# ezorita/seeq

Hardware: AMD Instinct MI355X
Metric: lines/s scanned (20 bp pattern, d=3, 150 bp reads; GB/s in gb_per_s) (higher is better)
Workload: dtype int (u16 automaton state ids; exact-pass columns u32 bit-vectors)

## Files before the change

seeq_amd/csrc/seeq_device.hip:

```cpp
#include <hip/hip_runtime.h>

#include <errno.h>
#include <pthread.h>
#include <stdint.h>
#include <stdio.h>
#include <stdlib.h>
#include <string.h>
#include <time.h>

#include "seeq_amd.h"
#include "seeq_kernel_core.h"
extern "C" {
#include "seeq_pattern.h"
}

static thread_local char g_last_error[256] = "";

static int hip_fail(hipError_t e, const char *what, int err_no)
{
   snprintf(g_last_error, sizeof g_last_error, "%s: %s", what, hipGetErrorString(e));
   seeqerr = 0;
   errno = err_no;
   return -1;
}

#define HIP_TRY(call, err_no)                                        \
   do {                                                              \
      hipError_t e_ = (call);                                        \
      if (e_ != hipSuccess) return hip_fail(e_, #call, (err_no));    \
   } while (0)

extern "C" const char *seeqdevLastError(void) { return g_last_error; }

static int use_device(int device)
{
   int cur = -1;
   if (hipGetDevice(&cur) == hipSuccess && cur == device) return 0;
   HIP_TRY(hipSetDevice(device), ENODEV);
   return 0;
}

extern "C" int seeqdevDeviceCount(void)
{
   int n = 0;
   if (hipGetDeviceCount(&n) != hipSuccess) return 0;
   return n;
}

extern "C" int seeqdevSetDevice(int device)
{
   HIP_TRY(hipSetDevice(device), ENODEV);
   return 0;
}

#include "seeq_types.h"
#include "seeq_scan_common.h"

static constexpr int WG = 256;
static constexpr int TILE = 16384;
static constexpr size_t FUSED_MIN_TILE = 512;
static constexpr int STREAM_NW_HOST = 16;
static constexpr uint32_t STREAM_CH_HOST = 128;
static constexpr size_t MAX_FUSED_GRID = 16384;
static constexpr size_t SAMPLE_BYTES = 65536;

#include "seeq_generic.h"
#include "seeq_scan.h"
#include "seeq_fused_post.h"
#include "seeq_direct.h"
#include "seeq_exact1.h"
#include "seeq_stream.h"
#include "seeq_pair.h"
#include "seeq_packed.h"
#include "seeq_multi.h"
#include "seeq_demux.h"
#include "seeq_tiles.h"
#include "seeq_fastq.h"
#include "seeq_strand.h"
#include "seeq_insert.h"
#include "seeq_tally.h"
#include "seeq_tally_group.h"
#include "seeq_tally_library.h"
#include "seeq_tally_collapse.h"
#include "seeq_qgate.h"
static_assert(sizeof(seeqdev_tally_pair_t) == 24 && sizeof(seeqdev_tally_group_t) == 24, "pair and group entries are written as three 64-bit words");
static_assert(sizeof(seeqdev_tally_collapse_t) == sizeof(uint4) && SEEQ_COLLAPSE_DIRECTIONAL == SEEQDEV_COLLAPSE_DIRECTIONAL && SEEQ_COLLAPSE_ANY == SEEQDEV_COLLAPSE_ANY,
              "collapse rows are written as uint4");
static_assert(sizeof(seeqdev_demux_t) == 16 && sizeof(seeqdev_hit_t) == sizeof(uint4), "demux records are written as uint4");
static_assert(sizeof(seeqdev_insert_t) == sizeof(uint4), "insert records are written as uint4");
static_assert(sizeof(seeqdev_tally_t) == sizeof(uint4) && SEEQ_TALLY_LEN_MAX == SEEQDEV_TALLY_MAX_LEN, "tally entries are written as uint4");
#include "seeq_post.h"
static_assert(STREAM_NW == STREAM_NW_HOST, "waves per k_stream workgroup");
extern "C" {
#include "seeq_dfa.h"
}
#include "seeq_synth.h"

static unsigned long g_pattern_ids = 0;

struct seeqdev_pattern {
   unsigned long id;
   int       wlen, tau, words;
   int       device;
   uint32_t *d_peq;
   char     *keys;
   uint32_t *h_peq;
   int       sdfa_state;
   uint16_t *d_sdfa;
   uint16_t *d_sdfa_skip;
   uint16_t *d_sdfa_restart;
   uint32_t  sdfa_rows, sdfa_final_base;
   int       sdfa_parts;
   int       sdfa_warm;
   double    sdfa_pacc;
   int       pair_state;
   uint16_t *d_pair;
   uint32_t  pair_units;
   uint32_t  pair_states;
   int       pair_parts, pair_mp, pair_warm;
   double    pair_pacc;
   int       quad_state;
   uint16_t *d_quad;
   uint32_t  quad_units;
   uint32_t  quad_states;
   int       quad_parts, quad_mp;
   double    quad_pacc;
   pthread_mutex_t plan_lock;
   struct seeqdev_pattern *twin;
};

#define SEEQ_FOR_WORDS(words, FN, ...) \
   ((words) <= 1 ? FN<1>(__VA_ARGS__) : (words) <= 2 ? FN<2>(__VA_ARGS__) : (words) <= 4 ? FN<4>(__VA_ARGS__) : (words) <= 8 ? FN<8>(__VA_ARGS__) : FN<16>(__VA_ARGS__))

extern "C" seeqdev_pattern_t *seeqdevPatternNew(const char *keys, int wlen, int tau)
{
   seeqerr = 0;
   if (!keys || wlen < 1 || tau < 0 || tau >= wlen) { errno = EINVAL; return NULL; }
   if (wlen > SEEQDEV_MAX_WLEN) {
      snprintf(g_last_error, sizeof g_last_error, "pattern longer than %d positions", SEEQDEV_MAX_WLEN);
      errno = E2BIG;
      return NULL;
   }
   if (seeqdevDeviceCount() < 1) {
      snprintf(g_last_error, sizeof g_last_error, "no HIP device: seeq-mi355x has no CPU matcher");
      errno = ENODEV;
      return NULL;
   }
   seeqdev_pattern *p = (seeqdev_pattern *)calloc(1, sizeof *p);
   if (!p) return NULL;
   p->id = __atomic_add_fetch(&g_pattern_ids, 1ul, __ATOMIC_RELAXED);
   pthread_mutex_init(&p->plan_lock, NULL);
   p->wlen = wlen; p->tau = tau; p->words = seeq_words_for(wlen);
   p->keys = (char *)malloc((size_t)wlen);
   if (p->keys) memcpy(p->keys, keys, (size_t)wlen);
   const size_t nw = (size_t)10 * p->words;
   uint32_t *h = (uint32_t *)malloc(nw * sizeof(uint32_t));
   char *rkeys = (char *)malloc((size_t)wlen);
   if (!h || !rkeys || !p->keys) { free(h); free(rkeys); free(p->keys); free(p); errno = ENOMEM; return NULL; }
   for (int i = 0; i < wlen; i++) rkeys[i] = keys[wlen - 1 - i];
   seeq_build_peq(keys, wlen, p->words, h);
   seeq_build_peq(rkeys, wlen, p->words, h + 5 * p->words);
   hipError_t e = hipGetDevice(&p->device);
   if (e == hipSuccess) e = hipMalloc((void **)&p->d_peq, nw * sizeof(uint32_t));
   if (e == hipSuccess) e = hipMemcpy(p->d_peq, h, nw * sizeof(uint32_t), hipMemcpyHostToDevice);
   free(rkeys);
   p->h_peq = h;
   if (e != hipSuccess) {
      hip_fail(e, "seeqdevPatternNew", e == hipErrorOutOfMemory ? ENOMEM : EIO);
      if (p->d_peq) (void)hipFree(p->d_peq);
      free(p->keys);
      free(h);
      free(p);
      return NULL;
   }
   return p;
}

extern "C" int seeqdevPatternDevice(const seeqdev_pattern_t *p) { return p ? p->device : -1; }

extern "C" void seeqdevPatternFree(seeqdev_pattern_t *p)
{
   if (!p) return;
   if (p->twin) seeqdevPatternFree(p->twin);
   (void)use_device(p->device);
   if (p->d_peq) (void)hipFree(p->d_peq);
   if (p->d_sdfa) (void)hipFree(p->d_sdfa);
   if (p->d_sdfa_skip) (void)hipFree(p->d_sdfa_skip);
   if (p->d_sdfa_restart) (void)hipFree(p->d_sdfa_restart);
   if (p->d_pair) (void)hipFree(p->d_pair);
   if (p->d_quad) (void)hipFree(p->d_quad);
   pthread_mutex_destroy(&p->plan_lock);
   free(p->keys);
   free(p->h_peq);
   free(p);
}

static void pattern_plan_stream(seeqdev_pattern *mp, bool complete_only)
{
   pthread_mutex_lock(&mp->plan_lock);
   if (mp->sdfa_state == 0 && mp->keys) {
      int state = -1;
      seeq_dfa_t *d = seeq_dfa_plan_stream(mp->keys, mp->wlen, mp->tau, complete_only ? 1 : 0);
      if (d) {
         const size_t bytes = (size_t)d->nrows * 16;
         uint16_t *skip = seeq_dfa_skip_variant(d);
         uint16_t *rst = d->nparts > 1 ? seeq_dfa_restart_variant(d) : nullptr;
         uint16_t *t0 = nullptr, *t1 = nullptr, *t2 = nullptr;
         if (skip && (rst || d->nparts <= 1) && hipMalloc((void **)&t0, bytes) == hipSuccess && hipMemcpy(t0, d->table, bytes, hipMemcpyHostToDevice) == hipSuccess &&
             hipMalloc((void **)&t1, bytes) == hipSuccess && hipMemcpy(t1, skip, bytes, hipMemcpyHostToDevice) == hipSuccess &&
             (!rst || (hipMalloc((void **)&t2, bytes) == hipSuccess && hipMemcpy(t2, rst, bytes, hipMemcpyHostToDevice) == hipSuccess))) {
            mp->d_sdfa = t0; mp->d_sdfa_skip = t1; mp->d_sdfa_restart = t2;
            mp->sdfa_rows = d->nrows;
            mp->sdfa_final_base = d->acc_final;
            mp->sdfa_parts = d->nparts;
            mp->sdfa_warm = d->warm;
            mp->sdfa_pacc = d->p_accept;
            state = 1;
         } else {
            if (t0) (void)hipFree(t0);
            if (t1) (void)hipFree(t1);
            if (t2) (void)hipFree(t2);
         }
         free(skip);
         free(rst);
         seeq_dfa_free(d);
      }
      __atomic_store_n(&mp->sdfa_state, state, __ATOMIC_RELEASE);
   }
   pthread_mutex_unlock(&mp->plan_lock);
}

static void pattern_plan_pair(seeqdev_pattern *mp)
{
   pthread_mutex_lock(&mp->plan_lock);
   if (mp->pair_state == 0 && mp->keys) {
      int state = -1;
      seeq_pair_t *d = seeq_pair_plan(mp->keys, mp->wlen, mp->tau);
      if (d) {
         const size_t bytes = d->table_bytes;
         uint16_t *t0 = nullptr;
         if (hipMalloc((void **)&t0, bytes) == hipSuccess && hipMemcpy(t0, d->table, bytes, hipMemcpyHostToDevice) == hipSuccess) {
            mp->d_pair = t0;
            mp->pair_units = d->table_bytes / 16;
            mp->pair_states = d->nstates;
            mp->pair_parts = d->nparts; mp->pair_mp = d->mp; mp->pair_warm = d->warm;
            mp->pair_pacc = d->p_accept;
            state = 1;
         } else if (t0) {
            (void)hipFree(t0);
         }
         seeq_pair_free(d);
      }
      __atomic_store_n(&mp->pair_state, state, __ATOMIC_RELEASE);
   }
   pthread_mutex_unlock(&mp->plan_lock);
}

static void pattern_plan_quad(seeqdev_pattern *mp)
{
   pthread_mutex_lock(&mp->plan_lock);
   if (mp->quad_state == 0 && mp->keys) {
      int state = -1;
      seeq_quad_t *d = seeq_quad_plan(mp->keys, mp->wlen, mp->tau);
      if (d) {
         uint16_t *t0 = nullptr;
         if (hipMalloc((void **)&t0, d->table_bytes) == hipSuccess && hipMemcpy(t0, d->table, d->table_bytes, hipMemcpyHostToDevice) == hipSuccess) {
            mp->d_quad = t0;
            mp->quad_units = d->table_bytes / 16;
            mp->quad_states = d->nstates;
            mp->quad_parts = d->nparts; mp->quad_mp = d->mp;
            mp->quad_pacc = d->p_accept;
            state = 1;
         } else if (t0) {
            (void)hipFree(t0);
         }
         seeq_quad_free(d);
      }
      __atomic_store_n(&mp->quad_state, state, __ATOMIC_RELEASE);
   }
   pthread_mutex_unlock(&mp->plan_lock);
}

struct MultiPlan {
   int            npat;
   unsigned long  ids[SEEQ_MULTI_MAX];
   int            state;
   seeqdev_pattern upat;
   uint16_t      *d_res_next;
   uint32_t      *d_res_mask;
   uint32_t       res_states;
   int            maxspan;
   int            m[SEEQ_MULTI_MAX], tau[SEEQ_MULTI_MAX], fw[SEEQ_MULTI_MAX];
   uint32_t      *d_eq;
   int            eq_options;
   uint32_t       pair_states, raw_states;
   int            lp_min, exact;
};

static void multi_plan_free(MultiPlan *mp)
{
   if (!mp) return;
   if (mp->d_res_next) (void)hipFree(mp->d_res_next);
   if (mp->d_res_mask) (void)hipFree(mp->d_res_mask);
   if (mp->d_eq) (void)hipFree(mp->d_eq);
   if (mp->upat.d_pair) (void)hipFree(mp->upat.d_pair);
   if (mp->upat.d_peq) (void)hipFree(mp->upat.d_peq);
   free(mp->upat.h_peq);
   free(mp);
}

static MultiPlan *multi_plan_for(MultiPlan **slot, const seeqdev_pattern_t *const *pats, int npat)
{
   MultiPlan *mp = *slot;
   if (mp && mp->npat == npat) {
      bool same = true;
      for (int k = 0; k < npat; k++) same = same && mp->ids[k] == pats[k]->id;
      if (same) return mp;
   }
   multi_plan_free(mp);
   *slot = mp = (MultiPlan *)calloc(1, sizeof *mp);
   if (!mp) return NULL;
   mp->npat = npat;
   mp->state = -1;
   mp->eq_options = -1;
   for (int k = 0; k < npat; k++) mp->ids[k] = pats[k]->id;
   if (npat < 2 || npat > SEEQ_MULTI_MAX) return mp;
   const char *keys[SEEQ_MULTI_MAX];
   for (int k = 0; k < npat; k++) {
      if (!pats[k]->keys || pats[k]->wlen > FUSED_MAX_WLEN2) return mp;
      keys[k] = pats[k]->keys; mp->m[k] = pats[k]->wlen; mp->tau[k] = pats[k]->tau;
      mp->fw[k] = pats[k]->wlen <= FUSED_MAX_WLEN ? 1 : 2;
   }
   seeq_multi_t *d = seeq_multi_build(keys, mp->m, mp->tau, npat);
   if (!d) return mp;
   if (d->maxspan <= FUSED_MAX_WLEN2) {
      seeqdev_pattern &u = mp->upat;
      u.id = __atomic_add_fetch(&g_pattern_ids, 1ul, __ATOMIC_RELAXED);
      u.wlen = d->maxspan; u.tau = 0; u.words = seeq_words_for(d->maxspan);
      u.device = pats[0]->device;
      u.sdfa_state = -1;
      u.h_peq = (uint32_t *)calloc((size_t)10 * u.words, sizeof(uint32_t));
      bool ok = u.h_peq != NULL;
      ok = ok && hipMalloc((void **)&u.d_peq, (size_t)10 * u.words * sizeof(uint32_t)) == hipSuccess;
      ok = ok && hipMemset(u.d_peq, 0, (size_t)10 * u.words * sizeof(uint32_t)) == hipSuccess;
      ok = ok && hipMalloc((void **)&u.d_pair, d->pair->table_bytes) == hipSuccess;
      ok = ok && hipMemcpy(u.d_pair, d->pair->table, d->pair->table_bytes, hipMemcpyHostToDevice) == hipSuccess;
      ok = ok && hipMalloc((void **)&mp->d_res_next, (size_t)d->res_states * 16) == hipSuccess;
      ok = ok && hipMemcpy(mp->d_res_next, d->res_next, (size_t)d->res_states * 16, hipMemcpyHostToDevice) == hipSuccess;
      ok = ok && hipMalloc((void **)&mp->d_res_mask, (size_t)d->res_states * 4) == hipSuccess;
      ok = ok && hipMemcpy(mp->d_res_mask, d->res_mask, (size_t)d->res_states * 4, hipMemcpyHostToDevice) == hipSuccess;
      ok = ok && hipMalloc((void **)&mp->d_eq, (size_t)npat * 1536 * sizeof(uint32_t)) == hipSuccess;
      if (ok) {
         u.pair_state = 1;
         u.pair_units = d->pair->table_bytes / 16;
         u.pair_states = d->pair->nstates;
         u.pair_parts = npat; u.pair_mp = d->pair->mp; u.pair_warm = d->pair->warm;
         u.pair_pacc = d->pair->p_accept;
         mp->res_states = d->res_states;
         mp->maxspan = d->maxspan;
         mp->pair_states = d->pair->nstates; mp->raw_states = d->pair->nstates_raw;
         mp->exact = d->res_exact;
         mp->lp_min = d->lp[0];
         for (int k = 1; k < npat; k++) if (d->lp[k] < mp->lp_min) mp->lp_min = d->lp[k];
         mp->state = 1;
      }
   }
   seeq_multi_free(d);
   return mp;
}

#include "seeq_plan.h"
#include "seeq_workspace.h"
#include "seeq_rerun.h"

struct OccMemo { const void *fn; size_t lds; int per_cu; };

struct EventPair {
   hipEvent_t ev[2];
   bool       made;
   float      ms;
   int begin(bool on, hipStream_t st)
   {
      if (!on) return 0;
      if (!made) {
         HIP_TRY(hipEventCreate(&ev[0]), EIO);
         HIP_TRY(hipEventCreate(&ev[1]), EIO);
         made = true;
      }
      HIP_TRY(hipEventRecord(ev[0], st), EIO);
      return 0;
   }
   int end(bool on, hipStream_t st)
   {
      if (on) HIP_TRY(hipEventRecord(ev[1], st), EIO);
      return 0;
   }
   void read(bool on)
   {
      ms = 0.f;
      if (on && made) (void)hipEventElapsedTime(&ms, ev[0], ev[1]);
   }
};

static constexpr size_t PACKED_SEG_READS_DEFAULT = (size_t)1 << 26;

struct seeqdev_scan {
   hipStream_t stream;
   bool        own_stream;
   int         device;
   EventPair   tm_h2d;
   float      *launch_ms; size_t cap_launch_ms;
   unsigned long long *clk_probe;
   size_t      cap_clk_probe;
   float       clk_mhz;
   bool        clk_valid;
   int         ncu;
   size_t      lds_per_wg;
   size_t      lds_per_cu;
   ScanKnobs   knobs;
   OccMemo     occ[8]; int nocc;
   bool        last_filter;
   int         last_plan[16];
   bool        last_packed_quad;
   size_t      pk_seg_reads;
   Workspace   ws;
   uint32_t *line_start;  size_t cap_lines;
   uint32_t *tile_cnt;    size_t cap_tiles;
   uint64_t *hitmask, *hdrmask; uint32_t *wave_off, *hdr_off; size_t cap_chunks;
   uint4    *ent;
   uint32_t *hit_start, *hit_line, *nh, *hit_col, *nh_sum; size_t cap_hitlines;
   struct OnePassWs {
      uint32_t *tile_cl, *tile_hits, *tile_dirty; uint64_t *tile_dmask;
      uint4    *tmp;
      uint32_t *wg_hits;
      uint32_t *wg_part;
      uint32_t *wg_lastnl;
   } ow;
   size_t cap_ftiles, cap_slices;
   uint32_t *d_eqtab, *h_eqtab;
   unsigned long eq_pat_id; int eq_options;
   double avg_line;
   double line_hint;
   uint8_t *h_sample;
   const void *avg_text; size_t avg_nbytes;
   int force_path;
   int last_path;
   seeqdev_hit_t *records; uint64_t *rec_off; size_t cap_records;
   seeqdev_hit_t *fq_rec; uint64_t *fq_off; uint32_t *fq_bsum; size_t cap_fq;
   FastqCnt *d_fqcnt, *h_fqcnt;
   bool fq_ws;
   bool fastq;
   bool fq_done;
   int  fq_want;
   uint32_t *scan_ws;           size_t cap_scan_ws;
   uint32_t *lead_fidx, *lead_flag, *lead_wend; unsigned long long *lead_key; size_t cap_lead;
   Counters *d_cnt;
   Counters *h_cnt;
   uint8_t *h_str;
   uint32_t *h_strout; size_t cap_strout;
   uint32_t  str_seq;
   uint8_t *d_text; size_t cap_text;
   seeqdev_counts_t *multi_cnt; size_t *multi_first; int multi_n, cap_multi_n;
   seeqdev_hit_t *multi_rec; size_t cap_multi_rec, multi_nrec;
   struct MultiPlan *mplan;
   bool      multi_active;
   int       multi_rc;
   uint32_t *ml_mask, *ml_first, *ml_last; size_t cap_ml;
   uint32_t *mp_idx, *mp_nh; size_t cap_mp;
   uint32_t *m_bsum; size_t cap_m_bsum;
   Counters *d_mcnt, *h_mcnt;
   MultiExact *d_mx, *h_mx; size_t mx_slots, mx_next;
   uint32_t *m_scan_ws; size_t cap_m_scan_ws;
   int       last_multi;
   uint32_t *dm_key, *dm_aux; size_t cap_dm_lines;
   uint4    *dm_out; size_t cap_dm_out;
   DemuxCnt *d_dmcnt, *h_dmcnt;
   size_t    dm_nrec;
   uint64_t  dm_nlines;
   seeqdev_hit_t *side_rec; uint64_t *side_off; size_t cap_side;
   uint4    *st_mrg; uint64_t *st_mrg_off; uint32_t *st_bsum; size_t cap_st_mrg;
   StrandCnt *d_stcnt, *h_stcnt;
   EventPair tm_st;
   uint4    *ins_jn; uint32_t *ins_bsum; uint64_t *ins_bbytes; size_t cap_ins_jn;
   uint4    *ins_rec; uint64_t *ins_off, *ins_pos; size_t cap_ins;
   InsertCnt *d_inscnt, *h_inscnt;
   size_t    ins_n;
   uint64_t  ins_text_bytes;
   bool      ins_staged; size_t ins_staged_nbytes;
   EventPair tm_ins;
   bool      ins_done;
   uint64_t *tl_key0, *tl_key1; uint32_t *tl_mat, *tl_sum, *tl_stat; size_t cap_tl;
   seeqdev_tally_t *tl_tab; size_t cap_tl_tab;
   TallyCnt *d_tlcnt, *h_tlcnt;
   size_t    tl_n;
   EventPair tm_tl;
   uint32_t *th_line; uint64_t *th_key; uint32_t *th_stat; size_t cap_th;
   size_t    th_n;
   uint32_t  th_key_bits;
   bool      th_done;
   bool      dm_done;
   uint64_t *tg_g0, *tg_g1; uint32_t *tg_sum, *tg_stat; size_t cap_tg;
   seeqdev_tally_pair_t *tg_pairs; size_t cap_tg_pairs;
   seeqdev_tally_group_t *tg_groups; size_t cap_tg_groups;
   TallyGroupCnt *d_tgcnt, *h_tgcnt;
   size_t    tg_np, tg_ng;
   EventPair tm_tg;
   uint64_t *lb_key; uint32_t *lb_id; size_t cap_lb;
   size_t    lb_n;
   int       lb_mismatch;
   uint32_t *lb_sum; size_t cap_lb_sum;
   uint4    *lb_nstat; size_t cap_lb_near;
   TallyLibCnt *d_lbcnt, *h_lbcnt;
   bool      tg_done;
   uint64_t  tg_npaired; uint32_t tg_max_len;
   uint32_t *tc_parent, *tc_proot; uint64_t *tc_pread; uint32_t *tc_rsum; uint64_t *tc_qsum; CollapseWg *tc_wst; size_t cap_tc;
   seeqdev_tally_collapse_t *tc_groups; uint4 *tc_gst; size_t cap_tc_groups;
   CollapseCnt *d_tccnt, *h_tccnt;
   size_t    tc_np, tc_ng;
   EventPair tm_tc;
   uint8_t  *qg_kind; uint32_t *qg_bsum; size_t cap_qg;
   uint4    *qg_rec; uint64_t *qg_off; size_t cap_qg_out;
   QGateCnt *d_qgcnt, *h_qgcnt;
   size_t    qg_n, qg_nsrc;
   bool      qg_done;
   bool      qg_from_inserts;
   EventPair tm_qg;
   uint32_t *pk_cand, *pk_slot, *pk_coff; uint64_t *pk_bmask; size_t cap_pk_reads;
   uint8_t  *pk_stage; size_t cap_pk_stage;
   uint8_t  *d_unpack; size_t cap_unpack;
   uint32_t *pk_last; size_t cap_pk_last;
   bool      is_packed; seeqdev_packed_t packed;
   const seeqdev_pattern *pat; const void *text; size_t nbytes; int options, want;
   bool ran;
   int  last_runs;
   seeqdev_counts_t counts;
   bool prof;
   hipEvent_t *ev;
   size_t nev_seg;
   size_t prof_segs;
   float acc_ms[4];
   float fwd_ms_avg;
   size_t seg_bytes;
   bool user_reserved;
   RerunFallback fallback;
   bool sample_dirty;
   unsigned sample_age;
};

static_assert(sizeof(seeqdev_scan) <= 8192, "seeqdev_scan has outgrown the tests' stand-in context");

static void *ws_hip_alloc(void *, int kind, size_t bytes)
{
   void *g = NULL;
   const hipError_t e = kind == WS_DEVICE ? hipMalloc(&g, bytes ? bytes : 16)
                      : hipHostMalloc(&g, bytes ? bytes : 16, kind == WS_COHERENT ? hipHostMallocCoherent : hipHostMallocDefault);
   if (e == hipSuccess) return g;
   (void)hipGetLastError();
   hip_fail(e, kind == WS_DEVICE ? "hipMalloc(workspace)" : "hipHostMalloc(workspace)", ENOMEM);
   return NULL;
}

static void ws_hip_release(void *, int kind, void *p)
{
   if (kind == WS_DEVICE) (void)hipFree(p);
   else (void)hipHostFree(p);
}

static int ws_hip_copy(void *ctx, int kind, void *dst, const void *src, size_t bytes)
{
   const hipStream_t st = ((seeqdev_scan *)ctx)->stream;
   HIP_TRY(hipStreamSynchronize(st), EIO);
   if (kind != WS_DEVICE) { memcpy(dst, src, bytes); return 0; }
   HIP_TRY(hipMemcpyAsync(dst, src, bytes, hipMemcpyDeviceToDevice, st), EIO);
   HIP_TRY(hipStreamSynchronize(st), EIO);
   return 0;
}

extern "C" seeqdev_scan_t *seeqdevScanNew(void *hip_stream)
{
   seeqerr = 0;
   if (seeqdevDeviceCount() < 1) {
      snprintf(g_last_error, sizeof g_last_error, "no HIP device: seeq-mi355x has no CPU matcher");
      errno = ENODEV;
      return NULL;
   }
   seeqdev_scan *s = (seeqdev_scan *)calloc(1, sizeof *s);
   if (!s) return NULL;
   if (hipGetDevice(&s->device) != hipSuccess) s->device = 0;
   s->ws.hooks = {ws_hip_alloc, ws_hip_release, s, ws_hip_copy};
   s->seg_bytes = (size_t)0xF0000000u;
   const char *env = getenv("SEEQ_SEGMENT_BYTES");
   if (env && atoll(env) >= 65536) s->seg_bytes = ((size_t)atoll(env) + 15) & ~(size_t)15;
   if (s->seg_bytes > 0xFFFF0000ull) s->seg_bytes = 0xFFFF0000ull;
   hipError_t e = hipSuccess;
   if (hip_stream) s->stream = (hipStream_t)hip_stream;
   else {
      e = hipStreamCreateWithFlags(&s->stream, hipStreamDefault);
      s->own_stream = true;
   }
   if (e == hipSuccess && ws_make(&s->ws, {{s->d_cnt, sizeof(Counters)}, {s->h_cnt, sizeof(Counters), WS_PINNED}, {s->h_eqtab, 2048 * sizeof(uint32_t), WS_PINNED},
                                           {s->d_eqtab, 2048 * sizeof(uint32_t)}, {s->h_sample, SAMPLE_BYTES, WS_PINNED}}))
      e = hipErrorOutOfMemory;
   {
      const char *pe = getenv("SEEQ_PATH");
      s->force_path = pe ? (!strcmp(pe, "generic") ? 1 : !strcmp(pe, "fused") ? 2 : 0) : 0;
      ScanKnobs &kn = s->knobs;
      const char *v;
      v = getenv("SEEQ_FUSED_KERNEL"); kn.kernel = v ? (!strcmp(v, "stream") ? 1 : !strcmp(v, "direct") ? 2 : !strcmp(v, "pair") ? 3 : 0) : 0;
      v = getenv("SEEQ_NO_LEADERS");   kn.no_leaders = v && atoi(v) == 1;
      v = getenv("SEEQ_TILE_BYTES");   kn.tile_bytes = v ? atoi(v) : 0;
      v = getenv("SEEQ_NO_FILTER");    kn.no_filter = v && atoi(v) == 1;
      v = getenv("SEEQ_STREAM_SUB");   kn.no_sub = v && atoi(v) == 0;
      v = getenv("SEEQ_STREAM_WU");    kn.min_wu = v ? atoi(v) : 0;
      v = getenv("SEEQ_NO_MYERS");     kn.no_myers = v && atoi(v) == 1;
      v = getenv("SEEQ_NO_WINDOW");    kn.no_window = v && atoi(v) == 1;
      v = getenv("SEEQ_EXPLAIN");      kn.explain = v && atoi(v) == 1;
      v = getenv("SEEQ_PACKED_QUAD");  kn.no_packed_quad = v && atoi(v) == 0;
      v = getenv("SEEQ_PACKED_SEG_READS");
      s->pk_seg_reads = v && atol(v) >= 64 && (size_t)atol(v) <= ((size_t)1 << 26) ? (size_t)atol(v) & ~(size_t)63 : PACKED_SEG_READS_DEFAULT;
      s->ncu = 256;
      s->lds_per_wg = 65536;
      s->lds_per_cu = 65536;
      int dev = 0;
      hipDeviceProp_t prop;
      if (e == hipSuccess && hipGetDevice(&dev) == hipSuccess && hipGetDeviceProperties(&prop, dev) == hipSuccess)
      { s->ncu = prop.multiProcessorCount; s->lds_per_wg = prop.sharedMemPerBlock; s->lds_per_cu = prop.maxSharedMemoryPerMultiProcessor; }
   }
   if (e != hipSuccess) {
      hip_fail(e, "seeqdevScanNew", EIO);
      seeqdevScanFree(s);
      return NULL;
   }
   return s;
}

extern "C" void seeqdevScanFree(seeqdev_scan_t *s)
{
   if (!s) return;
   (void)use_device(s->device);
   for (EventPair *t : {&s->tm_h2d, &s->tm_st, &s->tm_ins, &s->tm_tl, &s->tm_tg, &s->tm_tc, &s->tm_qg})
      if (t->made) { (void)hipEventDestroy(t->ev[0]); (void)hipEventDestroy(t->ev[1]); }
   (void)hipStreamSynchronize(s->stream);
   ws_free_all(&s->ws);
   multi_plan_free(s->mplan);
   for (size_t i = 0; i < 4 * s->nev_seg; i++) (void)hipEventDestroy(s->ev[i]);
   free(s->ev);
   free(s->launch_ms);
   free(s->multi_cnt); free(s->multi_first);
   if (s->own_stream && s->stream) (void)hipStreamDestroy(s->stream);
   free(s);
}

static int ensure_scan_ws(seeqdev_scan *s, size_t nblocks)
{
   return ws_grow(&s->ws, &s->cap_scan_ws, nblocks, {{s->scan_ws, nblocks * sizeof(uint32_t)}});
}

static size_t fastq_bsum_words(size_t n) { return 2 * (n / SEEQ_TILE + 2); }

static int reserve_impl(seeqdev_scan *s, size_t max_bytes, size_t max_lines, size_t max_hitlines, size_t max_records)
{
   seeqerr = 0;
   if (!s) { errno = EINVAL; return -1; }
   Workspace *w = &s->ws;
   if (max_bytes) {
      const size_t seg = max_bytes < s->seg_bytes ? max_bytes : s->seg_bytes;
      const size_t tiles = (seg + TILE - 1) / TILE + 1;
      if (ws_grow(w, &s->cap_tiles, tiles, {{s->tile_cnt, tiles * sizeof(uint32_t)}})) return -1;
      const size_t ftiles = seg / FUSED_MIN_TILE + 2;
      const size_t slices = MAX_FUSED_GRID;
      if (ws_grow(w, &s->cap_ftiles, ftiles, {{s->ow.tile_cl, ftiles * sizeof(uint32_t)}, {s->ow.tile_dirty, ftiles * sizeof(uint32_t)},
                                              {s->ow.tile_dmask, ftiles * sizeof(uint64_t)}, {s->ow.tile_hits, ftiles * sizeof(uint32_t)}})) return -1;
      if (ws_grow(w, &s->cap_slices, slices, {{s->ow.wg_hits, slices * sizeof(uint32_t)}, {s->ow.wg_part, 4 * slices * sizeof(uint32_t)},
                                              {s->ow.wg_lastnl, slices * sizeof(uint32_t)}})) return -1;
   }
   if (max_lines > s->cap_lines) {
      const size_t chunks = (max_lines + 63) / 64 + 1;
      if (ws_grow(w, &s->cap_lines, max_lines, {{s->line_start, (max_lines + 1) * sizeof(uint32_t)}, {s->hitmask, chunks * sizeof(uint64_t)},
                                                {s->hdrmask, chunks * sizeof(uint64_t)}, {s->wave_off, chunks * sizeof(uint32_t)},
                                                {s->hdr_off, chunks * sizeof(uint32_t)}})) return -1;
      s->cap_chunks = chunks;
   }
   if (ws_grow(w, &s->cap_hitlines, max_hitlines, {{s->hit_start, max_hitlines * sizeof(uint32_t)}, {s->hit_line, max_hitlines * sizeof(uint32_t)},
                                                   {s->ow.tmp, max_hitlines * sizeof(uint4)}, {s->nh, max_hitlines * sizeof(uint32_t)},
                                                   {s->hit_col, max_hitlines * sizeof(uint32_t)}, {s->ent, max_hitlines * sizeof(uint4)},
                                                   {s->nh_sum, 2 * (max_hitlines / 256 + 2) * sizeof(uint32_t)}})) return -1;
   if (s->fq_ws && max_records > s->cap_records) {
      if (ws_grow(w, &s->cap_records, max_records, {{s->records, max_records * sizeof(seeqdev_hit_t)}, {s->rec_off, max_records * sizeof(uint64_t)},
                                                    {s->fq_rec, max_records * sizeof(seeqdev_hit_t)}, {s->fq_off, max_records * sizeof(uint64_t)},
                                                    {s->fq_bsum, fastq_bsum_words(max_records) * sizeof(uint32_t)}})) return -1;
      s->cap_fq = s->cap_records;
   } else if (ws_grow(w, &s->cap_records, max_records, {{s->records, max_records * sizeof(seeqdev_hit_t)}, {s->rec_off, max_records * sizeof(uint64_t)}})) return -1;
   if (s->fq_ws) {
      const size_t n = s->cap_records;
      if (ws_grow(w, &s->cap_fq, n, {{s->fq_rec, n * sizeof(seeqdev_hit_t)}, {s->fq_off, n * sizeof(uint64_t)}, {s->fq_bsum, fastq_bsum_words(n) * sizeof(uint32_t)}})) return -1;
      if (ws_make(w, {{s->d_fqcnt, sizeof(FastqCnt)}, {s->h_fqcnt, sizeof(FastqCnt), WS_PINNED}})) return -1;
   }
   size_t largest = s->cap_tiles;
   if (s->cap_chunks > largest) largest = s->cap_chunks;
   if (s->cap_hitlines > largest) largest = s->cap_hitlines;
   if (s->cap_ftiles > largest) largest = s->cap_ftiles;
   size_t nb = largest / SCAN_BLOCK + 2;
   if (3 * (s->cap_ftiles / SCAN_BLOCK + 2) > nb) nb = 3 * (s->cap_ftiles / SCAN_BLOCK + 2);
   return ensure_scan_ws(s, nb);
}

extern "C" int seeqdevScanReserve(seeqdev_scan_t *s, size_t max_bytes, size_t max_lines, size_t max_hitlines,
                                  size_t max_records)
{
   if (reserve_impl(s, max_bytes, max_lines, max_hitlines, max_records)) return -1;
   if (max_lines) s->user_reserved = true;
   return 0;
}

extern "C" int seeqdevScanSetLineHint(seeqdev_scan_t *s, double avg_bytes_per_line)
{
   if (!s || avg_bytes_per_line < 0) { errno = EINVAL; return -1; }
   s->line_hint = avg_bytes_per_line;
   return 0;
}

extern "C" int seeqdevScanLastPath(const seeqdev_scan_t *s) { return s ? s->last_path : 0; }
extern "C" int seeqdevScanLastFilter(const seeqdev_scan_t *s) { return s && s->last_filter ? 1 : 0; }
extern "C" int seeqdevScanLastPlan(const seeqdev_scan_t *s, int out[16])
{
   if (!s || !out) { errno = EINVAL; return -1; }
   memcpy(out, s->last_plan, sizeof s->last_plan);
   return 0;
}
extern "C" int seeqdevScanLastPackedQuad(const seeqdev_scan_t *s) { return s && s->last_packed_quad ? 1 : 0; }
extern "C" int seeqdevScanLastRuns(const seeqdev_scan_t *s) { return s ? s->last_runs : 0; }

extern "C" int seeqdevScanFallback(const seeqdev_scan_t *s, unsigned *bits, int *scans_left)
{
   if (!s) { errno = EINVAL; return -1; }
   if (bits) *bits = s->fallback.bits;
   if (scans_left) *scans_left = s->fallback.bits ? s->fallback.ttl : 0;
   return 0;
}

extern "C" int seeqdevScanSetProfiling(seeqdev_scan_t *s, int on)
{
   if (!s) { errno = EINVAL; return -1; }
   s->prof = on != 0;
   return 0;
}

extern "C" int seeqdevScanLastTimes(const seeqdev_scan_t *s, float ms[4])
{
   if (!s || !ms) { errno = EINVAL; return -1; }
   for (int i = 0; i < 4; i++) ms[i] = s->acc_ms[i];
   return 0;
}

static int occupancy_of(seeqdev_scan *s, const void *fn, int threads, size_t lds)
{
   for (int i = 0; i < s->nocc; i++)
      if (s->occ[i].fn == fn && s->occ[i].lds == lds) return s->occ[i].per_cu;
   if (lds) HIP_TRY(hipFuncSetAttribute(fn, hipFuncAttributeMaxDynamicSharedMemorySize, (int)lds), EIO);
   int per_cu = 0;
   if (hipOccupancyMaxActiveBlocksPerMultiprocessor(&per_cu, fn, threads, lds) != hipSuccess || per_cu < 1) per_cu = 1;
   OccMemo &m = s->occ[s->nocc < 8 ? s->nocc++ : 7];
   m.fn = fn; m.lds = lds; m.per_cu = per_cu;
   return per_cu;
}

static int multi_post(seeqdev_scan *s, const ScanPlan &plan, const ScanArgs &ua, hipStream_t st);

static void pattern_automata(const seeqdev_pattern *p, PlanAutomata *au)
{
   au->sdfa_state = __atomic_load_n(&p->sdfa_state, __ATOMIC_ACQUIRE);
   au->sdfa_parts = p->sdfa_parts; au->sdfa_warm = p->sdfa_warm; au->sdfa_pacc = p->sdfa_pacc;
   au->pair_state = __atomic_load_n(&p->pair_state, __ATOMIC_ACQUIRE);
   au->pair_warm = p->pair_warm; au->pair_pacc = p->pair_pacc;
}

static void plan_ensure(void *ctx, int which, int complete_only, PlanAutomata *au)
{
   seeqdev_pattern *mp = (seeqdev_pattern *)ctx;
   if (which == 0) pattern_plan_stream(mp, complete_only != 0);
   else pattern_plan_pair(mp);
   pattern_automata(mp, au);
}

struct SegRun {
   ScanPlan  plan;
   int       nw;
   uint32_t  tile_bytes;
   unsigned  fused_grid, grid_lines;
   const void *stream_fn;
   size_t    dfa_lds, seg_bytes, nseg;
};

static unsigned capped_grid(const seeqdev_scan *s, size_t n, size_t per_cu)
{
   const size_t blocks = (n + WG - 1) / WG, cap = (size_t)s->ncu * per_cu;
   const unsigned g = (unsigned)(blocks < cap ? blocks : cap);
   return g ? g : 1;
}

static int prof_events(seeqdev_scan *s, size_t nseg)
{
   s->prof_segs = 0;
   if (!s->prof) return 0;
   if (nseg > s->nev_seg) {
      hipEvent_t *g = (hipEvent_t *)realloc(s->ev, 4 * nseg * sizeof(hipEvent_t));
      if (!g) { seeqerr = 0; errno = ENOMEM; return -1; }
      s->ev = g;
      while (s->nev_seg < nseg) {
         hipEvent_t *e4 = s->ev + 4 * s->nev_seg;
         for (int i = 0; i < 4; i++) {
            const hipError_t e = hipEventCreate(&e4[i]);
            if (e != hipSuccess) { while (i--) (void)hipEventDestroy(e4[i]); return hip_fail(e, "hipEventCreate", EIO); }
         }
         s->nev_seg++;
      }
   }
   s->prof_segs = nseg;
   return 0;
}

static int seg_end_flags(bool need_nh, bool superset, bool nh_is_count) { return (need_nh ? 1 : 0) | (superset && !nh_is_count ? 2 : 0); }

static int verify_variant(int want, int options, bool nh_is_count, int seg_flags, uint32_t *fin)
{
   const int var = (want == SEEQDEV_WANT_RECORDS && (options & 3) == SQ_BEST) ? VERIFY_BEST : nh_is_count ? VERIFY_ALL : VERIFY_ANY;
   *fin = (want == SEEQDEV_WANT_RECORDS && var == VERIFY_ALL) ? 0u : 1u + (uint32_t)seg_flags;
   return var;
}

static void eq_fill(uint32_t *tab, const seeqdev_pattern *pat, int options, int fw)
{
   const int Wp = pat->words;
   for (int dir = 0; dir < 2; dir++)
      for (int b = 0; b < 256; b++) {
         const uint8_t cls = sq_class_of((uint32_t)b, options);
         uint64_t v;
         if (cls < 5) {
            const uint32_t *q = pat->h_peq + (dir * 5 + cls) * Wp;
            const uint64_t col = (uint64_t)q[0] | (Wp > 1 ? (uint64_t)q[1] << 32 : 0);
            v = col << (32 * fw - pat->wlen);
         } else {
            v = cls == SQC_TERM ? FUSED_FLAG_TERM : FUSED_FLAG_SKIP;
         }
         uint32_t *dst = tab + (size_t)(dir * 256 + b) * fw;
         dst[0] = (uint32_t)v;
         if (fw == 2) dst[1] = (uint32_t)(v >> 32);
      }
}

static int eq_tables_upload(seeqdev_scan *s, const seeqdev_pattern *pat, int options, int fw)
{
   if (s->eq_pat_id == pat->id && s->eq_options == options) return 0;
   eq_fill(s->h_eqtab, pat, options, fw);
   memcpy(s->h_eqtab + (size_t)512 * fw, s->h_eqtab, (size_t)256 * fw * sizeof(uint32_t));
   s->h_eqtab[(size_t)512 * fw + (size_t)'\n' * fw] |= 3u;
   HIP_TRY(hipMemcpyAsync(s->d_eqtab, s->h_eqtab, (size_t)768 * fw * sizeof(uint32_t), hipMemcpyHostToDevice, s->stream), EIO);
   HIP_TRY(hipStreamSynchronize(s->stream), EIO);
   s->eq_pat_id = pat->id;
   s->eq_options = options;
   return 0;
}

static int run_setup(seeqdev_scan *s, SegRun &r)
{
   const seeqdev_pattern *pat = s->pat;
   const bool fasta = (s->options & SEEQDEV_FASTA) != 0, single = (s->options & SEEQDEV_SINGLELINE) != 0;
   r.grid_lines = capped_grid(s, s->cap_lines, 16);

   PlanIn pin;
   memset(&pin, 0, sizeof pin);
   pin.wlen = pat->wlen; pin.tau = pat->tau; pin.options = s->options; pin.want = s->want;
   pin.avg_line = s->avg_line; pin.line_hint = s->line_hint; pin.force_path = s->force_path;
   const RerunFallback &fb = s->fallback;
   pin.no_stream = fb.no_stream(); pin.force_ll = fb.force_ll(); pin.no_stream_nd = fb.no_stream_nd(); pin.no_window = fb.no_window();
   pin.no_leaders = fb.no_leaders(); pin.sample_dirty = s->sample_dirty; pin.multi_active = s->multi_active;
   pin.seg_bytes = s->seg_bytes; pin.kn = &s->knobs;
   PlanAutomata au;
   pattern_automata(pat, &au);
   r.plan = seeq_plan_scan(pin, au, plan_ensure, const_cast<seeqdev_pattern *>(pat));
   const ScanPlan &plan = r.plan;
   if (s->knobs.explain) seeq_plan_print(stderr, pin, au, plan);
   if (plan.rc) return plan.rc;
   const int fw = plan.fw, stream_wu = plan.stream_wu;
   if (plan.use_fused) {
      if (plan.use_stream) {
         r.nw = STREAM_NW;
         r.tile_bytes = 64u * STREAM_CH_HOST;
#define SEEQ_STREAM_FN(...) (stream_wu == 4 ? (const void *)k_stream<4, __VA_ARGS__> : stream_wu == 6 ? (const void *)k_stream<6, __VA_ARGS__> \
                                                                                                      : (const void *)k_stream<8, __VA_ARGS__>)
         r.stream_fn = plan.stream_sub == 2 ? SEEQ_STREAM_FN(false, false, 2)
                     : plan.stream_sub ? (plan.stream_ll ? SEEQ_STREAM_FN(false, true, 1) : SEEQ_STREAM_FN(false, false, 1))
                     : plan.stream_ll ? (fasta ? SEEQ_STREAM_FN(true, true) : SEEQ_STREAM_FN(false, true))
                     : fasta ? SEEQ_STREAM_FN(true, false) : SEEQ_STREAM_FN(false, false);
#undef SEEQ_STREAM_FN
         r.dfa_lds = ((size_t)pat->sdfa_rows * 16 + 15) & ~(size_t)15;
         if (plan.use_myers) {
#define SEEQ_MYERS_FN(FA, MY) (stream_wu == 16 ? (const void *)k_stream<16, FA, true, 0, MY> : (const void *)k_stream<32, FA, true, 0, MY>)
            r.stream_fn = fw == 1 ? (fasta ? SEEQ_MYERS_FN(true, 1) : SEEQ_MYERS_FN(false, 1)) : (fasta ? SEEQ_MYERS_FN(true, 2) : SEEQ_MYERS_FN(false, 2));
#undef SEEQ_MYERS_FN
            r.dfa_lds = (size_t)256 * fw * sizeof(uint32_t);
         }
         if (plan.use_pair) {
#define SEEQ_PAIR_FN(...) (stream_wu == 4 ? (const void *)k_pair<4, __VA_ARGS__> : stream_wu == 5 ? (const void *)k_pair<5, __VA_ARGS__> : stream_wu == 6 ? (const void *)k_pair<6, __VA_ARGS__> \
                          : stream_wu == 7 ? (const void *)k_pair<7, __VA_ARGS__> : (const void *)k_pair<8, __VA_ARGS__>)
            r.stream_fn = fasta ? SEEQ_PAIR_FN(true) : plan.ig ? SEEQ_PAIR_FN(false, true) : plan.pair_ll ? SEEQ_PAIR_FN(false, false, true) : SEEQ_PAIR_FN(false);
            r.dfa_lds = (size_t)pat->pair_units * 16;
#undef SEEQ_PAIR_FN
         }
      } else {
         r.nw = 4;
         double want = s->avg_line * 63.5;
         if (want < 512) want = 512;
         if (want > DIRECT_MAXRR * 1024) want = DIRECT_MAXRR * 1024;
         r.tile_bytes = ((uint32_t)want) & ~15u;
         if (s->knobs.tile_bytes >= 512 && s->knobs.tile_bytes <= DIRECT_MAXRR * 1024) r.tile_bytes = (uint32_t)s->knobs.tile_bytes & ~15u;
      }
      const void *fn = plan.use_stream ? r.stream_fn : fw == 1 ? (const void *)k_direct<4, 1> : (const void *)k_direct<4, 2>;
      const int per_cu = occupancy_of(s, fn, 64 * r.nw, r.dfa_lds);
      if (per_cu < 0) return -1;
      r.fused_grid = (unsigned)(s->ncu * per_cu);
      if ((size_t)r.fused_grid * r.nw > MAX_FUSED_GRID) r.fused_grid = (unsigned)(MAX_FUSED_GRID / r.nw);
      if (eq_tables_upload(s, pat, s->options, fw)) return -1;
   }
   s->last_path = plan.path;
   s->last_filter = plan.filter;
   {
      const int v[16] = {plan.rc, plan.path, plan.fw, plan.use_stream, plan.use_pair, plan.use_myers, plan.filter, plan.stream_ll, plan.stream_sub, plan.stream_wu,
                         plan.verify, plan.order2, plan.leaders, plan.window_ok, plan.ll_restart ? 2 : (plan.ll_filter ? 1 : 0), (int)plan.skip_back};
      memcpy(s->last_plan, v, sizeof v);
   }

   const size_t nbytes = s->nbytes;
   r.seg_bytes = single ? (nbytes ? nbytes : 1) : s->seg_bytes;
   if (single && nbytes > 0xFFFF0000ull) { seeqerr = 0; errno = E2BIG; return -1; }
   r.nseg = nbytes ? (nbytes + r.seg_bytes - 1) / r.seg_bytes : 0;
   if (prof_events(s, r.nseg)) return -1;
   if (s->prof && r.nseg > s->cap_clk_probe) {
      ws_release(&s->ws, s->clk_probe);
      s->cap_clk_probe = 0;
      if (ws_make(&s->ws, {{s->clk_probe, r.nseg * 4 * sizeof(unsigned long long), WS_PINNED}}) == 0) s->cap_clk_probe = r.nseg;
   }
   if (s->prof && s->clk_probe) memset(s->clk_probe, 0, r.nseg * 4 * sizeof(unsigned long long));
   s->clk_valid = s->prof && s->clk_probe && plan.use_pair && plan.use_fused;
   return 0;
}

static int seg_onepass(seeqdev_scan *s, const SegRun &r, ScanArgs &a, size_t sg, hipEvent_t *ev, bool &order2, uint32_t &stream_ntiles)
{
   const ScanPlan &plan = r.plan;
   const seeqdev_pattern *pat = s->pat;
   const seeqdev_scan::OnePassWs &ow = s->ow;
   hipStream_t st = s->stream;

   FusedArgs f;
   memset(&f, 0, sizeof f);
   f.text = a.text; f.nbytes = s->nbytes; f.seg_base = a.seg_base; f.seg_len = a.seg_len; f.first_seg = a.first_seg;
   f.tile_bytes = r.tile_bytes;
   f.ntiles = (uint32_t)(((uint64_t)a.seg_len + r.tile_bytes - 1) / r.tile_bytes);
   stream_ntiles = f.ntiles;
   f.eqtab = s->d_eqtab; f.peq = pat->d_peq;
   f.m = pat->wlen; f.tau = pat->tau; f.options = s->options; f.want = s->want;
   f.tile_cl = ow.tile_cl; f.tile_hits = ow.tile_hits; f.tmp = ow.tmp; f.cap_tmp = (uint32_t)s->cap_hitlines;
   f.wg_hits = ow.wg_hits; f.wg_part = ow.wg_part; f.wg_lastnl = plan.stream_ll ? ow.wg_lastnl : nullptr;
   f.tile_dirty = f.wg_lastnl ? ow.tile_dirty : nullptr;
   f.tile_dmask = f.wg_lastnl ? ow.tile_dmask : nullptr;
   f.cnt = s->d_cnt;
   f.clk_probe = (s->prof && s->clk_probe && plan.use_pair) ? s->clk_probe + 4 * sg : nullptr;
   uint32_t pos_bias = 0;
   if (plan.use_stream) {
      f.dfa = plan.stream_sub == 2 ? pat->d_sdfa_skip : plan.ll_restart ? pat->d_sdfa_restart : pat->d_sdfa; f.dfa_rows = pat->sdfa_rows; f.dfa_final_base = pat->sdfa_final_base;
      f.ll_filter = plan.ll_restart ? 2u : plan.ll_filter ? 1u : 0u;
      f.skip_thr = plan.skip_thr;
      if (plan.use_pair) { f.dfa = pat->d_pair; f.dfa_rows = pat->pair_units; f.dfa_final_base = 0; f.pair = 1; f.ig_thr = plan.ig ? (uint32_t)(pat->wlen - pat->tau) : 0u; }
      if (plan.use_myers) { f.dfa = (const uint16_t *)(s->d_eqtab + (size_t)512 * plan.fw); f.dfa_rows = (uint32_t)(64 * plan.fw); f.dfa_final_base = 0; f.pair = 2; }
      uint64_t room = 0xFFFFFFF0ull - a.seg_len;
      if (room > ((uint64_t)1 << 30)) room = (uint64_t)1 << 30;
      pos_bias = (uint32_t)(a.seg_base < room ? a.seg_base : room) & ~127u;
      f.pos_bias = pos_bias;
   }
   if (ev) { HIP_TRY(hipEventRecord(ev[0], st), EIO); HIP_TRY(hipEventRecord(ev[1], st), EIO); }
   const unsigned nsl = r.fused_grid * r.nw;
   f.slice_cap = f.cap_tmp / nsl;
   if (plan.use_stream) {
      void *kargs[] = {&f};
      HIP_TRY(hipLaunchKernel(r.stream_fn, dim3(r.fused_grid), dim3(64 * (unsigned)r.nw), kargs, r.dfa_lds, st), EIO);
   }
   else if (plan.use_direct && plan.fw == 2) hipLaunchKernelGGL((k_direct<4, 2>), dim3(r.fused_grid), dim3(256), 0, st, f);
   else hipLaunchKernelGGL((k_direct<4, 1>), dim3(r.fused_grid), dim3(256), 0, st, f);
   if (ev) HIP_TRY(hipEventRecord(ev[2], st), EIO);
   const uint32_t order_nb = (f.ntiles + SEEQ_ORDER_BLOCK - 1) / SEEQ_ORDER_BLOCK;
   order2 = plan.order2 && order_nb <= SEEQ_ORDER_MAX_BLOCKS && 2 * (size_t)order_nb <= s->cap_scan_ws;
   if (plan.ig) {
      if (!order2) { snprintf(g_last_error, sizeof g_last_error, "SQ_IGNORE on k_pair needs the three-launch ordering (segment too large for its block sums)"); seeqerr = 0; errno = EIO; return -1; }
      a.ig_thr = f.ig_thr; a.ig_ent = (const uint4 *)s->ent;
      {
         static const char base_of_key[9] = {0, 'A', 'C', 0, 'G', 0, 0, 0, 'T'};
         int cnt[4] = {0, 0, 0, 0}, best = 3;
         for (int i = 0; i < pat->wlen; i++) { const int kb = pat->keys[i] & 0x1F; if (kb == 1) cnt[0]++; else if (kb == 2) cnt[1]++; else if (kb == 4) cnt[2]++; else if (kb == 8) cnt[3]++; }
         for (int b = 2; b >= 0; b--) if (cnt[b] > cnt[best]) best = b;
         const int need = cnt[best] - pat->tau;
         a.ig_need = need > 0 ? (uint32_t)need : 0u;
         a.ig_bval = (uint32_t)(unsigned char)base_of_key[1 << best];
         a.ig_bmask = best == 3 ? 0xDEu : 0xDFu;
      }
   }
   const unsigned rgrid = nsl / 4 + 1 < 2048 ? nsl / 4 + 1 : 2048;
   if (order2) {
      seeq_launch_tiles_post(st, f, (uint32_t)nsl, s->scan_ws, order_nb);
      seeq_launch_order(rgrid, st, f, (uint32_t)nsl, (const uint32_t *)s->scan_ws, order_nb, s->ent);
   }
   else hipLaunchKernelGGL(k_fused_post, dim3(1), dim3(256), 0, st, f, (uint32_t)nsl);
   if (!order2 && (s->want != SEEQDEV_WANT_COUNTLINES || plan.superset)) {
      launch_scanset(st, s->scan_ws, f.tile_hits, f.tile_cl, f.tile_dirty, f.ntiles, nullptr, nullptr, f.tile_dirty ? &s->d_cnt->seg_dirty_tiles : nullptr);
      if (plan.use_stream) hipLaunchKernelGGL(k_stream_reorder, dim3(rgrid), dim3(256), 0, st, f, (uint32_t)nsl, s->hit_start, s->hit_line, s->nh, s->hit_col);
      else hipLaunchKernelGGL(k_fused_reorder, dim3(rgrid), dim3(256), 0, st, f, (uint32_t)nsl, s->hit_start, s->hit_line);
   }
   a.seg_base -= pos_bias;
   a.pos_bias = pos_bias;
   a.tile_dirty = f.tile_dirty; a.tile_dmask = f.tile_dmask; a.stream_ntiles = f.ntiles; a.stream_tile_bytes = r.tile_bytes;
   a.stream_ch = plan.stream_ll ? STREAM_CH_HOST : 0u;
   a.walk_ext = plan.walk_ext; a.ll_restart = plan.ll_restart ? 1u : 0u;
   return 0;
}

template <int W>
static int seg_index_forward(seeqdev_scan *s, const SegRun &r, ScanArgs &a, hipEvent_t *ev)
{
   Counters *c = s->d_cnt;
   hipStream_t st = s->stream;
   if (ev) HIP_TRY(hipEventRecord(ev[0], st), EIO);
   if (s->options & SEEQDEV_SINGLELINE) {
      hipLaunchKernelGGL(k_single_line, dim3(1), dim3(1), 0, st, a);
   } else {
      hipLaunchKernelGGL(k_nl_count, dim3(a.ntiles), dim3(WG), 0, st, a);
      hipLaunchKernelGGL(k_scan_tiles, dim3(1), dim3(WG), 0, st, a.tile_cnt, a.ntiles, &c->seg_nlines);
      hipLaunchKernelGGL(k_index_finalize, dim3(1), dim3(1), 0, st, a);
      hipLaunchKernelGGL(k_nl_write, dim3(a.ntiles), dim3(WG), 0, st, a);
   }
   if (ev) HIP_TRY(hipEventRecord(ev[1], st), EIO);
   hipLaunchKernelGGL(k_forward<W>, dim3(r.grid_lines), dim3(WG), 0, st, a);
   if (ev) HIP_TRY(hipEventRecord(ev[2], st), EIO);
   launch_scan<1>(st, s->scan_ws, a.hitmask, a.wave_off, s->cap_chunks, &c->seg_nlines, 63u, 6u, &c->seg_nhitlines);
   if (s->options & SEEQDEV_FASTA) launch_scan<1>(st, s->scan_ws, a.hdrmask, a.hdr_off, s->cap_chunks, &c->seg_nlines, 63u, 6u, &c->seg_nheaders);
   return 0;
}

template <int W>
static int seg_post(seeqdev_scan *s, const SegRun &r, ScanArgs &a, hipEvent_t *ev, bool order2, uint32_t stream_ntiles)
{
   const ScanPlan &plan = r.plan;
   const int want = s->want, fw = plan.fw;
   Counters *c = s->d_cnt;
   hipStream_t st = s->stream;

   if (!plan.use_fused) hipLaunchKernelGGL(k_compact, dim3(r.grid_lines), dim3(WG), 0, st, a);
   if (!plan.use_fused) hipLaunchKernelGGL(k_seg_mid, dim3(1), dim3(1), 0, st, a);
   const unsigned grid_hits = capped_grid(s, s->cap_hitlines, 16);
   if (order2) seeq_launch_bounds2(grid_hits, st, a, s->ent, s->hit_col);
   else if (plan.use_stream) hipLaunchKernelGGL(k_stream_bounds, dim3(grid_hits), dim3(256), 0, st, a, s->hit_col,
                                           (const uint32_t *)s->ow.tile_cl, stream_ntiles, r.tile_bytes);
   if (s->multi_active) {
      { const int mr = multi_post(s, plan, a, st); if (mr > 0) return -2; if (mr) return -1; }
      hipLaunchKernelGGL(k_seg_end, dim3(1), dim3(1), 0, st, a, 3);
      if (ev) HIP_TRY(hipEventRecord(ev[3], st), EIO);
      HIP_TRY(hipGetLastError(), EIO);
      return 1;
   }
   const uint32_t lead_wback = a.skip_back > 32u ? a.skip_back : 32u;
   if (plan.leaders) {
      if (ws_grow(&s->ws, &s->cap_lead, s->cap_hitlines, {{s->lead_fidx, s->cap_hitlines * sizeof(uint32_t)}, {s->lead_flag, s->cap_hitlines * sizeof(uint32_t)},
                                                          {s->lead_wend, s->cap_hitlines * sizeof(uint32_t)},
                                                          {s->lead_key, s->cap_hitlines * sizeof(unsigned long long)}})) return -1;
      const unsigned nbl = (unsigned)(s->cap_hitlines / LEAD_BLOCK + 1);
      hipLaunchKernelGGL(k_lead_reduce, dim3(nbl), dim3(256), 0, st, a, s->scan_ws);
      hipLaunchKernelGGL(k_lead_top, dim3(1), dim3(256), 0, st, a, s->scan_ws);
      hipLaunchKernelGGL(k_lead_apply, dim3(nbl), dim3(256), 0, st, a, (const uint32_t *)s->hit_col, (const uint32_t *)s->scan_ws, s->lead_fidx, s->lead_flag, s->ow.tmp, lead_wback, plan.lead_best ? s->lead_key : (unsigned long long *)nullptr);
      a.walk_end = s->lead_wend;
      if (plan.lead_best) a.filter = 1u;
      hipLaunchKernelGGL(k_lead_commit, dim3(grid_hits), dim3(256), 0, st, a, s->hit_col, (const uint4 *)s->ow.tmp);
   }
   const uint32_t *hcol = plan.use_stream ? s->hit_col : nullptr;
   uint4 *ecache = (plan.use_fused && plan.need_nh && want == SEEQDEV_WANT_RECORDS) ? s->ow.tmp : nullptr;
   const uint32_t *eqp = (const uint32_t *)s->d_eqtab;
   bool emitted = false;
   if (plan.verify) {
      const int var = verify_variant(want, s->options, plan.nh_is_count, seg_end_flags(plan.need_nh, plan.superset, plan.nh_is_count), &a.fin);
      a.nh_sum = s->nh_sum;
      a.nz_sum = plan.superset && plan.nh_is_count ? s->nh_sum + (s->cap_hitlines / 256 + 2) : nullptr;
      a.vrange = (plan.use_pair ? s->pat->pair_parts > 1 : s->pat->sdfa_parts > 1) ? 512u : 0u;
      seeq_launch_verify(fw, var, grid_hits, st, a, eqp, hcol, ecache);
      if (want == SEEQDEV_WANT_RECORDS && var != VERIFY_ALL) seeq_launch_emit1(grid_hits, st, a, ecache);
      else if (want == SEEQDEV_WANT_RECORDS && ecache)
         seeq_launch_emit_all(fw, grid_hits, grid_hits, st, a, eqp, hcol, ecache);
      emitted = want == SEEQDEV_WANT_RECORDS && (var != VERIFY_ALL || ecache);
   }
   else if (plan.need_nh) {
      if (plan.use_fused) {
   #define SEEQ_COUNT1(WW, WK) hipLaunchKernelGGL((k_exact1<SQ_MODE_COUNT, WW, -1, WK>), dim3(grid_hits), dim3(WG), 0, st, a, eqp, hcol, ecache)
         if (fw == 2) { if (a.stream_ch) SEEQ_COUNT1(2, true); else SEEQ_COUNT1(2, false); }
         else { if (a.stream_ch) SEEQ_COUNT1(1, true); else SEEQ_COUNT1(1, false); }
   #undef SEEQ_COUNT1
      }
      else hipLaunchKernelGGL((k_exact<W, SQ_MODE_COUNT>), dim3(grid_hits), dim3(WG), 0, st, a);
      if (plan.leaders) {
         hipLaunchKernelGGL(k_lead_check, dim3(grid_hits), dim3(256), 0, st, a, (const uint32_t *)s->hit_col, (const uint32_t *)s->lead_flag, lead_wback);
         if (plan.lead_best) {
            hipLaunchKernelGGL(k_lead_best, dim3(grid_hits), dim3(256), 0, st, a, (const uint32_t *)s->lead_fidx, s->lead_key, (const uint4 *)ecache, 0);
            hipLaunchKernelGGL(k_lead_best, dim3(grid_hits), dim3(256), 0, st, a, (const uint32_t *)s->lead_fidx, s->lead_key, (const uint4 *)ecache, 1);
         }
         else hipLaunchKernelGGL(k_lead_lines, dim3(grid_hits < 512 ? grid_hits : 512), dim3(256), 0, st, a, (const uint32_t *)s->lead_fidx, s->lead_flag);
      }
      else if (plan.superset && plan.nh_is_count) hipLaunchKernelGGL(k_count_nonzero, dim3(grid_hits < 512 ? grid_hits : 512), dim3(WG), 0, st, a);
      launch_scan<0>(st, s->scan_ws, a.nh, a.nh, s->cap_hitlines, &c->seg_nhitlines, 0u, 0u, &c->seg_nrec);
   }
   if (want == SEEQDEV_WANT_RECORDS && !emitted) {
      if (!plan.verify) hipLaunchKernelGGL(k_rec_check, dim3(1), dim3(1), 0, st, a);
      if (plan.use_fused) {
         const int mo = (s->options & 3) == SQ_COUNT ? SQ_FIRST : (s->options & 3);
   #define SEEQ_EMIT1(WW, OO, WK) hipLaunchKernelGGL((k_exact1<SQ_MODE_EMIT, WW, OO, WK>), dim3(grid_hits), dim3(WG), 0, st, a, eqp, hcol, ecache)
         if (a.stream_ch) {
            if (fw == 2) { if (mo == SQ_BEST) SEEQ_EMIT1(2, SQ_BEST, true); else SEEQ_EMIT1(2, -1, true); }
            else { if (mo == SQ_BEST) SEEQ_EMIT1(1, SQ_BEST, true); else SEEQ_EMIT1(1, -1, true); }
         } else {
            if (fw == 2) { if (mo == SQ_BEST) SEEQ_EMIT1(2, SQ_BEST, false); else SEEQ_EMIT1(2, -1, false); }
            else { if (mo == SQ_BEST) SEEQ_EMIT1(1, SQ_BEST, false); else SEEQ_EMIT1(1, -1, false); }
         }
   #undef SEEQ_EMIT1
      }
      else {
         hipLaunchKernelGGL((k_exact<W, SQ_MODE_EMIT>), dim3(grid_hits), dim3(WG), 0, st, a);
         hipLaunchKernelGGL(k_rec_offsets, dim3(grid_hits), dim3(WG), 0, st, a);
      }
   }
   return 0;
}

template <int W>
static int run_segments(seeqdev_scan *s)
{
   Counters *c = s->d_cnt;
   hipStream_t st = s->stream;
   HIP_TRY(hipMemsetAsync(c, 0, sizeof(Counters), st), EIO);
   SegRun r;
   memset(&r, 0, sizeof r);
   { const int rc = run_setup(s, r); if (rc) return rc; }
   const ScanPlan &plan = r.plan;
   const seeqdev_pattern *pat = s->pat;
   const size_t nbytes = s->nbytes;
   for (size_t sg = 0; sg < r.nseg; sg++) {
      hipEvent_t *ev = s->prof ? s->ev + 4 * sg : NULL;
      uint32_t stream_ntiles = 0;
      bool order2 = false;
      ScanArgs a;
      memset(&a, 0, sizeof a);
      a.text = (const uint8_t *)s->text;
      a.nbytes = nbytes;
      a.seg_base = (uint64_t)sg * r.seg_bytes;
      a.seg_len = (uint32_t)((nbytes - a.seg_base) < r.seg_bytes ? (nbytes - a.seg_base) : r.seg_bytes);
      a.first_seg = sg == 0;
      a.peq = pat->d_peq;
      a.m = pat->wlen; a.tau = pat->tau; a.options = s->options; a.want = s->want;
      a.line_start = s->line_start; a.cap_lines = (uint32_t)s->cap_lines;
      a.tile_cnt = s->tile_cnt; a.ntiles = (a.seg_len + TILE - 1) / TILE;
      a.hitmask = s->hitmask; a.hdrmask = s->hdrmask; a.wave_off = s->wave_off; a.hdr_off = s->hdr_off;
      a.hit_start = s->hit_start; a.hit_line = s->hit_line; a.cap_hitlines = (uint32_t)s->cap_hitlines; a.nh = s->nh;
      a.records = s->records; a.cap_records = s->cap_records; a.rec_off = s->rec_off;
      a.use_nh = plan.need_nh ? (plan.use_stream ? 3u : 1u) : 0u;
      a.filter = plan.filter ? 1u : 0u;
      a.skip_back = plan.skip_back;
      a.window_ok = plan.window_ok ? 1u : 0u;
      a.cnt = c;

      if (plan.use_fused) { if (seg_onepass(s, r, a, sg, ev, order2, stream_ntiles)) return -1; }
      else if (seg_index_forward<W>(s, r, a, ev)) return -1;
      if (s->want != SEEQDEV_WANT_COUNTLINES || plan.superset) {
         const int pr = seg_post<W>(s, r, a, ev, order2, stream_ntiles);
         if (pr < 0) return pr;
         if (pr > 0) continue;
      }
      if (!a.fin) hipLaunchKernelGGL(k_seg_end, dim3(1), dim3(1), 0, st, a, seg_end_flags(plan.need_nh, plan.superset, plan.nh_is_count));
      if (ev) HIP_TRY(hipEventRecord(ev[3], st), EIO);
      HIP_TRY(hipGetLastError(), EIO);
   }
   HIP_TRY(hipMemcpyAsync(s->h_cnt, c, sizeof(Counters), hipMemcpyDeviceToHost, st), EIO);
   return 0;
}


static int run_packed(seeqdev_scan *s)
{
   const seeqdev_pattern *pat = s->pat;
   const seeqdev_packed_t &b = s->packed;
   const int options = s->options, want = s->want;
   const int match_opt = options & 3;
   const bool nh_is_count = want == SEEQDEV_WANT_COUNTMATCH || (want == SEEQDEV_WANT_RECORDS && match_opt == SQ_ALL);
   const int seg_flags = seg_end_flags(true, true, nh_is_count);
   const int fw = pat->wlen <= FUSED_MAX_WLEN ? 1 : 2;
   Counters *c = s->d_cnt;
   hipStream_t st = s->stream;
   const uint32_t L = b.read_len;
   const bool direct = !(want == SEEQDEV_WANT_RECORDS && match_opt == SQ_ALL);
   const uint32_t pitch = (L + 1u + 15u) & ~15u;
   size_t PACKED_SEG_READS = s->pk_seg_reads;
   const size_t stage_lines_max = (size_t)(0xFFFF0000ull / pitch);
   if (!direct && PACKED_SEG_READS + 64u * MAX_FUSED_GRID > stage_lines_max)
      PACKED_SEG_READS = (stage_lines_max - 64u * MAX_FUSED_GRID) & ~(size_t)63;
   const size_t seg_reads = b.nreads < PACKED_SEG_READS ? (size_t)b.nreads : PACKED_SEG_READS;
   const size_t cap_use = (!direct && s->cap_hitlines > stage_lines_max) ? stage_lines_max : s->cap_hitlines;
   if (ws_grow(&s->ws, &s->cap_pk_reads, seg_reads, {{s->pk_cand, seg_reads * sizeof(uint32_t)}, {s->pk_slot, seg_reads * sizeof(uint32_t)},
                                                     {s->pk_coff, (seg_reads / 64 + 1) * sizeof(uint32_t)},
                                                     {s->pk_bmask, (seg_reads / 64 + 1) * sizeof(uint64_t)}})) return -1;
   if (!direct && ws_grow(&s->ws, &s->cap_pk_stage, cap_use * (size_t)pitch, {{s->pk_stage, cap_use * (size_t)pitch + 64}})) return -1;
   if (ws_grow(&s->ws, &s->cap_pk_last, s->cap_hitlines, {{s->pk_last, s->cap_hitlines * sizeof(uint32_t)}})) return -1;
   if (ensure_scan_ws(s, seg_reads / SCAN_BLOCK + 2)) return -1;
   if (eq_tables_upload(s, pat, options, fw)) return -1;
   HIP_TRY(hipMemsetAsync(c, 0, sizeof(Counters), st), EIO);
   s->clk_valid = false;
   const bool quad = pat->quad_state == 1 && !s->knobs.no_packed_quad && (pat->quad_pacc - pat->pair_pacc) * (double)L <= 0.04;
   s->last_packed_quad = quad;
   const size_t dfa_lds = quad ? (size_t)pat->quad_units * 16 : (size_t)pat->pair_units * 16;
   const void *walk_fn = quad ? (const void *)k_packed_walk<true> : (const void *)k_packed_walk<false>;
   int per_cu = occupancy_of(s, walk_fn, 64 * STREAM_NW, dfa_lds);
   if (per_cu < 0) return -1;
   unsigned wgrid = (unsigned)(s->ncu * per_cu);
   {
      const size_t nblocks = (seg_reads + 63) / 64, need = (nblocks + STREAM_NW_HOST - 1) / STREAM_NW_HOST;
      if (need < wgrid) wgrid = (unsigned)(need ? need : 1);
   }
   const unsigned grid_hits = capped_grid(s, s->cap_hitlines, 16);
   const size_t nseg = (size_t)((b.nreads + PACKED_SEG_READS - 1) / PACKED_SEG_READS);
   if (prof_events(s, nseg)) return -1;
   for (size_t sg = 0; sg < nseg; sg++) {
      hipEvent_t *ev = s->prof ? s->ev + 4 * sg : NULL;
      PackedArgs p;
      memset(&p, 0, sizeof p);
      p.bases = (const uint8_t *)b.bases; p.nmask = (const uint8_t *)b.nmask;
      p.first = (uint64_t)sg * PACKED_SEG_READS;
      p.nreads = (uint32_t)(b.nreads - p.first < PACKED_SEG_READS ? b.nreads - p.first : PACKED_SEG_READS);
      p.read_len = L; p.stride = b.stride; p.nstride = b.nstride;
      p.total_bytes = b.nreads * (uint64_t)b.stride;
      p.dfa = quad ? pat->d_quad : pat->d_pair; p.dfa_units = quad ? pat->quad_units : pat->pair_units;
      p.cand = s->pk_cand; p.cslot = s->pk_slot; p.boff = s->pk_coff; p.bmask = s->pk_bmask; p.stage = direct ? nullptr : s->pk_stage;
      p.wave_cap = (uint32_t)(cap_use / ((size_t)wgrid * STREAM_NW_HOST));
      p.pitch = pitch;
      p.hit_start = s->hit_start; p.hit_line = s->hit_line; p.hit_col = s->hit_col; p.hit_last = s->pk_last; p.nh = s->nh;
      p.cap = (uint32_t)cap_use;
      p.line_base = p.first;
      p.cnt = c;
      if (ev) { HIP_TRY(hipEventRecord(ev[0], st), EIO); HIP_TRY(hipEventRecord(ev[1], st), EIO); }
      {
         void *kargs[] = {&p};
         HIP_TRY(hipLaunchKernel(walk_fn, dim3(wgrid), dim3(64 * STREAM_NW), kargs, dfa_lds, st), EIO);
      }
      if (ev) HIP_TRY(hipEventRecord(ev[2], st), EIO);
      launch_scanset(st, s->scan_ws, s->pk_coff, nullptr, nullptr, (p.nreads + 63u) >> 6, &c->seg_nhitlines, nullptr, nullptr);
      hipLaunchKernelGGL(k_packed_counts, dim3(1), dim3(1), 0, st, p);
      hipLaunchKernelGGL(k_packed_list, dim3((unsigned)(((size_t)p.nreads / 1024 + 4) / 4)), dim3(256), 0, st, p);
      ScanArgs a;
      memset(&a, 0, sizeof a);
      a.text = direct ? nullptr : s->pk_stage;
      a.nbytes = direct ? 0 : cap_use * (uint64_t)pitch;
      a.seg_base = 0; a.seg_len = (uint32_t)a.nbytes; a.first_seg = sg == 0;
      a.peq = pat->d_peq;
      a.m = pat->wlen; a.tau = pat->tau; a.options = options & ~(MASK_NONDNA | MASK_INPUT); a.want = want;
      a.hit_start = s->hit_start; a.hit_line = s->hit_line; a.cap_hitlines = (uint32_t)s->cap_hitlines; a.nh = s->nh;
      a.records = s->records; a.cap_records = s->cap_records; a.rec_off = s->rec_off;
      a.use_nh = 3u; a.filter = 1u;
      a.skip_back = (uint32_t)(pat->wlen + pat->tau);
      a.hit_last = s->pk_last;
      a.window_ok = 1u;
      a.cnt = c;
      a.rec_pitch = L + 1u;
      const uint32_t *eqp = (const uint32_t *)s->d_eqtab;
      const uint32_t *hcol = s->hit_col;
      uint4 *ecache = want == SEEQDEV_WANT_RECORDS ? s->ow.tmp : nullptr;
      {
         const int var = verify_variant(want, options, nh_is_count, seg_flags, &a.fin);
         a.nh_sum = s->nh_sum;
         a.nz_sum = nh_is_count ? s->nh_sum + (s->cap_hitlines / 256 + 2) : nullptr;
         if (direct) seeq_launch_verify_packed(fw, var, grid_hits, st, a, b.bases, b.nmask, b.stride, b.nstride, L, p.total_bytes,
                                               b.nmask ? b.nreads * (uint64_t)b.nstride : 0ull, eqp, hcol, ecache);
         else seeq_launch_verify(fw, var, grid_hits, st, a, eqp, hcol, ecache);
         if (want == SEEQDEV_WANT_RECORDS && var != VERIFY_ALL) seeq_launch_emit1(grid_hits, st, a, ecache);
         else if (want == SEEQDEV_WANT_RECORDS) {
            seeq_launch_emit_all(fw, grid_hits, grid_hits, st, a, eqp, hcol, ecache);
            hipLaunchKernelGGL(k_seg_end, dim3(1), dim3(1), 0, st, a, seg_flags);
         }
      }
      if (ev) HIP_TRY(hipEventRecord(ev[3], st), EIO);
      HIP_TRY(hipGetLastError(), EIO);
   }
   HIP_TRY(hipMemcpyAsync(s->h_cnt, c, sizeof(Counters), hipMemcpyDeviceToHost, st), EIO);
   s->last_path = 8;
   s->last_filter = true;
   memset(s->last_plan, 0, sizeof s->last_plan);
   s->last_plan[1] = 8; s->last_plan[6] = 1;
   return 0;
}


static int dispatch_run(seeqdev_scan *s)
{
   if (s->is_packed) return run_packed(s);
   return SEEQ_FOR_WORDS(s->pat->words, run_segments, s);
}

static int scan_args_ok(const seeqdev_scan_t *s, const seeqdev_pattern_t *const *pats, int npat, int options, int want)
{
   if (!s || !pats || npat < 1 || want < 0 || want > 2) return 0;
   for (int k = 0; k < npat; k++) {
      if (!pats[k]) return 0;
      if (pats[k]->device != s->device) {
         snprintf(g_last_error, sizeof g_last_error, "pattern lives on device %d, scan context on device %d", pats[k]->device, s->device);
         return 0;
      }
   }
   return !((options & SEEQDEV_FASTQ) && (options & (SEEQDEV_FASTA | SEEQDEV_SINGLELINE | MASK_INPUT)));
}

static int scan_setup(seeqdev_scan_t *s, const seeqdev_pattern_t *pat, const void *d_text, size_t nbytes, int options, int want, int hl_div)
{
   seeqerr = 0;
   if (!scan_args_ok(s, &pat, 1, options, want) || (!d_text && nbytes)) { errno = EINVAL; return -1; }
   const bool fastq = (options & SEEQDEV_FASTQ) != 0;
   if (use_device(s->device)) return -1;
   s->fastq = fastq; s->fq_done = false; s->fq_want = want;
   if (fastq) {
      s->fq_ws = true;
      options &= ~SEEQDEV_FASTQ;
      if (want != SEEQDEV_WANT_RECORDS) {
         options = (options & ~MASK_MATCH) | (want == SEEQDEV_WANT_COUNTLINES ? SQ_FIRST : SQ_ALL);
         want = SEEQDEV_WANT_RECORDS;
      }
   }
   s->pat = pat; s->text = d_text; s->nbytes = nbytes; s->options = options; s->want = want;
   s->ran = false;
   s->is_packed = false;
   s->fallback.age();
   const RerunCaps w = seeq_first_reservation(nbytes < s->seg_bytes ? nbytes : s->seg_bytes, (options & SEEQDEV_SINGLELINE) != 0, hl_div,
                                              {s->cap_lines, s->cap_hitlines, s->cap_records}, s->user_reserved);
   if (reserve_impl(s, nbytes ? nbytes : 1, w.lines, w.hitlines, w.records)) return -1;
   if (s->line_hint > 0) {
      s->avg_line = s->line_hint;
   } else if (!(options & SEEQDEV_SINGLELINE) && nbytes && (s->avg_text != d_text || s->avg_nbytes != nbytes || ++s->sample_age >= 64)) {
      s->sample_age = 0;
      const size_t n = nbytes < SAMPLE_BYTES ? nbytes : SAMPLE_BYTES;
      HIP_TRY(hipMemcpyAsync(s->h_sample, d_text, n, hipMemcpyDeviceToHost, s->stream), EIO);
      HIP_TRY(hipStreamSynchronize(s->stream), EIO);
      size_t nl = 0;
      size_t foreign = 0;
      for (size_t i = 0; i < n; i++) {
         const uint8_t b = s->h_sample[i];
         nl += b == '\n';
         foreign += b != '\n' && sq_class_of(b, 0) >= 5;
      }
      s->avg_line = nl ? (double)n / (double)nl : 1e9;
      s->sample_dirty = foreign * 4096 > n;
      s->avg_text = d_text;
      s->avg_nbytes = nbytes;
   }
   return 0;
}

extern "C" int seeqdevScanRun(seeqdev_scan_t *s, const seeqdev_pattern_t *pat, const void *d_text, size_t nbytes,
                              int options, int want)
{
   if (scan_setup(s, pat, d_text, nbytes, options, want, SEEQ_HL_DIV)) return -1;
   if (dispatch_run(s)) return -1;
   s->ran = true;
   return 0;
}

static int rerun_next(seeqdev_scan *s, int run, const Counters &u, const Counters *per = NULL, int npat = 0)
{
   const RerunStep d = seeq_rerun_decide(run, {s->cap_lines, s->cap_hitlines, s->cap_records}, u, per, npat);
   s->fallback.note(d.note);
   if (d.verdict == RERUN_DONE) return 0;
   if (d.verdict == RERUN_NOT_ONE_WALK) return 2;
   if (d.verdict == RERUN_AGAIN) return reserve_impl(s, s->nbytes, d.cap.lines, d.cap.hitlines, d.cap.records) ? -1 : 1;
   const bool bad = d.verdict == RERUN_BAD_ENTRY;
   snprintf(g_last_error, sizeof g_last_error, "%s", bad ? "internal inconsistency in the hit list (k_stream_bounds)" : "workspace did not converge");
   errno = bad ? EIO : ENOMEM;
   return -1;
}

static seeqdev_counts_t counts_of(const Counters &h) { return {h.lines, h.matchlines, h.hits, h.records, h.headers}; }

static uint32_t cap_u32(size_t cap) { return (uint32_t)(cap < 0xFFFFFFFFull ? cap : 0xFFFFFFFFull); }

static int counters_copy(seeqdev_scan *s, void *h, const void *d, size_t bytes)
{
   HIP_TRY(hipGetLastError(), EIO);
   HIP_TRY(hipMemcpyAsync(h, d, bytes, hipMemcpyDeviceToHost, s->stream), EIO);
   return 0;
}

static int counters_fetch(seeqdev_scan *s, void *h, const void *d, size_t bytes)
{
   if (counters_copy(s, h, d, bytes)) return -1;
   HIP_TRY(hipStreamSynchronize(s->stream), EIO);
   return 0;
}

static int copy_out(seeqdev_scan *s, void *host_out, const void *base, size_t elem, size_t have, size_t first, size_t n)
{
   seeqerr = 0;
   if (!s || (!host_out && n) || first > have || n > have - first) { errno = EINVAL; return -1; }
   if (n == 0) return 0;
   if (use_device(s->device)) return -1;
   HIP_TRY(hipMemcpyAsync(host_out, (const char *)base + first * elem, n * elem, hipMemcpyDeviceToHost, s->stream), EIO);
   HIP_TRY(hipStreamSynchronize(s->stream), EIO);
   return 0;
}

static int fastq_filter(seeqdev_scan *s, const void *in, const uint64_t *off_in, uint32_t n, bool demux, FastqCnt *cnt)
{
   const hipStream_t st = s->stream;
   FastqArgs a;
   memset(&a, 0, sizeof a);
   a.in = (const uint4 *)in; a.off_in = off_in;
   a.out = (uint4 *)s->fq_rec; a.off_out = s->fq_off;
   a.n = n; a.cap_out = cap_u32(s->cap_fq);
   a.nb = (uint32_t)seeq_tiles_of(n);
   a.bsum = s->fq_bsum;
   a.cnt = s->d_fqcnt;
   if (!s->fq_rec || !s->d_fqcnt || n > s->cap_fq || fastq_bsum_words(s->cap_fq) < 2 * (size_t)a.nb) {
      snprintf(g_last_error, sizeof g_last_error, "FASTQ filter: %u records, scratch for %zu", n, s->cap_fq);
      errno = EIO;
      return -1;
   }
   HIP_TRY(hipMemsetAsync(s->d_fqcnt, 0, sizeof(FastqCnt), st), EIO);
   if (demux) hipLaunchKernelGGL(k_fastq_reduce<true>, dim3(a.nb), dim3(SEEQ_TILE_WG), 0, st, a);
   else hipLaunchKernelGGL(k_fastq_reduce<false>, dim3(a.nb), dim3(SEEQ_TILE_WG), 0, st, a);
   hipLaunchKernelGGL(k_fastq_top, dim3(1), dim3(SEEQ_TILE_WG), 0, st, a);
   hipLaunchKernelGGL(k_fastq_apply, dim3(a.nb), dim3(SEEQ_TILE_WG), 0, st, a);
   if (counters_fetch(s, s->h_fqcnt, s->d_fqcnt, sizeof(FastqCnt))) return -1;
   *cnt = *s->h_fqcnt;
   if (cnt->bad || cnt->kept > n || cnt->opened > cnt->kept) {
      snprintf(g_last_error, sizeof g_last_error, "internal inconsistency in the FASTQ filter (flags %u, %u of %u kept, %u lines)", cnt->bad, cnt->kept, n, cnt->opened);
      errno = EIO;
      return -1;
   }
   return 0;
}

static int fastq_filter_swap(seeqdev_scan *s, uint32_t n, FastqCnt *cnt)
{
   if (s->cap_fq != s->cap_records) {
      snprintf(g_last_error, sizeof g_last_error, "FASTQ filter: scratch for %zu records, record workspace for %zu", s->cap_fq, s->cap_records);
      errno = EIO;
      return -1;
   }
   if (fastq_filter(s, s->records, s->rec_off, n, false, cnt)) return -1;
   seeqdev_hit_t *r = s->records; s->records = s->fq_rec; s->fq_rec = r;
   uint64_t *o = s->rec_off; s->rec_off = s->fq_off; s->fq_off = o;
   return 0;
}

static int fastq_finish(seeqdev_scan *s, const Counters &h)
{
   if (h.records > 0xFFFFFFFFull) {
      snprintf(g_last_error, sizeof g_last_error, "SEEQDEV_FASTQ: more than 2^32 - 1 records to filter");
      errno = E2BIG;
      return -1;
   }
   FastqCnt f;
   f.kept = f.opened = 0;
   if (h.records && fastq_filter_swap(s, (uint32_t)h.records, &f)) return -1;
   s->counts.nlines = fastq_nlines(h.lines);
   s->counts.nmatchlines = f.opened;
   s->counts.nhits = s->fq_want == SEEQDEV_WANT_COUNTLINES ? f.opened : f.kept;
   s->counts.nrecords = s->fq_want == SEEQDEV_WANT_RECORDS ? f.kept : 0;
   s->counts.nheaders = 0;
   return 0;
}

extern "C" int seeqdevScanFetch(seeqdev_scan_t *s, seeqdev_counts_t *counts)
{
   seeqerr = 0;
   if (!s || !s->ran) { errno = EINVAL; return -1; }
   if (use_device(s->device)) return -1;
   for (int run = 0;; run++) {
      HIP_TRY(hipStreamSynchronize(s->stream), EIO);
      const Counters h = *s->h_cnt;
      const int next = rerun_next(s, run, h);
      if (next < 0) return -1;
      if (next == 0) {
         s->last_runs = run + 1;
         if (s->fastq) {
            if (!s->fq_done && fastq_finish(s, h)) return -1;
            s->fq_done = true;
         } else s->counts = counts_of(h);
         if (counts) *counts = s->counts;
         for (int i = 0; i < 4; i++) s->acc_ms[i] = 0.f;
         s->fwd_ms_avg = 0.f;
         for (size_t sg = 0; sg < s->prof_segs; sg++) {
            hipEvent_t *ev = s->ev + 4 * sg;
            float t01 = 0, t12 = 0, t23 = 0;
            if (sg == 0 && s->prof_segs > s->cap_launch_ms) {
               float *g = (float *)realloc(s->launch_ms, s->prof_segs * sizeof(float));
               if (g) { s->launch_ms = g; s->cap_launch_ms = s->prof_segs; }
            }
            (void)hipEventElapsedTime(&t01, ev[0], ev[1]);
            (void)hipEventElapsedTime(&t12, ev[1], ev[2]);
            (void)hipEventElapsedTime(&t23, ev[2], ev[3]);
            s->acc_ms[0] += t01; s->acc_ms[1] += t12; s->acc_ms[2] += t23; s->acc_ms[3] += t01 + t12 + t23;
            if (sg < s->cap_launch_ms) s->launch_ms[sg] = t12;
         }
         s->clk_mhz = 0.f;
         if (s->clk_valid && s->prof_segs && s->clk_probe && s->cap_clk_probe >= s->prof_segs) {
            double sum = 0; size_t nn = 0;
            for (size_t sg = 0; sg < s->prof_segs; sg++) {
               const unsigned long long *q = s->clk_probe + 4 * sg;
               if (q[3] > q[1] && q[2] > q[0]) { sum += (double)(q[2] - q[0]) / (double)(q[3] - q[1]) * 100.0; nn++; }
            }
            if (nn) s->clk_mhz = (float)(sum / (double)nn);
         }
         if (s->prof_segs) s->fwd_ms_avg = s->acc_ms[1] / (float)s->prof_segs;
         s->tm_h2d.read(s->prof);
         return 0;
      }
      if (dispatch_run(s)) return -1;
   }
}

extern "C" const seeqdev_hit_t *seeqdevScanRecordsDevice(const seeqdev_scan_t *s) { return s ? s->records : NULL; }

extern "C" int seeqdevScanCopyRecords(seeqdev_scan_t *s, seeqdev_hit_t *host_out, size_t first, size_t n)
{
   return copy_out(s, host_out, s ? s->records : NULL, sizeof(seeqdev_hit_t), s ? (size_t)s->counts.nrecords : 0, first, n);
}

extern "C" int seeqdevScanPacked(seeqdev_scan_t *s, const seeqdev_pattern_t *pat, const seeqdev_packed_t *batch, int options, int want)
{
   seeqerr = 0;
   if (!scan_args_ok(s, &pat, 1, options, want) || !batch || (batch->nreads && !batch->bases)) { errno = EINVAL; return -1; }
   if (batch->read_len < 1 || batch->read_len > 256 || batch->stride < (batch->read_len + 3) / 4 ||
       (batch->nmask && batch->nstride < (batch->read_len + 7) / 8) || (options & (MASK_INPUT | SEEQDEV_FASTA | SEEQDEV_SINGLELINE | SEEQDEV_FASTQ))) { errno = EINVAL; return -1; }
   if (use_device(s->device)) return -1;
   s->fastq = false;
   seeqdev_pattern *mp = const_cast<seeqdev_pattern *>(pat);
   if (pat->wlen <= FUSED_MAX_WLEN2 && __atomic_load_n(&mp->pair_state, __ATOMIC_ACQUIRE) == 0) pattern_plan_pair(mp);
   if (pat->wlen <= FUSED_MAX_WLEN2 && mp->pair_state == 1 && __atomic_load_n(&mp->quad_state, __ATOMIC_ACQUIRE) == 0) pattern_plan_quad(mp);
   if (pat->wlen > FUSED_MAX_WLEN2 || mp->pair_state != 1) {
      const size_t tbytes = (size_t)batch->nreads * (batch->read_len + 1u);
      if (ws_grow(&s->ws, &s->cap_unpack, tbytes, {{s->d_unpack, tbytes + 64}})) return -1;
      if (batch->nreads) {
         const uint64_t threads = batch->nreads * (uint64_t)(batch->read_len / 16u + 1u), blocks = (threads + 255) / 256;
         if (blocks > 0x7FFFFFFFull) { errno = E2BIG; return -1; }
         hipLaunchKernelGGL(k_unpack_ascii, dim3((unsigned)blocks), dim3(256), 0, s->stream, (const uint8_t *)batch->bases, (const uint8_t *)batch->nmask,
                            batch->nreads, batch->read_len, batch->stride, batch->nstride, s->d_unpack);
         HIP_TRY(hipGetLastError(), EIO);
      }
      s->avg_text = NULL;
      return seeqdevScanRun(s, pat, s->d_unpack, tbytes, options, want);
   }
   s->pat = pat; s->text = NULL; s->nbytes = 0; s->options = options; s->want = want;
   s->ran = false;
   s->is_packed = true;
   s->packed = *batch;
   const RerunCaps w = seeq_first_reservation_packed(batch->nreads < s->pk_seg_reads ? (size_t)batch->nreads : s->pk_seg_reads,
                                                     {s->cap_lines, s->cap_hitlines, s->cap_records}, s->user_reserved);
   if (reserve_impl(s, 1, w.lines, w.hitlines, w.records)) return -1;
   if (dispatch_run(s)) return -1;
   s->ran = true;
   return 0;
}

extern "C" int seeqdevPackReadsDevice(const void *d_text, uint64_t nreads, uint32_t read_len, void *d_bases, void *d_nmask, uint32_t stride, uint32_t nstride,
                                      void *hip_stream)
{
   seeqerr = 0;
   if ((!d_text || !d_bases) && nreads) { errno = EINVAL; return -1; }
   if (read_len < 1 || read_len > 256 || stride < (read_len + 3) / 4 || (d_nmask && nstride < (read_len + 7) / 8)) { errno = EINVAL; return -1; }
   if (nreads == 0) return 0;
   const uint64_t blocks = (nreads + 255) / 256;
   if (blocks > 0x7FFFFFFFull) { errno = E2BIG; return -1; }
   hipLaunchKernelGGL(k_pack_ascii, dim3((unsigned)blocks), dim3(256), 0, (hipStream_t)hip_stream, (const uint8_t *)d_text, nreads, read_len,
                      (uint8_t *)d_bases, (uint8_t *)d_nmask, stride, nstride);
   HIP_TRY(hipGetLastError(), EIO);
   return 0;
}

extern "C" long seeqdevPackReads(const char *text, size_t nbytes, uint32_t read_len, void *bases_out, void *nmask_out, uint32_t stride, uint32_t nstride)
{
   seeqerr = 0;
   if (!text || !bases_out || read_len < 1 || read_len > 256 || stride < (read_len + 3) / 4 || (nmask_out && nstride < (read_len + 7) / 8)) { errno = EINVAL; return -1; }
   uint8_t *bo = (uint8_t *)bases_out, *no = (uint8_t *)nmask_out;
   long r = 0;
   size_t p = 0;
   while (p < nbytes) {
      if (p + read_len > nbytes) { errno = EINVAL; return -1; }
      uint8_t *b = bo + (size_t)r * stride, *n = no ? no + (size_t)r * nstride : NULL;
      memset(b, 0, stride);
      if (n) memset(n, 0, nstride);
      for (uint32_t i = 0; i < read_len; i++) {
         const unsigned char ch = (unsigned char)text[p + i];
         const unsigned char up = ch & 0xDF;
         unsigned code;
         if (up == 'A' || up == 'C' || up == 'G' || up == 'T' || up == 'U') code = (ch >> 1) & 3u;
         else if (up == 'N') { code = 0; if (!n) { errno = EINVAL; return -1; } n[i >> 3] |= (uint8_t)(0x80u >> (i & 7)); }
         else { errno = EINVAL; return -1; }
         b[i >> 2] |= (uint8_t)(code << (6 - 2 * (i & 3)));
      }
      p += read_len;
      if (p < nbytes) { if (text[p] != '\n') { errno = EINVAL; return -1; } p++; }
      r++;
   }
   return r;
}

#include "seeq_text_alloc.h"

extern "C" int seeqdevScanCopyOffsets(seeqdev_scan_t *s, uint64_t *host_out, size_t first, size_t n)
{
   return copy_out(s, host_out, s ? s->rec_off : NULL, sizeof(uint64_t), s ? (size_t)s->counts.nrecords : 0, first, n);
}

static int text_ensure(seeqdev_scan *s, size_t nbytes)
{
   if (nbytes <= s->cap_text) return 0;
   const size_t cap = nbytes + (nbytes >> 2) + 4096;
   return ws_grow(&s->ws, &s->cap_text, cap, {{s->d_text, cap}});
}

static int text_upload(seeqdev_scan *s, const char *host_text, size_t nbytes, bool timed)
{
   if (text_ensure(s, nbytes)) return -1;
   if (s->tm_h2d.begin(timed, s->stream)) return -1;
   if (nbytes) HIP_TRY(hipMemcpyAsync(s->d_text, host_text, nbytes, hipMemcpyHostToDevice, s->stream), EIO);
   if (s->tm_h2d.end(timed, s->stream)) return -1;
   s->avg_text = NULL;
   s->ins_staged = false;
   return 0;
}

static int staged_text(seeqdev_scan *s, const char *who, const void **d_text, size_t *nbytes)
{
   if (*d_text) return 0;
   if (!s->ins_staged) {
      snprintf(g_last_error, sizeof g_last_error, "%s: the context holds no staged text of an inserts call", who);
      errno = EINVAL;
      return -1;
   }
   *d_text = s->d_text;
   *nbytes = s->ins_staged_nbytes;
   return 0;
}

static int side_keep(seeqdev_scan *s, size_t n)
{
   if (!n) return 0;
   if (ws_grow(&s->ws, &s->cap_side, n, {{s->side_rec, n * sizeof(seeqdev_hit_t)}, {s->side_off, n * sizeof(uint64_t)}})) return -1;
   HIP_TRY(hipMemcpyAsync(s->side_rec, s->records, n * sizeof(seeqdev_hit_t), hipMemcpyDeviceToDevice, s->stream), EIO);
   HIP_TRY(hipMemcpyAsync(s->side_off, s->rec_off, n * sizeof(uint64_t), hipMemcpyDeviceToDevice, s->stream), EIO);
   HIP_TRY(hipStreamSynchronize(s->stream), EIO);
   return 0;
}

extern "C" int seeqdevScanHostBegin(seeqdev_scan_t *s, const seeqdev_pattern_t *pat, const char *host_text, size_t nbytes,
                                    int options, int want)
{
   seeqerr = 0;
   if (!s || !pat || (!host_text && nbytes)) { errno = EINVAL; return -1; }
   if (use_device(s->device)) return -1;
   if (text_upload(s, host_text, nbytes, s->prof)) return -1;
   if (s->line_hint <= 0 && !(options & SEEQDEV_SINGLELINE) && nbytes) {
      const size_t n = nbytes < SAMPLE_BYTES ? nbytes : SAMPLE_BYTES;
      size_t nl = 0;
      for (size_t i = 0; i < n; i++) nl += host_text[i] == '\n';
      s->avg_line = nl ? (double)n / (double)nl : 1e9;
      s->avg_text = s->d_text;
      s->avg_nbytes = nbytes;
   }
   return seeqdevScanRun(s, pat, s->d_text, nbytes, options, want);
}

extern "C" int seeqdevScanHost(seeqdev_scan_t *s, const seeqdev_pattern_t *pat, const char *host_text, size_t nbytes,
                               int options, int want, seeqdev_counts_t *counts)
{
   if (seeqdevScanHostBegin(s, pat, host_text, nbytes, options, want)) return -1;
   return seeqdevScanFetch(s, counts);
}

#include "seeq_multi_host.h"
#include "seeq_demux_host.h"
#include "seeq_strand_host.h"
#include "seeq_insert_host.h"
#include "seeq_tally_host.h"
#include "seeq_tally_group_host.h"
#include "seeq_tally_library_host.h"
#include "seeq_tally_collapse_host.h"
#include "seeq_qgate_host.h"

extern "C" int seeqdevScanLastCopyMs(const seeqdev_scan_t *s, float *h2d_ms)
{
   if (!s || !h2d_ms) { errno = EINVAL; return -1; }
   *h2d_ms = s->tm_h2d.ms;
   return 0;
}

extern "C" int seeqdevScanLastLaunches(const seeqdev_scan_t *s) { return s ? (int)s->prof_segs : 0; }

extern "C" float seeqdevScanLastClockMHz(const seeqdev_scan_t *s) { return s ? s->clk_mhz : 0.f; }

extern "C" int seeqdevScanLastLaunchTimes(const seeqdev_scan_t *s, float *ms, int cap)
{
   if (!s || (!ms && cap > 0)) { errno = EINVAL; return -1; }
   const size_t n = s->prof_segs < s->cap_launch_ms ? s->prof_segs : s->cap_launch_ms;
   for (size_t i = 0; i < n && (int)i < cap; i++) ms[i] = s->launch_ms[i];
   return (int)n;
}

#include "seeq_string.h"
```

seeq_amd/csrc/seeq_order.h:

```cpp
#ifndef SEEQ_ORDER_H_
#define SEEQ_ORDER_H_

#define ORDER_SCAN_ITEMS 8
#define ORDER_SCAN_BLOCK (256 * ORDER_SCAN_ITEMS)
#define ORDER_MAX_BLOCKS 1024

__global__ __launch_bounds__(256) void k_tiles_post(FusedArgs f, uint32_t nslices, uint32_t *bsum, uint32_t nb)
{
   if (blockIdx.y == 2) {
      if (blockIdx.x == 0) fused_post_body(f, nslices);
      return;
   }
   __shared__ uint32_t s_wave[4];
   uint32_t *arr = blockIdx.y == 0 ? f.tile_hits : f.tile_cl;
   const uint32_t n = f.ntiles, base = blockIdx.x * ORDER_SCAN_BLOCK;
   uint32_t item[ORDER_SCAN_ITEMS], v = 0;
#pragma unroll
   for (int k = 0; k < ORDER_SCAN_ITEMS; k++) {
      const uint32_t i = base + threadIdx.x * ORDER_SCAN_ITEMS + k;
      item[k] = i < n ? arr[i] : 0u;
      v += item[k];
   }
   uint32_t tot;
   uint32_t ex = block_excl_scan(v, &tot, s_wave);
#pragma unroll
   for (int k = 0; k < ORDER_SCAN_ITEMS; k++) {
      const uint32_t i = base + threadIdx.x * ORDER_SCAN_ITEMS + k;
      if (i < n) arr[i] = ex;
      ex += item[k];
   }
   if (threadIdx.x == 0) bsum[blockIdx.y * nb + blockIdx.x] = tot;
}

__device__ __forceinline__ void order_block_prefix(const uint32_t *bsum, uint32_t nb, uint32_t *s_ph, uint32_t *s_pc, uint32_t *s_wave)
{
   uint32_t run_h = 0, run_c = 0;
   for (uint32_t b0 = 0; b0 < nb; b0 += 256u) {
      const uint32_t i = b0 + threadIdx.x;
      const uint32_t vh = i < nb ? bsum[i] : 0u, vc = i < nb ? bsum[nb + i] : 0u;
      uint32_t th, tc;
      const uint32_t eh = block_excl_scan(vh, &th, s_wave), ec = block_excl_scan(vc, &tc, s_wave);
      if (i < nb) { s_ph[i] = run_h + eh; s_pc[i] = run_c + ec; }
      run_h += th; run_c += tc;
   }
   __syncthreads();
}

__global__ __launch_bounds__(256) void k_order(FusedArgs f, uint32_t nslices, const uint32_t *bsum, uint32_t nb, uint4 *ent)
{
   __shared__ uint32_t s_ph[ORDER_MAX_BLOCKS], s_pc[ORDER_MAX_BLOCKS], s_wave[4];
   order_block_prefix(bsum, nb, s_ph, s_pc, s_wave);
   const Counters *c = f.cnt;
   if (c->overflow & OVF_HITLINES) return;
   const uint32_t lane = threadIdx.x & 63;
   const uint32_t lines0 = (uint32_t)c->lines;
   for (uint32_t sl = blockIdx.x * 4 + (threadIdx.x >> 6); sl < nslices; sl += gridDim.x * 4) {
      const uint32_t n = f.wg_hits[sl];
      const uint4 *slice = f.tmp + (size_t)sl * f.slice_cap;
      for (uint32_t i0 = lane; i0 < n; i0 += 256) {
         uint4 e[4];
         uint32_t th[4], tc[4];
#pragma unroll
         for (int u = 0; u < 4; u++) e[u] = i0 + 64u * u < n ? slice[i0 + 64u * u] : make_uint4(0u, 0u, 0u, 0u);
#pragma unroll
         for (int u = 0; u < 4; u++) {
            const uint32_t tile = e[u].x & 0x1FFFFFFFu;
            const bool ok = i0 + 64u * u < n;
            th[u] = ok ? f.tile_hits[tile] + s_ph[tile / ORDER_SCAN_BLOCK] : 0u;
            tc[u] = ok ? f.tile_cl[tile] + s_pc[tile / ORDER_SCAN_BLOCK] : 0u;
         }
#pragma unroll
         for (int u = 0; u < 4; u++) {
            if (i0 + 64u * u >= n) continue;
            const uint32_t dst = th[u] + (e[u].y & 0x1FFFu);
            ent[dst] = make_uint4(e[u].z, lines0 + tc[u] + e[u].w + 1u , (e[u].x >> 31) | (((e[u].y >> 13) & 0x3FFFFu) << 1), (e[u].x >> 29) & 3u);
         }
      }
   }
}

__device__ __forceinline__ uint32_t order_last_nl16(const fused_v4u &v)
{
   const uint32_t g3 = nl_flags(v.w), g2 = nl_flags(v.z), g1 = nl_flags(v.y), g0 = nl_flags(v.x);
   if (g3) return 13u + ((31u - (uint32_t)__builtin_clz(g3)) >> 3);
   if (g2) return 9u + ((31u - (uint32_t)__builtin_clz(g2)) >> 3);
   if (g1) return 5u + ((31u - (uint32_t)__builtin_clz(g1)) >> 3);
   if (g0) return 1u + ((31u - (uint32_t)__builtin_clz(g0)) >> 3);
   return 0u;
}

__device__ __forceinline__ uint64_t order_line_start(const uint8_t *text, uint64_t hi)
{
   uint64_t q = hi;
   while (q >= 128) {
      fused_v4u v[8];
#pragma unroll
      for (int u = 0; u < 8; u++) v[u] = *reinterpret_cast<const fused_v4u_unaligned *>(text + q - 128 + 16 * u);
#pragma unroll
      for (int u = 7; u >= 0; u--) {
         const uint32_t r = order_last_nl16(v[u]);
         if (r) return q - 128 + 16 * u + r;
      }
      q -= 128;
   }
   while (q > 0) { if (text[q - 1] == '\n') return q; q--; }
   return 0;
}

__device__ __forceinline__ void order_marker_word(uint32_t w, uint32_t nby, uint32_t bm, uint32_t bv, uint32_t &ns, uint32_t &nb)
{
   const uint32_t keepm = nby >= 4u ? 0xFFFFFFFFu : (1u << (8u * nby)) - 1u;
   const uint32_t y = (w ^ __builtin_amdgcn_perm(0x474E5554u, 0x43FF41FFu, w & 0x07070707u)) & keepm;
   ns += (uint32_t)__popc((((y & 0x5F5F5F5Fu) + 0x7F7F7F7Fu) | y) & 0x80808080u);
   const uint32_t z = ((w & bm) ^ bv) | ~keepm;
   nb += (uint32_t)__popc(~(((z & 0x7F7F7F7Fu) + 0x7F7F7F7Fu) | z) & 0x80808080u);
}

__device__ __forceinline__ bool order_marker_holds(const ScanArgs &a, uint64_t q)
{
   const uint8_t *text = a.text;
   uint32_t ns = 0, nb = 0, len = 0;
   const uint32_t bm = a.ig_bmask * 0x01010101u, bv = a.ig_bval * 0x01010101u;
   uint64_t p = q;
   for (; p + 16 <= a.nbytes; p += 16) {
      const fused_v4u v = *reinterpret_cast<const fused_v4u_unaligned *>(text + p);
      const uint32_t f0 = nl_flags(v.x), f1 = nl_flags(v.y), f2 = nl_flags(v.z), f3 = nl_flags(v.w);
      if ((f0 | f1 | f2 | f3) == 0u) {
         order_marker_word(v.x, 4u, bm, bv, ns, nb); order_marker_word(v.y, 4u, bm, bv, ns, nb);
         order_marker_word(v.z, 4u, bm, bv, ns, nb); order_marker_word(v.w, 4u, bm, bv, ns, nb);
         len += 16u;
         if (len > (1u << 20)) return true;
         continue;
      }
      const uint32_t wf = f0 ? 0u : f1 ? 1u : f2 ? 2u : 3u;
      const uint32_t fw = f0 ? f0 : f1 ? f1 : f2 ? f2 : f3;
      const uint32_t nby = (uint32_t)__builtin_ctz(fw) >> 3;
      order_marker_word(v.x, wf > 0u ? 4u : nby, bm, bv, ns, nb);
      if (wf >= 1u) order_marker_word(v.y, wf > 1u ? 4u : nby, bm, bv, ns, nb);
      if (wf >= 2u) order_marker_word(v.z, wf > 2u ? 4u : nby, bm, bv, ns, nb);
      if (wf >= 3u) order_marker_word(v.w, nby, bm, bv, ns, nb);
      len += 4u * wf + nby;
      return ns != 0u && len - ns >= a.ig_thr && nb >= a.ig_need;
   }
   for (; p < a.nbytes && text[p] != '\n'; p++) {
      const uint32_t ch = text[p], up = ch & 0xDFu;
      if (!(up == 'A' || up == 'C' || up == 'G' || up == 'T' || up == 'U' || up == 'N')) ns++;
      if (((ch & a.ig_bmask) ^ a.ig_bval) == 0u) nb++;
      len++;
   }
   return ns != 0u && len - ns >= a.ig_thr && nb >= a.ig_need;
}

__global__ __launch_bounds__(256) void k_bounds2(ScanArgs a, uint4 *ent, uint32_t *hit_col)
{
   Counters *c = a.cnt;
   const uint32_t nhl = c->seg_nhitlines;
   const uint32_t stride = gridDim.x * 256;
   const uint64_t segb = a.seg_base + a.pos_bias;
   const uint32_t prev0 = c->prev_hit_line;
   for (uint32_t k = blockIdx.x * 256 + threadIdx.x; k < nhl; k += stride) {
      const uint4 e = ent[k];
      const uint32_t prev = k ? ent[k - 1].y : prev0;
      const uint32_t unresolved = e.z & 1u, col = e.z >> 1;
      a.hit_line[k] = e.y;
      uint32_t repeat = e.y == prev ? 1u : 0u;
      if (repeat && k != 0u && a.ig_thr != 0u) {
         const uint4 pe = ent[k - 1];
         const uint32_t pprev = k > 1u ? ent[k - 2].y : prev0;
         if ((pe.w & 3u) == 2u && pprev != pe.y) {
            const uint64_t pq = (pe.z & 1u) ? order_line_start(a.text, a.seg_base + pe.x) : a.seg_base + pe.x;
            const uint32_t pholds = (pq < a.seg_base || order_marker_holds(a, pq)) ? 1u : 0u;
            if (!pholds) repeat = 0u;
         }
      }
      if (repeat) {
         hit_col[k] = unresolved ? e.x : e.x + col;
         if (a.window_ok && e.y == prev0 && !a.first_seg) {
            bool voids = true;
            if (a.ig_thr && (e.w & 2u) && unresolved) {
               const uint64_t hp0 = a.seg_base + e.x;
               voids = hp0 < a.nbytes && order_marker_holds(a, order_line_start(a.text, hp0));
            }
            if (voids) atomicOr(&c->overflow, OVF_SEAM);
         }
         a.hit_start[k] = 0xFFFFFFFFu;
         continue;
      }
      if (!unresolved) {
         uint32_t keep = 1u;
         if (a.ig_need != 0u && (e.w & 2u) != 0u) {
            const uint32_t holds = order_marker_holds(a, a.seg_base + e.x) ? 1u : 0u;
            if (!holds) { keep = e.w & 1u; ent[k].w = e.w | 4u; }
         }
         a.hit_start[k] = keep ? e.x : 0xFFFFFFFFu; hit_col[k] = keep ? col : 0u;
         continue;
      }
      const uint64_t hp = a.seg_base + e.x;
      if (hp >= a.nbytes || hp < segb || hp >= segb + a.seg_len) {
         atomicOr(&c->overflow, OVF_BAD_ENTRY);
         a.hit_start[k] = 0xFFFFFFFFu;
         hit_col[k] = 0u;
         continue;
      }
      const uint64_t q = order_line_start(a.text, hp);
      uint32_t keep = 1u, holds = 1u;
      if (a.ig_thr != 0u && (e.w & 2u) != 0u && q >= a.seg_base) holds = order_marker_holds(a, q) ? 1u : 0u;
      if (!holds) {
         keep = e.w & 1u;
         ent[k].w = e.w | 4u;
      }
      uint32_t out_start, out_col;
      if (q < a.seg_base) { atomicOr(&c->overflow, OVF_NO_STREAM); out_start = 0xFFFFFFFFu; out_col = 0u; }
      else if (!keep) { out_start = 0xFFFFFFFFu; out_col = 0u; }
      else { out_start = (uint32_t)(q - a.seg_base); out_col = (uint32_t)(hp - q); }
      a.hit_start[k] = out_start;
      hit_col[k] = out_col;
   }
}

#endif
```

seeq_amd/csrc/seeq_post.h:

```cpp
#ifndef SEEQ_POST_H_
#define SEEQ_POST_H_

#include <hip/hip_runtime.h>
#include "seeq_types.h"
#include "seeq_scan_common.h"

#define VERIFY_ANY  0
#define VERIFY_BEST 1
#define VERIFY_ALL  2

void seeq_launch_verify(int fw, int var, unsigned grid, hipStream_t st, const ScanArgs &a, const uint32_t *eq, const uint32_t *hit_col,
                        uint4 *cache);
struct VerifyPacked;
void seeq_launch_verify_packed(int fw, int var, unsigned grid, hipStream_t st, const ScanArgs &a, const void *bases, const void *nmask, uint32_t stride,
                               uint32_t nstride, uint32_t read_len, uint64_t total_bytes, uint64_t ntotal_bytes, const uint32_t *eq, const uint32_t *hit_col, uint4 *cache);
void seeq_launch_emit1(unsigned grid, hipStream_t st, const ScanArgs &a, const uint4 *cache);
void seeq_launch_emit_all(int fw, unsigned grid, unsigned vgrid, hipStream_t st, const ScanArgs &a, const uint32_t *eq, const uint32_t *hit_col, uint4 *cache);

#define SEEQ_ORDER_MAX_BLOCKS 1024
#define SEEQ_ORDER_BLOCK      2048
void seeq_launch_tiles_post(hipStream_t st, const FusedArgs &f, uint32_t nslices, uint32_t *bsum, uint32_t nb);
void seeq_launch_order(unsigned grid, hipStream_t st, const FusedArgs &f, uint32_t nslices, const uint32_t *bsum, uint32_t nb, uint4 *ent);
void seeq_launch_bounds2(unsigned grid, hipStream_t st, const ScanArgs &a, uint4 *ent, uint32_t *hit_col);

#endif
```

seeq_amd/csrc/seeq_text_alloc.h:

```cpp
#ifndef SEEQ_TEXT_ALLOC_H_
#define SEEQ_TEXT_ALLOC_H_

extern "C" void *seeqdevHostAlloc(size_t bytes)
{
   void *p = NULL;
   hipError_t e = hipHostMalloc(&p, bytes ? bytes : 1, hipHostMallocPortable);
   if (e != hipSuccess) { snprintf(g_last_error, sizeof g_last_error, "hipHostMalloc: %s", hipGetErrorString(e)); errno = ENOMEM; return NULL; }
   return p;
}

extern "C" void seeqdevHostFree(void *p)
{
   if (p) (void)hipHostFree(p);
}

static void scan_forget(seeqdev_scan *s)
{
   s->pat = nullptr;
   s->ran = false;
   memset(&s->counts, 0, sizeof s->counts);
}

extern "C" void *seeqdevTextAllocFor(seeqdev_scan_t *scan, size_t bytes, int candidates, seeqdev_textinfo_t *info)
{
   seeqerr = 0;
   if (info) memset(info, 0, sizeof *info);
   if (bytes == 0) bytes = 1;
   void *blk[12] = {nullptr};
   size_t blk_bytes[12] = {0};
   float ms[12] = {0};
   int n = 0;
   if (candidates > 12) candidates = 12;
   if (candidates < 2 || bytes < ((size_t)64 << 20)) candidates = 1;
   size_t p2 = 1;
   while (p2 < bytes) p2 <<= 1;
   seeqdev_scan_t *sc = nullptr;
   const size_t seg = bytes < (size_t)0xF0000000u ? bytes : (size_t)0xF0000000u;
   const size_t headroom = seg / 2 + ((size_t)256 << 20);
   size_t peak = 0;
   for (int i = 0; i < candidates; i++) {
      size_t want = bytes;
      if (i > 0) {
         want = p2;
         size_t freeb = 0, total = 0;
         if (hipMemGetInfo(&freeb, &total) != hipSuccess) break;
         if (want + headroom > freeb) { want = bytes; if (want + headroom > freeb) break; }
      }
      if (hipMalloc(&blk[n], want) != hipSuccess) { (void)hipGetLastError(); blk[n] = nullptr; break; }
      blk_bytes[n] = want;
      peak += want;
      n++;
   }
   if (n == 0) { hip_fail(hipErrorOutOfMemory, "seeqdevTextAlloc", ENOMEM); return NULL; }
   int best = 0;
   if (n > 1) {
      static const char plain[] = "GATGTAGCGCGATTAGCCTG";
      char keys[20];
      for (int i = 0; i < 20; i++) keys[i] = plain[i] == 'A' ? 1 : plain[i] == 'C' ? 2 : plain[i] == 'G' ? 4 : 8;
      seeqdev_pattern_t *pat = seeqdevPatternNew(keys, 20, 3);
      sc = pat ? (scan ? scan : seeqdevScanNew(NULL)) : NULL;
      const bool own_sc = scan == nullptr;
      const bool prof_was = sc ? sc->prof : false;
      const uint64_t nreads = bytes / 151;
      bool ok = pat && sc && nreads > 0 && seeqdevScanSetProfiling(sc, 1) == 0;
      for (int i = 0; ok && i < n; i++) {
         ok = seeqdevSynthReads(blk[i], 0, nreads, 150, plain, 20, 3, 0x5EE92025ull, NULL) == 0 && hipStreamSynchronize(NULL) == hipSuccess;
         for (int rep = 0; ok && rep < 2; rep++) {
            seeqdev_counts_t cnt;
            ok = seeqdevScanRun(sc, pat, blk[i], (size_t)nreads * 151, SQ_BEST, SEEQDEV_WANT_COUNTLINES) == 0 && seeqdevScanFetch(sc, &cnt) == 0;
         }
         float t[4] = {0, 0, 0, 0};
         if (ok) ok = seeqdevScanLastTimes(sc, t) == 0;
         ms[i] = t[1];
      }
      if (sc && own_sc) seeqdevScanFree(sc);
      else if (sc) { (void)seeqdevScanSetProfiling(sc, prof_was ? 1 : 0); scan_forget(sc); }
      if (pat) seeqdevPatternFree(pat);
      if (ok) {
         for (int i = 1; i < n; i++) if (ms[i] < ms[best]) best = i;
         if (info) { for (int i = 0; i < n; i++) info->probe_ms[i] = ms[i]; info->nprobed = n; }
      }
      for (int i = 0; i < n; i++) if (i != best) (void)hipFree(blk[i]);
      seeqerr = 0;
   }
   if (info) { info->chosen = best; info->allocated_bytes = blk_bytes[best]; info->probe_peak_bytes = n > 1 ? peak + headroom : peak; }
   return blk[best];
}

extern "C" void *seeqdevTextAllocInfo(size_t bytes, int candidates, seeqdev_textinfo_t *info) { return seeqdevTextAllocFor(NULL, bytes, candidates, info); }

extern "C" void *seeqdevTextAlloc(size_t bytes, int candidates, float *probe_ms, int *nprobed)
{
   seeqdev_textinfo_t info;
   void *p = seeqdevTextAllocInfo(bytes, candidates, &info);
   if (nprobed) *nprobed = p ? info.nprobed : 0;
   if (p && probe_ms) for (int i = 0; i < info.nprobed; i++) probe_ms[i] = info.probe_ms[i];
   return p;
}

extern "C" void seeqdevTextFree(void *d_text)
{
   if (d_text) (void)hipFree(d_text);
}

#endif
```

seeq_amd/csrc/seeq_verify.h:

```cpp
#ifndef SEEQ_VERIFY_H_
#define SEEQ_VERIFY_H_

#include "seeq_post.h"

__device__ __forceinline__ uint32_t verify_top(uint32_t x, uint32_t n) { return (uint32_t)((((uint64_t)x) << 32) >> n); }

#define VERIFY_ADDR(dst, word, SEL) \
   asm("v_lshlrev_b32_sdwa %0, %1, %2 dst_sel:DWORD dst_unused:UNUSED_PAD src0_sel:DWORD src1_sel:BYTE_" #SEL : "=v"(dst) : "v"(sh), "v"(word))

#define VERIFY_BARE 0
#define VERIFY_REV  1
#define VERIFY_FWD  2
template <int W> struct verify_col;
template <> struct verify_col<1> {
   template <int MODE>
   static __device__ __forceinline__ void run(const fused_eq_t<1> &e, fused_state_t<1> &st, uint32_t lim, uint32_t &L, uint32_t &PH, uint32_t &MH, uint32_t &T)
   {
      const uint32_t eq = e.w0, pv = st.pv, mv = st.mv;
      if (MODE == VERIFY_FWD) T = __builtin_amdgcn_alignbit(eq, T, 1);
      const uint32_t s = (eq & pv) + pv;
      const uint32_t d0 = ((s ^ pv) | eq) | mv;
      const uint32_t ph = mv | ~(d0 | pv);
      const uint32_t mh = pv & d0;
      if (MODE == VERIFY_FWD) { PH = __builtin_amdgcn_alignbit(PH, ph, 31); MH = __builtin_amdgcn_alignbit(MH, mh, 31); }
      uint32_t ph2, mh2, score = st.score;
      asm("v_add_co_u32 %0, vcc, %2, %2\n\tv_addc_co_u32 %1, vcc, 0, %1, vcc" : "=v"(ph2), "+v"(score) : "v"(ph) : "vcc");
      asm("v_add_co_u32 %0, vcc, %2, %2\n\tv_subbrev_co_u32 %1, vcc, 0, %1, vcc" : "=v"(mh2), "+v"(score) : "v"(mh) : "vcc");
      st.pv = mh2 | ~(d0 | ph2);
      st.mv = ph2 & d0;
      st.score = score;
      if (MODE != VERIFY_BARE) L = __builtin_amdgcn_alignbit(L, lim - score, 31);
   }
};
template <> struct verify_col<2> {
   template <int MODE>
   static __device__ __forceinline__ void run(const fused_eq_t<2> &e, fused_state_t<2> &st, uint32_t lim, uint32_t &L, uint32_t &PH, uint32_t &MH, uint32_t &T)
   {
      const uint32_t pv0 = st.pv0, pv1 = st.pv1, mv0 = st.mv0, mv1 = st.mv1;
      if (MODE == VERIFY_FWD) T = __builtin_amdgcn_alignbit(e.w0, T, 1);
      const uint64_t pv = ((uint64_t)pv1 << 32) | pv0, eq = ((uint64_t)e.w1 << 32) | e.w0;
      const uint64_t s = (eq & pv) + pv;
      const uint32_t s0 = (uint32_t)s, s1 = (uint32_t)(s >> 32);
      const uint32_t d00 = ((s0 ^ pv0) | e.w0) | mv0, d01 = ((s1 ^ pv1) | e.w1) | mv1;
      const uint32_t ph0 = mv0 | ~(d00 | pv0), ph1 = mv1 | ~(d01 | pv1);
      const uint32_t mh0 = pv0 & d00, mh1 = pv1 & d01;
      if (MODE == VERIFY_FWD) { PH = __builtin_amdgcn_alignbit(PH, ph1, 31); MH = __builtin_amdgcn_alignbit(MH, mh1, 31); }
      uint32_t p0, p1, m0, m1, score = st.score;
      asm("v_add_co_u32 %0, vcc, %3, %3\n\tv_addc_co_u32 %1, vcc, %4, %4, vcc\n\tv_addc_co_u32 %2, vcc, 0, %2, vcc"
          : "=&v"(p0), "=&v"(p1), "+v"(score) : "v"(ph0), "v"(ph1) : "vcc");
      asm("v_add_co_u32 %0, vcc, %3, %3\n\tv_addc_co_u32 %1, vcc, %4, %4, vcc\n\tv_subbrev_co_u32 %2, vcc, 0, %2, vcc"
          : "=&v"(m0), "=&v"(m1), "+v"(score) : "v"(mh0), "v"(mh1) : "vcc");
      st.pv0 = m0 | ~(d00 | p0); st.pv1 = m1 | ~(d01 | p1);
      st.mv0 = p0 & d00;         st.mv1 = p1 & d01;
      st.score = score;
      if (MODE != VERIFY_BARE) L = __builtin_amdgcn_alignbit(L, lim - score, 31);
   }
};

template <int W, int MODE>
__device__ __forceinline__ void verify_word(uint32_t word, uint32_t eq_base, uint32_t sh, fused_state_t<W> &st, uint32_t lim,
                                            uint32_t &L, uint32_t &PH, uint32_t &MH, uint32_t &T)
{
   uint32_t a0, a1, a2, a3;
   VERIFY_ADDR(a0, word, 0); VERIFY_ADDR(a1, word, 1); VERIFY_ADDR(a2, word, 2); VERIFY_ADDR(a3, word, 3);
   const fused_eq_t<W> e0 = fused_eq_load<W>(eq_base + a0), e1 = fused_eq_load<W>(eq_base + a1),
                       e2 = fused_eq_load<W>(eq_base + a2), e3 = fused_eq_load<W>(eq_base + a3);
   if (MODE != VERIFY_REV) {
      verify_col<W>::template run<MODE>(e0, st, lim, L, PH, MH, T);
      verify_col<W>::template run<MODE>(e1, st, lim, L, PH, MH, T);
      verify_col<W>::template run<MODE>(e2, st, lim, L, PH, MH, T);
      verify_col<W>::template run<MODE>(e3, st, lim, L, PH, MH, T);
   } else {
      verify_col<W>::template run<MODE>(e3, st, lim, L, PH, MH, T);
      verify_col<W>::template run<MODE>(e2, st, lim, L, PH, MH, T);
      verify_col<W>::template run<MODE>(e1, st, lim, L, PH, MH, T);
      verify_col<W>::template run<MODE>(e0, st, lim, L, PH, MH, T);
   }
}

__device__ __forceinline__ uint32_t verify_word_of(const fused_v4u (&v)[4], int g)
{
   const fused_v4u &q = v[g >> 2];
   return (g & 3) == 0 ? q.x : (g & 3) == 1 ? q.y : (g & 3) == 2 ? q.z : q.w;
}

template <int W>
__device__ __forceinline__ uint32_t verify_reverse(const ScanArgs &a, bool need, uint64_t off, uint32_t i, uint32_t dist,
                                                   uint32_t eqr_base, uint32_t sh, uint32_t m, uint32_t tau1)
{
   constexpr int NB = W == 1 ? 32 : 64;
   constexpr int NV = NB / 16;
   const uint64_t end = off + i;
   const bool fast = need && end >= (uint64_t)NB;
   fused_v4u v[4];
   {
#pragma unroll
      for (int q = 0; q < NV; q++) v[q] = fused_v4u{0u, 0u, 0u, 0u};
      if (fast) {
         const uint8_t *p = a.text + (end - NB);
#pragma unroll
         for (int q = 0; q < NV; q++) v[q] = *reinterpret_cast<const fused_v4u_unaligned *>(p + 16 * q);
      }
   }
   fused_state_t<W> st;
   st.init(m);
   uint32_t Rh = 0, Rl = 0, dummy = 0;
   uint32_t nsteps = NB;
#pragma unroll
   for (int g = 0; g < NB / 4; g++) {
      const uint32_t seen = g < 8 ? Rh : Rl;
      const uint32_t full = (g & 7) == 0 ? 0u : (1u << (4 * (g & 7))) - 1u;
      const bool more = fast && (g < 8 || Rh == 0xFFFFFFFFu) && seen == full && 4u * g < i;
      if (!__any(more)) { nsteps = 4u * g; break; }
      const uint32_t word = verify_word_of(v, NV * 4 - 1 - g);
      verify_word<W, VERIFY_REV>(word, eqr_base, sh, st, dist, g < 8 ? Rh : Rl, dummy, dummy, dummy);
   }
   uint32_t start = 0;
   bool slow = need && !fast;
   if (fast) {
      const uint32_t nh_ = nsteps < 32u ? nsteps : 32u, nl_ = nsteps > 32u ? nsteps - 32u : 0u;
      const uint64_t F = ((uint64_t)verify_top(~Rh, nh_) << 32) | verify_top(~Rl, nl_);
      const uint32_t j = F ? (uint32_t)__builtin_clzll(F) + 1u : 0xFFFFFFFFu;
      if (j <= i) start = i - j;
      else slow = true;
   }
   if (slow) start = exact1_reverse<W>(a.text, off, a.nbytes, i, dist, eqr_base, m, tau1, nullptr);
   return start;
}

template <int VAR>
struct verify_rules {
   uint32_t prevL, latch, nhits, best_d, best_end, ce0, ce1;
   bool done;
   template <typename EMIT2>
   __device__ __forceinline__ void group(uint32_t L, uint32_t PH, uint32_t MH, uint32_t tcol, uint32_t s_in, uint32_t p0, EMIT2 second)
   {
      uint32_t Q = (L >> 1) | (prevL << 31);
      int lastj = -1;
      while (Q) {
         const uint32_t j = (uint32_t)__builtin_clz(Q);
         Q &= ~(0x80000000u >> j);
         const uint32_t below = ~(0xFFFFFFFFu >> j);
         const uint32_t streak = s_in + (uint32_t)__popc(PH & below) - (uint32_t)__popc(MH & below);
         const bool rise = j == tcol || ((PH << j) & 0x80000000u) != 0u;
         const bool zero = streak == 0u;
         const uint32_t p = p0 + j;
         if (VAR == VERIFY_BEST) {
            if ((rise || zero) && streak < best_d) { best_d = streak; best_end = p; }
         } else {
            if ((int)j != lastj + 1) latch = 0u;
            const bool emit = rise ? latch == 0u : zero;
            latch = (rise || zero) ? 1u : 0u;
            lastj = (int)j;
            if (emit) {
               if (nhits == 0u) { ce0 = p; ce1 = streak; }
               else second(p, streak);
               nhits++;
               if (VAR == VERIFY_ANY) { Q = 0; done = true; }
            }
         }
      }
      if (VAR != VERIFY_BEST && lastj != 31) latch = 0u;
      prevL = L & 1u;
   }
};

__device__ __forceinline__ bool verify_prefix_dirty(const ScanArgs &a, uint64_t off, uint32_t pos)
{
   const bool nul_only = (a.options & SQ_CONVERT) != 0;
   uint32_t bad = 0;
   for (uint32_t o = 0; __any(o < pos && bad == 0u); o += 64u) {
      if (o >= pos || bad) continue;
      const uint64_t p0 = off + o;
      fused_v4u v[4];
      if (p0 + 64 <= a.nbytes) {
#pragma unroll
         for (int q = 0; q < 4; q++) v[q] = *reinterpret_cast<const fused_v4u_unaligned *>(a.text + p0 + 16 * q);
      } else {
#pragma unroll
         for (int q = 0; q < 4; q++) v[q] = direct_load16(a.text, p0 + 16 * q, a.nbytes);
      }
      const uint32_t n = pos - o;
#pragma unroll
      for (int g = 0; g < 16; g++) {
         const uint32_t w = verify_word_of(v, g);
         const uint32_t b = nul_only ? (~(((w & 0x7F7F7F7Fu) + 0x7F7F7F7Fu) | w) & 0x80808080u) : fused_bad4(w);
         const uint32_t keep = n >= 4u * g + 4u ? 0xFFFFFFFFu : n <= 4u * g ? 0u : (1u << (8u * (n - 4u * g))) - 1u;
         bad |= b & keep;
      }
   }
   return bad != 0u;
}

template <int W, int VAR>
__device__ __forceinline__ void verify_body(const ScanArgs &a, const uint32_t *eq2, const uint32_t *hit_col, uint4 *cache)
{
   __shared__ __align__(8) uint32_t s_eqf[256 * W];
   __shared__ __align__(8) uint32_t s_eqr[256 * W];
   __shared__ uint32_t s_novf[4], s_wave[4];
   if (threadIdx.x < 4) s_novf[threadIdx.x] = 0;
   for (int i = threadIdx.x; i < 256 * W; i += 256) { s_eqf[i] = eq2[i]; s_eqr[i] = eq2[256 * W + i]; }
   __syncthreads();
   const uint32_t eqf_base = (uint32_t)(uintptr_t)(fused_lds_cu32 *)s_eqf;
   const uint32_t eqr_base = (uint32_t)(uintptr_t)(fused_lds_cu32 *)s_eqr;
   Counters *c = a.cnt;
   const uint32_t nhl = c->seg_nhitlines;
   const uint32_t m = (uint32_t)a.m, tau = (uint32_t)a.tau, tau1 = tau + 1u;
   const bool caching = cache != nullptr && a.want == SEEQDEV_WANT_RECORDS;
   const bool dirty = c->dirty != 0;
   uint32_t sh = W == 1 ? 2u : 3u;
   asm volatile("" : "+v"(sh));
   const uint32_t ovf_r = (a.cap_hitlines > nhl ? a.cap_hitlines - nhl : 0u) / (gridDim.x * 4u);
   const uint32_t wave_id = threadIdx.x >> 6;
   uint4 *const ovf_all = cache ? cache + nhl : nullptr;
   __shared__ uint16_t s_idx[1024];
   __shared__ uint32_t s_cnt[1024];
   const bool compact = a.vrange != 0u;
   const uint32_t range = (a.vrange == 512u || a.vrange == 1024u) && nhl >= 65536u ? a.vrange : 256u;
   const uint32_t nranges = (nhl + range - 1u) / range;
#define VERIFY_NR        ((nranges == 0u || nranges > gridDim.x) ? gridDim.x : nranges)
#define VERIFY_MY_LISTS  (blockIdx.x < VERIFY_NR ? (gridDim.x - blockIdx.x + VERIFY_NR - 1u) / VERIFY_NR : 0u)
#define VERIFY_LIST_ROOM (ovf_r > 1u ? ovf_r - 1u : 0u)
   for (uint32_t rg = blockIdx.x; rg < nranges; rg += gridDim.x) {
    const uint32_t r0 = rg * range;
    uint32_t nact = 0;
    if (!compact) {
       s_cnt[threadIdx.x] = 0u;
       nact = nhl - r0 < 256u ? nhl - r0 : 256u;
    }
    else for (uint32_t u = 0; u < range; u += 256u) {
       const uint32_t k = r0 + u + threadIdx.x;
       const bool live = k < nhl;
       const uint32_t kk = (a.hit_idx && live) ? a.hit_idx[k] : k;
       const bool act = live && a.hit_start[kk] != 0xFFFFFFFFu;
       s_cnt[u + threadIdx.x] = 0u;
       uint32_t tot;
       const uint32_t ex = block_excl_scan(act ? 1u : 0u, &tot, s_wave);
       if (act) s_idx[nact + ex] = (uint16_t)(u + threadIdx.x);
       if (live && !act && caching) cache[k] = make_uint4(0u, 0u, 0u, 0u);
       nact += tot;
    }
    __syncthreads();
    for (uint32_t j0 = 0; j0 < nact; j0 += 256u) {
      bool done = j0 + threadIdx.x >= nact;
      const uint32_t k = r0 + (done ? 0u : compact ? (uint32_t)s_idx[j0 + threadIdx.x] : threadIdx.x);
#define VERIFY_MINE (j0 + threadIdx.x < nact)
      const uint32_t kk = (a.hit_idx && !done) ? a.hit_idx[k] : k;
      const uint32_t hs = done ? 0u : a.hit_start[kk];
      if (hs == 0xFFFFFFFFu) done = true;
      const uint64_t off = done ? a.seg_base : a.seg_base + hs;
      if (a.use_nh == 3 && (a.options & SEEQDEV_FASTA) && !done && a.text[off] == '>') done = true;
      uint32_t pos = 0, stop_at = 0xFFFFFFFFu;
      if (!done) {
         const uint32_t col = hit_col[kk];
         if (col > a.skip_back) pos = col - a.skip_back;
         if (a.window_ok) {
            uint32_t lastcol = a.hit_last ? a.hit_last[kk] : col;
            bool unbounded = false;
            if (a.hit_idx) { unbounded = lastcol == 0xFFFFFFFFu; lastcol += a.skip_back - (m + tau1 - 1u); }
            else for (uint32_t j = k + 1; j < nhl && a.hit_start[j] == 0xFFFFFFFFu; j++) lastcol = hit_col[j] - hs;
            if (!unbounded) stop_at = lastcol + m + tau1 + 1u;
         }
      }
      if (dirty && verify_prefix_dirty(a, off, pos)) pos = 0;
      fused_state_t<W> st;
      st.init(m);
      verify_rules<VAR> r;
      r.prevL = 0; r.latch = 0; r.nhits = 0; r.best_d = tau1; r.best_end = 0; r.ce0 = 0; r.ce1 = 0; r.done = false;
      auto second = [&](uint32_t p, uint32_t streak) {
         if (VAR == VERIFY_ALL && caching) {
            const uint32_t idx = atomicAdd(&s_novf[wave_id], 1u);
            const uint32_t list_room = VERIFY_LIST_ROOM;
            if (idx < VERIFY_MY_LISTS * list_room) {
               const uint32_t t = idx / list_room;
               ovf_all[(size_t)((blockIdx.x + t * VERIFY_NR) * 4u + wave_id) * ovf_r + 1u + (idx - t * list_room)] = make_uint4(k, r.nhits, p, streak);
            }
         }
      };
      while (__any(!done)) {
         fused_v4u v[4];
         {
            const uint64_t p0 = off + pos;
            if (p0 + 64 <= a.nbytes) {
#pragma unroll
               for (int q = 0; q < 4; q++) v[q] = *reinterpret_cast<const fused_v4u_unaligned *>(a.text + p0 + 16 * q);
            } else {
#pragma unroll
               for (int q = 0; q < 4; q++) v[q] = direct_load16(a.text, p0 + 16 * q, a.nbytes);
            }
         }
         const uint32_t stop_rel = done ? 0u : stop_at - pos;
         const uint32_t s_in = st.score;
         uint32_t Lh = 0, Ll = 0, Ph = 0, Pl = 0, Mh = 0, Ml = 0, Th = 0, Tl = 0;
         uint32_t ncols = 64;
#pragma unroll
         for (int g = 0; g < 16; g++) {
            if (!__any(stop_rel > 4u * g)) { ncols = 4u * g; break; }
            verify_word<W, VERIFY_FWD>(verify_word_of(v, g), eqf_base, sh, st, tau, g < 8 ? Lh : Ll, g < 8 ? Ph : Pl, g < 8 ? Mh : Ml, g < 8 ? Th : Tl);
         }
         const uint32_t nh_ = ncols < 32u ? ncols : 32u, nl_ = ncols > 32u ? ncols - 32u : 0u;
         Lh = verify_top(~Lh, nh_); Ph = verify_top(Ph, nh_); Mh = verify_top(Mh, nh_); Th = verify_top(__builtin_bitreverse32(Th), nh_);
         Ll = verify_top(~Ll, nl_); Pl = verify_top(Pl, nl_); Ml = verify_top(Ml, nl_); Tl = verify_top(__builtin_bitreverse32(Tl), nl_);
         uint32_t tcol = Th ? (uint32_t)__builtin_clz(Th) : Tl ? 32u + (uint32_t)__builtin_clz(Tl) : 64u;
         tcol = stop_rel < tcol ? stop_rel : tcol;
         if (done) { Lh = 0; Ll = 0; r.prevL = 0; }
         if (tcol < 32u) { Lh &= ~(0xFFFFFFFFu >> tcol); Ll = 0; }
         else if (tcol < 64u) Ll &= ~(0xFFFFFFFFu >> (tcol - 32u));
         r.group(Lh, Ph, Mh, tcol, s_in, pos, second);
         if (__any(!r.done && (Ll | r.prevL) != 0u)) {
            const uint32_t s_mid = s_in + (uint32_t)__popc(Ph) - (uint32_t)__popc(Mh);
            if (!r.done) r.group(Ll, Pl, Ml, tcol - 32u, s_mid, pos + 32u, second);
         } else {
            if (VAR != VERIFY_BEST) r.latch = 0u;
            r.prevL = 0u;
         }
         if (tcol < 64u || r.done) done = true;
         pos += done ? 0u : 64u;
      }
      uint32_t nhits = r.nhits, ce0 = r.ce0, ce1 = r.ce1;
      if (VAR == VERIFY_BEST) { nhits = r.best_d < tau1 ? 1u : 0u; ce0 = r.best_end; ce1 = r.best_d; }
      uint32_t ce2 = 0, ce3 = 0;
      if (caching) {
         const bool need = VERIFY_MINE && nhits != 0u;
         if (__any(need)) {
            const uint32_t s0 = verify_reverse<W>(a, need, off, ce0, ce1, eqr_base, sh, m, tau1);
            if (need) { ce2 = s0; ce3 = 1u; }
         }
      }
      if (caching && VERIFY_MINE) cache[k] = make_uint4(ce0, ce1, ce2, ce3);
      if (VERIFY_MINE) s_cnt[k - r0] = nhits;
#undef VERIFY_MINE
    }
    __syncthreads();
    for (uint32_t u = 0; u < range && r0 + u < nhl; u += 256u) {
      const uint32_t k0 = r0 + u, k = k0 + threadIdx.x;
      const uint32_t nhits = s_cnt[u + threadIdx.x];
      uint32_t tot;
      const uint32_t ex = block_excl_scan(nhits, &tot, s_wave);
      if (k < nhl) a.nh[k] = ex;
      if (threadIdx.x == 0) a.nh_sum[k0 >> 8] = tot;
      if (a.nz_sum) {
         const uint32_t nzw = (uint32_t)__popcll(__ballot(nhits != 0u));
         if ((threadIdx.x & 63u) == 0) s_wave[wave_id] = nzw;
         __syncthreads();
         if (threadIdx.x == 0) a.nz_sum[k0 >> 8] = s_wave[0] + s_wave[1] + s_wave[2] + s_wave[3];
         __syncthreads();
      }
    }
    __syncthreads();
   }
   if (caching && (threadIdx.x & 63u) == 0) {
      const uint32_t n = s_novf[wave_id];
      if (ovf_r) {
         const uint32_t my_lists = VERIFY_MY_LISTS, list_room = VERIFY_LIST_ROOM, nr = VERIFY_NR;
         for (uint32_t t = 0; t < my_lists; t++) {
            const uint32_t before = t * list_room;
            const uint32_t cnt = n > before ? (n - before < list_room ? n - before : list_room) : 0u;
            ovf_all[(size_t)((blockIdx.x + t * nr) * 4u + wave_id) * ovf_r] = make_uint4(cnt, 0u, 0u, 0u);
         }
         if (n > my_lists * list_room) c->seg_novf = 1u;
      }
      else if (n) c->seg_novf = 1u;
#undef VERIFY_NR
#undef VERIFY_MY_LISTS
#undef VERIFY_LIST_ROOM
   }
}

__global__ __launch_bounds__(256) void k_nh_top(ScanArgs a)
{
   __shared__ uint32_t s_wave[4];
   Counters *c = a.cnt;
   const uint32_t nhl = c->seg_nhitlines;
   const uint32_t nch = (nhl + 255u) >> 8;
   uint32_t running = 0, nz = 0;
   for (uint32_t b0 = 0; b0 < nch; b0 += 2048u) {
      uint32_t item[8], v = 0;
#pragma unroll
      for (int q = 0; q < 8; q++) {
         const uint32_t i = b0 + threadIdx.x * 8u + q;
         item[q] = i < nch ? a.nh_sum[i] : 0u;
         if (a.nz_sum && i < nch) nz += a.nz_sum[i];
      }
#pragma unroll
      for (int q = 0; q < 8; q++) v += item[q];
      uint32_t tot;
      uint32_t ex = running + block_excl_scan(v, &tot, s_wave);
#pragma unroll
      for (int q = 0; q < 8; q++) {
         const uint32_t i = b0 + threadIdx.x * 8u + q;
         if (i < nch) a.nh_sum[i] = ex;
         ex += item[q];
      }
      running += tot;
   }
   if (a.nz_sum) {
      uint32_t tot;
      block_excl_scan(nz, &tot, s_wave);
      nz = tot;
   }
   if (threadIdx.x == 0) {
      c->seg_nrec = running;
      if (a.nz_sum) c->seg_nmatch = nz;
      if (a.want == SEEQDEV_WANT_RECORDS) rec_check_body(a);
      c->emit_nhl = nhl;
      c->emit_base = c->records;
      if (a.fin) seg_end_body(a, (int)a.fin - 1);
   }
}

__global__ __launch_bounds__(256) void k_emit1(ScanArgs a, const uint4 *cache)
{
   const Counters *c = a.cnt;
   if (c->overflow & OVF_RECORDS) return;
   const uint32_t nhl = c->emit_nhl;
   const uint64_t base = c->emit_base;
   for (uint32_t k = blockIdx.x * 256u + threadIdx.x; k < nhl; k += gridDim.x * 256u) {
      const uint4 ce = cache[k];
      if (!ce.w) continue;
      const uint32_t kk = a.hit_idx ? a.hit_idx[k] : k;
      const uint64_t slot = base + nh_at(a, k);
      seeqdev_hit_t h;
      h.line = a.hit_line[kk];
      h.start = ce.z;
      h.end = ce.x;
      h.dist = ce.y;
      a.records[slot] = h;
      a.rec_off[slot] = rec_off_of(a, a.seg_base + a.hit_start[kk], h.line);
   }
}

template <int W>
__global__ __launch_bounds__(256, W == 1 ? 6 : 5) void k_emit_all(ScanArgs a, const uint32_t *eq2, const uint32_t *hit_col, uint4 *cache, uint32_t vgrid)
{
   const Counters *c = a.cnt;
   if (c->overflow & OVF_RECORDS) return;
   if (c->seg_novf) { exact1_body<SQ_MODE_EMIT, W, -1, false>(a, eq2, hit_col, cache); return; }
   __shared__ __align__(8) uint32_t s_eqr[256 * W];
   for (int i = threadIdx.x; i < 256 * W; i += 256) s_eqr[i] = eq2[256 * W + i];
   __syncthreads();
   const uint32_t eqr_base = (uint32_t)(uintptr_t)(fused_lds_cu32 *)s_eqr;
   const uint32_t nhl = c->seg_nhitlines;
   const uint64_t base = c->records;
   const uint32_t m = (uint32_t)a.m, tau1 = (uint32_t)a.tau + 1u;
   uint32_t sh = W == 1 ? 2u : 3u;
   asm volatile("" : "+v"(sh));
   for (uint32_t k = blockIdx.x * 256u + threadIdx.x; k < nhl; k += gridDim.x * 256u) {
      const uint4 ce = cache[k];
      if (!ce.w) continue;
      const uint32_t kk = a.hit_idx ? a.hit_idx[k] : k;
      const uint64_t slot = base + nh_at(a, k);
      seeqdev_hit_t h;
      h.line = a.hit_line[kk];
      h.start = ce.z;
      h.end = ce.x;
      h.dist = ce.y;
      a.records[slot] = h;
      a.rec_off[slot] = rec_off_of(a, a.seg_base + a.hit_start[kk], h.line);
   }
   const uint32_t nlists = vgrid * 4u;
   const uint32_t ovf_r = (a.cap_hitlines > nhl ? a.cap_hitlines - nhl : 0u) / nlists;
   if (!ovf_r) return;
   const uint32_t lane = threadIdx.x & 63u;
   for (uint32_t l = blockIdx.x * 4u + (threadIdx.x >> 6); l < nlists; l += gridDim.x * 4u) {
      const uint4 *ovf = cache + nhl + (size_t)l * ovf_r;
      const uint32_t novf = (uint32_t)__builtin_amdgcn_readfirstlane((int)ovf[0].x);
      for (uint32_t e0 = 1u; e0 <= novf; e0 += 64u) {
         const bool need = e0 + lane <= novf;
         const uint4 o = need ? ovf[e0 + lane] : make_uint4(0u, 0u, 0u, 0u);
         const uint32_t ox = (need && a.hit_idx) ? a.hit_idx[o.x] : o.x;
         const uint32_t hs = need ? a.hit_start[ox] : 0u;
         const uint64_t off = a.seg_base + hs;
         const uint32_t s0 = verify_reverse<W>(a, need, off, o.z, o.w, eqr_base, sh, m, tau1);
         if (need) {
            const uint64_t slot = base + nh_at(a, o.x) + o.y;
            seeqdev_hit_t h;
            h.line = a.hit_line[ox];
            h.start = s0;
            h.end = o.z;
            h.dist = o.w;
            a.records[slot] = h;
            a.rec_off[slot] = rec_off_of(a, off, h.line);
         }
      }
   }
}

template <int W, int VAR, int OCC>
__global__ __launch_bounds__(256, OCC) void k_verify(ScanArgs a, const uint32_t *eq2, const uint32_t *hit_col, uint4 *cache)
{
   verify_body<W, VAR>(a, eq2, hit_col, cache);
}

#undef VERIFY_ADDR

#endif
```

seeq_amd/csrc/seeq_verify.hip:

```cpp
#include <hip/hip_runtime.h>

#include <stdint.h>

#include "seeq_amd.h"
#include "seeq_kernel_core.h"
#include "seeq_types.h"
#include "seeq_scan_common.h"
#include "seeq_direct.h"
#include "seeq_exact1.h"
#include "seeq_verify.h"
#include "seeq_verify_packed.h"
#include "seeq_order.h"
#include "seeq_post.h"

void seeq_launch_verify(int fw, int var, unsigned grid, hipStream_t st, const ScanArgs &a, const uint32_t *eq, const uint32_t *hit_col,
                        uint4 *cache)
{
#define SEEQ_VERIFY(WW, VV) hipLaunchKernelGGL((k_verify<WW, VV, (WW == 1 ? 6 : 5)>), dim3(grid), dim3(256), 0, st, a, eq, hit_col, cache)
   if (fw == 1) {
      if (var == VERIFY_BEST) SEEQ_VERIFY(1, VERIFY_BEST); else if (var == VERIFY_ALL) SEEQ_VERIFY(1, VERIFY_ALL); else SEEQ_VERIFY(1, VERIFY_ANY);
   } else {
      if (var == VERIFY_BEST) SEEQ_VERIFY(2, VERIFY_BEST); else if (var == VERIFY_ALL) SEEQ_VERIFY(2, VERIFY_ALL); else SEEQ_VERIFY(2, VERIFY_ANY);
   }
#undef SEEQ_VERIFY
   hipLaunchKernelGGL(k_nh_top, dim3(1), dim3(256), 0, st, a);
}

void seeq_launch_emit1(unsigned grid, hipStream_t st, const ScanArgs &a, const uint4 *cache)
{
   hipLaunchKernelGGL(k_emit1, dim3(grid), dim3(256), 0, st, a, cache);
}

void seeq_launch_emit_all(int fw, unsigned grid, unsigned vgrid, hipStream_t st, const ScanArgs &a, const uint32_t *eq, const uint32_t *hit_col, uint4 *cache)
{
   if (fw == 1) hipLaunchKernelGGL(k_emit_all<1>, dim3(grid), dim3(256), 0, st, a, eq, hit_col, cache, vgrid);
   else hipLaunchKernelGGL(k_emit_all<2>, dim3(grid), dim3(256), 0, st, a, eq, hit_col, cache, vgrid);
}

static_assert(ORDER_MAX_BLOCKS == SEEQ_ORDER_MAX_BLOCKS && ORDER_SCAN_BLOCK == SEEQ_ORDER_BLOCK, "seeq_order.h / seeq_post.h");

void seeq_launch_tiles_post(hipStream_t st, const FusedArgs &f, uint32_t nslices, uint32_t *bsum, uint32_t nb)
{
   hipLaunchKernelGGL(k_tiles_post, dim3(nb ? nb : 1, 3), dim3(256), 0, st, f, nslices, bsum, nb);
}

void seeq_launch_order(unsigned grid, hipStream_t st, const FusedArgs &f, uint32_t nslices, const uint32_t *bsum, uint32_t nb, uint4 *ent)
{
   hipLaunchKernelGGL(k_order, dim3(grid), dim3(256), 0, st, f, nslices, bsum, nb, ent);
}

void seeq_launch_bounds2(unsigned grid, hipStream_t st, const ScanArgs &a, uint4 *ent, uint32_t *hit_col)
{
   hipLaunchKernelGGL(k_bounds2, dim3(grid), dim3(256), 0, st, a, ent, hit_col);
}

void seeq_launch_verify_packed(int fw, int var, unsigned grid, hipStream_t st, const ScanArgs &a, const void *bases, const void *nmask, uint32_t stride,
                               uint32_t nstride, uint32_t read_len, uint64_t total_bytes, uint64_t ntotal_bytes, const uint32_t *eq, const uint32_t *hit_col, uint4 *cache)
{
   VerifyPacked pk;
   pk.bases = (const uint8_t *)bases; pk.nmask = (const uint8_t *)nmask; pk.stride = stride; pk.nstride = nstride; pk.read_len = read_len;
   pk.total_bytes = total_bytes; pk.ntotal_bytes = ntotal_bytes;
#define SEEQ_VERIFYP(WW, VV) hipLaunchKernelGGL((k_verify_packed<WW, VV>), dim3(grid), dim3(256), 0, st, a, pk, eq, hit_col, cache)
   if (fw == 1) {
      if (var == VERIFY_BEST) SEEQ_VERIFYP(1, VERIFY_BEST); else if (var == VERIFY_ALL) SEEQ_VERIFYP(1, VERIFY_ALL); else SEEQ_VERIFYP(1, VERIFY_ANY);
   } else {
      if (var == VERIFY_BEST) SEEQ_VERIFYP(2, VERIFY_BEST); else if (var == VERIFY_ALL) SEEQ_VERIFYP(2, VERIFY_ALL); else SEEQ_VERIFYP(2, VERIFY_ANY);
   }
#undef SEEQ_VERIFYP
   hipLaunchKernelGGL(k_nh_top, dim3(1), dim3(256), 0, st, a);
}
```

Measured before the change: 26.68 billion.

## Batch post-scan kernels across groups of segments with per-segment workspace regions

```diff
diff --git a/seeq_amd/csrc/seeq_device.hip b/seeq_amd/csrc/seeq_device.hip
--- a/seeq_amd/csrc/seeq_device.hip
+++ b/seeq_amd/csrc/seeq_device.hip
@@ -372,6 +372,7 @@
 #include "seeq_plan.h"
 #include "seeq_workspace.h"
 #include "seeq_rerun.h"
+#include "seeq_post_group.h"
 
 struct OccMemo { const void *fn; size_t lds; int per_cu; };
 
@@ -437,6 +438,7 @@
       uint32_t *wg_lastnl;
    } ow;
    size_t cap_ftiles, cap_slices;
+   unsigned post_group, ws_regions;
    uint32_t *d_eqtab, *h_eqtab;
    unsigned long eq_pat_id; int eq_options;
    double avg_line;
@@ -598,7 +600,7 @@
       e = hipStreamCreateWithFlags(&s->stream, hipStreamDefault);
       s->own_stream = true;
    }
-   if (e == hipSuccess && ws_make(&s->ws, {{s->d_cnt, sizeof(Counters)}, {s->h_cnt, sizeof(Counters), WS_PINNED}, {s->h_eqtab, 2048 * sizeof(uint32_t), WS_PINNED},
+   if (e == hipSuccess && ws_make(&s->ws, {{s->d_cnt, (1 + SEEQ_POST_GROUP_MAX) * sizeof(Counters)}, {s->h_cnt, sizeof(Counters), WS_PINNED}, {s->h_eqtab, 2048 * sizeof(uint32_t), WS_PINNED},
                                            {s->d_eqtab, 2048 * sizeof(uint32_t)}, {s->h_sample, SAMPLE_BYTES, WS_PINNED}}))
       e = hipErrorOutOfMemory;
    {
@@ -618,6 +620,8 @@
       v = getenv("SEEQ_PACKED_QUAD");  kn.no_packed_quad = v && atoi(v) == 0;
       v = getenv("SEEQ_PACKED_SEG_READS");
       s->pk_seg_reads = v && atol(v) >= 64 && (size_t)atol(v) <= ((size_t)1 << 26) ? (size_t)atol(v) & ~(size_t)63 : PACKED_SEG_READS_DEFAULT;
+      s->post_group = seeq_post_group_knob(getenv("SEEQ_POST_GROUP"));
+      s->ws_regions = s->post_group;
       s->ncu = 256;
       s->lds_per_wg = 65536;
       s->lds_per_cu = 65536;
@@ -658,21 +662,32 @@
 
 static size_t fastq_bsum_words(size_t n) { return 2 * (n / SEEQ_TILE + 2); }
 
+static int reserve_regions(seeqdev_scan *s, size_t regions, size_t ftiles, size_t slices, size_t max_hitlines)
+{
+   Workspace *w = &s->ws;
+   const size_t R = regions;
+   if (ftiles && ws_grow(w, &s->cap_ftiles, ftiles, {{s->ow.tile_cl, R * ftiles * sizeof(uint32_t)}, {s->ow.tile_dirty, ftiles * sizeof(uint32_t)},
+                                                     {s->ow.tile_dmask, ftiles * sizeof(uint64_t)}, {s->ow.tile_hits, R * ftiles * sizeof(uint32_t)}})) return -1;
+   if (slices && ws_grow(w, &s->cap_slices, slices, {{s->ow.wg_hits, R * slices * sizeof(uint32_t)}, {s->ow.wg_part, R * 4 * slices * sizeof(uint32_t)},
+                                                     {s->ow.wg_lastnl, slices * sizeof(uint32_t)}})) return -1;
+   return ws_grow(w, &s->cap_hitlines, max_hitlines, {{s->hit_start, R * max_hitlines * sizeof(uint32_t)}, {s->hit_line, R * max_hitlines * sizeof(uint32_t)},
+                                                      {s->ow.tmp, R * max_hitlines * sizeof(uint4)}, {s->nh, R * max_hitlines * sizeof(uint32_t)},
+                                                      {s->hit_col, R * max_hitlines * sizeof(uint32_t)}, {s->ent, R * max_hitlines * sizeof(uint4)},
+                                                      {s->nh_sum, R * seeq_post_nhsum_words(max_hitlines) * sizeof(uint32_t)}});
+}
+
 static int reserve_impl(seeqdev_scan *s, size_t max_bytes, size_t max_lines, size_t max_hitlines, size_t max_records)
 {
    seeqerr = 0;
    if (!s) { errno = EINVAL; return -1; }
    Workspace *w = &s->ws;
+   size_t ftiles = 0, slices = 0;
    if (max_bytes) {
       const size_t seg = max_bytes < s->seg_bytes ? max_bytes : s->seg_bytes;
       const size_t tiles = (seg + TILE - 1) / TILE + 1;
       if (ws_grow(w, &s->cap_tiles, tiles, {{s->tile_cnt, tiles * sizeof(uint32_t)}})) return -1;
-      const size_t ftiles = seg / FUSED_MIN_TILE + 2;
-      const size_t slices = MAX_FUSED_GRID;
-      if (ws_grow(w, &s->cap_ftiles, ftiles, {{s->ow.tile_cl, ftiles * sizeof(uint32_t)}, {s->ow.tile_dirty, ftiles * sizeof(uint32_t)},
-                                              {s->ow.tile_dmask, ftiles * sizeof(uint64_t)}, {s->ow.tile_hits, ftiles * sizeof(uint32_t)}})) return -1;
-      if (ws_grow(w, &s->cap_slices, slices, {{s->ow.wg_hits, slices * sizeof(uint32_t)}, {s->ow.wg_part, 4 * slices * sizeof(uint32_t)},
-                                              {s->ow.wg_lastnl, slices * sizeof(uint32_t)}})) return -1;
+      ftiles = seg / FUSED_MIN_TILE + 2;
+      slices = MAX_FUSED_GRID;
    }
    if (max_lines > s->cap_lines) {
       const size_t chunks = (max_lines + 63) / 64 + 1;
@@ -681,10 +696,12 @@
                                                 {s->hdr_off, chunks * sizeof(uint32_t)}})) return -1;
       s->cap_chunks = chunks;
    }
-   if (ws_grow(w, &s->cap_hitlines, max_hitlines, {{s->hit_start, max_hitlines * sizeof(uint32_t)}, {s->hit_line, max_hitlines * sizeof(uint32_t)},
-                                                   {s->ow.tmp, max_hitlines * sizeof(uint4)}, {s->nh, max_hitlines * sizeof(uint32_t)},
-                                                   {s->hit_col, max_hitlines * sizeof(uint32_t)}, {s->ent, max_hitlines * sizeof(uint4)},
-                                                   {s->nh_sum, 2 * (max_hitlines / 256 + 2) * sizeof(uint32_t)}})) return -1;
+   if (reserve_regions(s, s->ws_regions, ftiles, slices, max_hitlines)) {
+      if (s->ws_regions == 1 || errno != ENOMEM) return -1;
+      s->ws_regions = 1;
+      if (reserve_regions(s, 1, ftiles, slices, max_hitlines)) return -1;
+      seeqerr = 0;
+   }
    if (s->fq_ws && max_records > s->cap_records) {
       if (ws_grow(w, &s->cap_records, max_records, {{s->records, max_records * sizeof(seeqdev_hit_t)}, {s->rec_off, max_records * sizeof(uint64_t)},
                                                     {s->fq_rec, max_records * sizeof(seeqdev_hit_t)}, {s->fq_off, max_records * sizeof(uint64_t)},
@@ -702,6 +719,10 @@
    if (s->cap_ftiles > largest) largest = s->cap_ftiles;
    size_t nb = largest / SCAN_BLOCK + 2;
    if (3 * (s->cap_ftiles / SCAN_BLOCK + 2) > nb) nb = 3 * (s->cap_ftiles / SCAN_BLOCK + 2);
+   {
+      const size_t ob = 2 * (size_t)s->ws_regions * (s->cap_ftiles / SEEQ_ORDER_BLOCK + 1);
+      if (ob > nb) nb = ob;
+   }
    return ensure_scan_ws(s, nb);
 }
 
@@ -946,7 +967,8 @@
    return 0;
 }
 
-static int seg_onepass(seeqdev_scan *s, const SegRun &r, ScanArgs &a, size_t sg, hipEvent_t *ev, bool &order2, uint32_t &stream_ntiles)
+static int seg_onepass(seeqdev_scan *s, const SegRun &r, ScanArgs &a, size_t sg, hipEvent_t *ev, bool &order2, uint32_t &stream_ntiles,
+                       const PostGroup *pg = nullptr, unsigned z = 0, FusedArgs *fout = nullptr)
 {
    const ScanPlan &plan = r.plan;
    const seeqdev_pattern *pat = s->pat;
@@ -966,6 +988,10 @@
    f.tile_dirty = f.wg_lastnl ? ow.tile_dirty : nullptr;
    f.tile_dmask = f.wg_lastnl ? ow.tile_dmask : nullptr;
    f.cnt = s->d_cnt;
+   if (pg) {
+      f.tile_cl += (size_t)z * pg->tile_stride; f.tile_hits += (size_t)z * pg->tile_stride; f.tmp += (size_t)z * pg->hl_stride;
+      f.wg_hits += (size_t)z * pg->slice_stride; f.wg_part += (size_t)z * pg->slice_stride * 4;
+   }
    f.clk_probe = (s->prof && s->clk_probe && plan.use_pair) ? s->clk_probe + 4 * sg : nullptr;
    uint32_t pos_bias = 0;
    if (plan.use_stream) {
@@ -974,9 +1000,7 @@
       f.skip_thr = plan.skip_thr;
       if (plan.use_pair) { f.dfa = pat->d_pair; f.dfa_rows = pat->pair_units; f.dfa_final_base = 0; f.pair = 1; f.ig_thr = plan.ig ? (uint32_t)(pat->wlen - pat->tau) : 0u; }
       if (plan.use_myers) { f.dfa = (const uint16_t *)(s->d_eqtab + (size_t)512 * plan.fw); f.dfa_rows = (uint32_t)(64 * plan.fw); f.dfa_final_base = 0; f.pair = 2; }
-      uint64_t room = 0xFFFFFFF0ull - a.seg_len;
-      if (room > ((uint64_t)1 << 30)) room = (uint64_t)1 << 30;
-      pos_bias = (uint32_t)(a.seg_base < room ? a.seg_base : room) & ~127u;
+      pos_bias = seeq_stream_pos_bias(a.seg_base, a.seg_len);
       f.pos_bias = pos_bias;
    }
    if (ev) { HIP_TRY(hipEventRecord(ev[0], st), EIO); HIP_TRY(hipEventRecord(ev[1], st), EIO); }
@@ -989,6 +1013,7 @@
    else if (plan.use_direct && plan.fw == 2) hipLaunchKernelGGL((k_direct<4, 2>), dim3(r.fused_grid), dim3(256), 0, st, f);
    else hipLaunchKernelGGL((k_direct<4, 1>), dim3(r.fused_grid), dim3(256), 0, st, f);
    if (ev) HIP_TRY(hipEventRecord(ev[2], st), EIO);
+   if (fout) *fout = f;
    const uint32_t order_nb = (f.ntiles + SEEQ_ORDER_BLOCK - 1) / SEEQ_ORDER_BLOCK;
    order2 = plan.order2 && order_nb <= SEEQ_ORDER_MAX_BLOCKS && 2 * (size_t)order_nb <= s->cap_scan_ws;
    if (plan.ig) {
@@ -1006,12 +1031,13 @@
       }
    }
    const unsigned rgrid = nsl / 4 + 1 < 2048 ? nsl / 4 + 1 : 2048;
-   if (order2) {
+   if (pg) {}
+   else if (order2) {
       seeq_launch_tiles_post(st, f, (uint32_t)nsl, s->scan_ws, order_nb);
       seeq_launch_order(rgrid, st, f, (uint32_t)nsl, (const uint32_t *)s->scan_ws, order_nb, s->ent);
    }
    else hipLaunchKernelGGL(k_fused_post, dim3(1), dim3(256), 0, st, f, (uint32_t)nsl);
-   if (!order2 && (s->want != SEEQDEV_WANT_COUNTLINES || plan.superset)) {
+   if (!pg && !order2 && (s->want != SEEQDEV_WANT_COUNTLINES || plan.superset)) {
       launch_scanset(st, s->scan_ws, f.tile_hits, f.tile_cl, f.tile_dirty, f.ntiles, nullptr, nullptr, f.tile_dirty ? &s->d_cnt->seg_dirty_tiles : nullptr);
       if (plan.use_stream) hipLaunchKernelGGL(k_stream_reorder, dim3(rgrid), dim3(256), 0, st, f, (uint32_t)nsl, s->hit_start, s->hit_line, s->nh, s->hit_col);
       else hipLaunchKernelGGL(k_fused_reorder, dim3(rgrid), dim3(256), 0, st, f, (uint32_t)nsl, s->hit_start, s->hit_line);
@@ -1136,6 +1162,48 @@
    return 0;
 }
 
+static unsigned post_group_of(const seeqdev_scan *s, const SegRun &r)
+{
+   const ScanPlan &plan = r.plan;
+   if (s->post_group < 2 || !(plan.use_fused && plan.use_stream && plan.order2 && plan.verify)) return 0;
+   if (plan.ig || s->multi_active || plan.leaders || plan.stream_ll || plan.pair_ll) return 0;
+   if (s->want == SEEQDEV_WANT_COUNTLINES && !plan.superset) return 0;
+   if (s->want == SEEQDEV_WANT_RECORDS && !plan.need_nh) return 0;
+   const uint32_t seg_len = seeq_post_seg_len(s->nbytes, r.seg_bytes, 0);
+   const uint32_t order_nb = seeq_post_order_blocks(seeq_post_tiles(seg_len, r.tile_bytes));
+   if (seeq_post_tiles(seg_len, r.tile_bytes) > s->cap_ftiles || (size_t)r.fused_grid * r.nw > s->cap_slices) return 0;
+   const unsigned g = seeq_post_group_size(s->post_group, s->ws_regions, order_nb, s->cap_scan_ws);
+   return g;
+}
+
+static int group_post(seeqdev_scan *s, const SegRun &r, ScanArgs &a, const FusedArgs &f, PostGroup &g)
+{
+   const ScanPlan &plan = r.plan;
+   const int want = s->want, fw = plan.fw;
+   hipStream_t st = s->stream;
+   const unsigned nsl = r.fused_grid * r.nw;
+   const unsigned rgrid = nsl / 4 + 1 < 2048 ? nsl / 4 + 1 : 2048;
+   const uint32_t order_nb = seeq_post_order_blocks(g.row[0].ntiles);
+   g.grp = s->d_cnt + 1;
+   g.tot = s->d_cnt;
+   g.end_flags = (uint32_t)seg_end_flags(plan.need_nh, plan.superset, plan.nh_is_count);
+   seeq_launch_tiles_post_group(st, f, g, (uint32_t)nsl, s->scan_ws, order_nb);
+   seeq_launch_order_group(rgrid, st, f, g, (uint32_t)nsl, (const uint32_t *)s->scan_ws, s->ent);
+   const unsigned grid_hits = capped_grid(s, s->cap_hitlines, 16);
+   seeq_launch_bounds2_group(grid_hits, st, a, g, s->ent, s->hit_col);
+   uint4 *ecache = (plan.need_nh && want == SEEQDEV_WANT_RECORDS) ? s->ow.tmp : nullptr;
+   const uint32_t *eqp = (const uint32_t *)s->d_eqtab;
+   const int var = verify_variant(want, s->options, plan.nh_is_count, (int)g.end_flags, &a.fin);
+   a.fin = 0;
+   a.nh_sum = s->nh_sum;
+   a.nz_sum = plan.superset && plan.nh_is_count ? s->nh_sum + (s->cap_hitlines / 256 + 2) : nullptr;
+   a.vrange = (plan.use_pair ? s->pat->pair_parts > 1 : s->pat->sdfa_parts > 1) ? 512u : 0u;
+   seeq_launch_verify_group(fw, var, grid_hits, st, a, g, eqp, s->hit_col, ecache);
+   if (want == SEEQDEV_WANT_RECORDS && var != VERIFY_ALL) seeq_launch_emit1_group(grid_hits, st, a, g, ecache);
+   else if (want == SEEQDEV_WANT_RECORDS) seeq_launch_emit_all_group(fw, grid_hits, grid_hits, st, a, g, eqp, s->hit_col, ecache);
+   return 0;
+}
+
 template <int W>
 static int run_segments(seeqdev_scan *s)
 {
@@ -1148,8 +1216,19 @@
    const ScanPlan &plan = r.plan;
    const seeqdev_pattern *pat = s->pat;
    const size_t nbytes = s->nbytes;
+   const unsigned gsize = post_group_of(s, r);
+   PostGroup pg;
+   memset(&pg, 0, sizeof pg);
+   FusedArgs f0;
+   ScanArgs a0;
+   unsigned gn = 0;
    for (size_t sg = 0; sg < r.nseg; sg++) {
       hipEvent_t *ev = s->prof ? s->ev + 4 * sg : NULL;
+      const unsigned z = gsize ? (unsigned)(sg % gsize) : 0;
+      if (gsize && z == 0) {
+         gn = seeq_post_group_rows(&pg, nbytes, r.seg_bytes, r.tile_bytes, sg, gsize);
+         seeq_post_group_strides(&pg, s->cap_hitlines, s->cap_ftiles, s->cap_slices, seeq_post_order_blocks(pg.row[0].ntiles));
+      }
       uint32_t stream_ntiles = 0;
       bool order2 = false;
       ScanArgs a;
@@ -1172,6 +1251,14 @@
       a.window_ok = plan.window_ok ? 1u : 0u;
       a.cnt = c;
 
+      if (gsize) {
+         if (seg_onepass(s, r, a, sg, ev, order2, stream_ntiles, &pg, z, z == 0 ? &f0 : nullptr)) return -1;
+         if (z == 0) a0 = a;
+         if (z + 1 == gn && group_post(s, r, a0, f0, pg)) return -1;
+         if (ev) HIP_TRY(hipEventRecord(ev[3], st), EIO);
+         HIP_TRY(hipGetLastError(), EIO);
+         continue;
+      }
       if (plan.use_fused) { if (seg_onepass(s, r, a, sg, ev, order2, stream_ntiles)) return -1; }
       else if (seg_index_forward<W>(s, r, a, ev)) return -1;
       if (s->want != SEEQDEV_WANT_COUNTLINES || plan.superset) {
diff --git a/seeq_amd/csrc/seeq_order.h b/seeq_amd/csrc/seeq_order.h
--- a/seeq_amd/csrc/seeq_order.h
+++ b/seeq_amd/csrc/seeq_order.h
@@ -1,11 +1,54 @@
 #ifndef SEEQ_ORDER_H_
 #define SEEQ_ORDER_H_
+
+#include "seeq_post_group.h"
 
 #define ORDER_SCAN_ITEMS 8
 #define ORDER_SCAN_BLOCK (256 * ORDER_SCAN_ITEMS)
 #define ORDER_MAX_BLOCKS 1024
 
-__global__ __launch_bounds__(256) void k_tiles_post(FusedArgs f, uint32_t nslices, uint32_t *bsum, uint32_t nb)
+__device__ __forceinline__ void post_group_fused(FusedArgs &f, const PostGroup &g, uint32_t z)
+{
+   const PostGroupRow &r = g.row[z];
+   f.seg_base = r.base + r.pos_bias; f.seg_len = r.seg_len; f.first_seg = r.first_seg; f.pos_bias = r.pos_bias; f.ntiles = r.ntiles;
+   f.tile_cl += (size_t)z * g.tile_stride; f.tile_hits += (size_t)z * g.tile_stride;
+   f.tmp += (size_t)z * g.hl_stride;
+   f.wg_hits += (size_t)z * g.slice_stride; f.wg_part += (size_t)z * g.slice_stride * 4;
+   f.cnt = g.grp + z;
+}
+
+__device__ __forceinline__ void post_group_args(ScanArgs &a, const PostGroup &g, uint32_t z)
+{
+   const PostGroupRow &r = g.row[z];
+   a.seg_base = r.base; a.seg_len = r.seg_len; a.first_seg = r.first_seg; a.pos_bias = r.pos_bias; a.stream_ntiles = r.ntiles;
+   a.hit_start += (size_t)z * g.hl_stride; a.hit_line += (size_t)z * g.hl_stride; a.nh += (size_t)z * g.hl_stride;
+   a.nh_sum += (size_t)z * g.nhsum_stride;
+   if (a.nz_sum) a.nz_sum += (size_t)z * g.nhsum_stride;
+   a.cnt = g.grp + z;
+}
+
+struct PostGroupView { uint32_t lines0, nhl, dirty, hl_ovf; };
+__device__ __forceinline__ PostGroupView post_group_view(const PostGroup &g, uint32_t z)
+{
+   const Counters *t = g.tot;
+   uint32_t lines = (uint32_t)t->lines, ovf = t->overflow, dirty = t->dirty;
+   for (uint32_t i = 0; i < z; i++) {
+      const Counters *c = g.grp + i;
+      lines += c->seg_nlines - c->seg_nheaders;
+      ovf |= c->overflow;
+      dirty |= c->dirty;
+   }
+   ovf |= g.grp[z].overflow;
+   dirty |= g.grp[z].dirty;
+   PostGroupView v;
+   v.lines0 = lines;
+   v.hl_ovf = ovf & OVF_HITLINES;
+   v.nhl = v.hl_ovf ? 0u : g.grp[z].seg_nhitlines;
+   v.dirty = dirty;
+   return v;
+}
+
+__device__ __forceinline__ void tiles_post_body(const FusedArgs &f, uint32_t nslices, uint32_t *bsum, uint32_t nb)
 {
    if (blockIdx.y == 2) {
       if (blockIdx.x == 0) fused_post_body(f, nslices);
@@ -30,6 +73,21 @@
       ex += item[k];
    }
    if (threadIdx.x == 0) bsum[blockIdx.y * nb + blockIdx.x] = tot;
+}
+
+__global__ __launch_bounds__(256) void k_tiles_post(FusedArgs f, uint32_t nslices, uint32_t *bsum, uint32_t nb) { tiles_post_body(f, nslices, bsum, nb); }
+
+__global__ __launch_bounds__(256) void k_tiles_post_g(FusedArgs f, PostGroup g, uint32_t nslices, uint32_t *bsum)
+{
+   const uint32_t z = blockIdx.z;
+   post_group_fused(f, g, z);
+   const uint32_t nb = (f.ntiles + ORDER_SCAN_BLOCK - 1) / ORDER_SCAN_BLOCK;
+   if (blockIdx.y == 2) {
+      if (blockIdx.x != 0) return;
+      if (threadIdx.x == 0) { Counters zero = {}; *f.cnt = zero; }
+   }
+   else if (blockIdx.x >= nb) return;
+   tiles_post_body(f, nslices, bsum + (size_t)z * g.bsum_stride, nb);
 }
 
 __device__ __forceinline__ void order_block_prefix(const uint32_t *bsum, uint32_t nb, uint32_t *s_ph, uint32_t *s_pc, uint32_t *s_wave)
@@ -46,14 +104,12 @@
    __syncthreads();
 }
 
-__global__ __launch_bounds__(256) void k_order(FusedArgs f, uint32_t nslices, const uint32_t *bsum, uint32_t nb, uint4 *ent)
+__device__ __forceinline__ void order_body(const FusedArgs &f, uint32_t nslices, const uint32_t *bsum, uint32_t nb, uint4 *ent, uint32_t lines0, uint32_t hl_ovf)
 {
    __shared__ uint32_t s_ph[ORDER_MAX_BLOCKS], s_pc[ORDER_MAX_BLOCKS], s_wave[4];
    order_block_prefix(bsum, nb, s_ph, s_pc, s_wave);
-   const Counters *c = f.cnt;
-   if (c->overflow & OVF_HITLINES) return;
+   if (hl_ovf) return;
    const uint32_t lane = threadIdx.x & 63;
-   const uint32_t lines0 = (uint32_t)c->lines;
    for (uint32_t sl = blockIdx.x * 4 + (threadIdx.x >> 6); sl < nslices; sl += gridDim.x * 4) {
       const uint32_t n = f.wg_hits[sl];
       const uint4 *slice = f.tmp + (size_t)sl * f.slice_cap;
@@ -77,6 +133,19 @@
          }
       }
    }
+}
+
+__global__ __launch_bounds__(256) void k_order(FusedArgs f, uint32_t nslices, const uint32_t *bsum, uint32_t nb, uint4 *ent)
+{
+   order_body(f, nslices, bsum, nb, ent, (uint32_t)f.cnt->lines, f.cnt->overflow & OVF_HITLINES);
+}
+
+__global__ __launch_bounds__(256) void k_order_g(FusedArgs f, PostGroup g, uint32_t nslices, const uint32_t *bsum, uint4 *ent)
+{
+   const uint32_t z = blockIdx.z;
+   const PostGroupView v = post_group_view(g, z);
+   post_group_fused(f, g, z);
+   order_body(f, nslices, bsum + (size_t)z * g.bsum_stride, (f.ntiles + ORDER_SCAN_BLOCK - 1) / ORDER_SCAN_BLOCK, ent + (size_t)z * g.hl_stride, v.lines0, v.hl_ovf);
 }
 
 __device__ __forceinline__ uint32_t order_last_nl16(const fused_v4u &v)
@@ -151,13 +220,11 @@
    return ns != 0u && len - ns >= a.ig_thr && nb >= a.ig_need;
 }
 
-__global__ __launch_bounds__(256) void k_bounds2(ScanArgs a, uint4 *ent, uint32_t *hit_col)
+__device__ __forceinline__ void bounds2_body(ScanArgs &a, uint4 *ent, uint32_t *hit_col, uint32_t nhl, uint32_t prev0)
 {
    Counters *c = a.cnt;
-   const uint32_t nhl = c->seg_nhitlines;
    const uint32_t stride = gridDim.x * 256;
    const uint64_t segb = a.seg_base + a.pos_bias;
-   const uint32_t prev0 = c->prev_hit_line;
    for (uint32_t k = blockIdx.x * 256 + threadIdx.x; k < nhl; k += stride) {
       const uint4 e = ent[k];
       const uint32_t prev = k ? ent[k - 1].y : prev0;
@@ -190,7 +257,7 @@
          uint32_t keep = 1u;
          if (a.ig_need != 0u && (e.w & 2u) != 0u) {
             const uint32_t holds = order_marker_holds(a, a.seg_base + e.x) ? 1u : 0u;
-            if (!holds) { keep = e.w & 1u; ent[k].w = e.w | 4u; }
+            if (!holds) { keep = e.w & 1u; atomicOr(&ent[k].w, 4u); }
          }
          a.hit_start[k] = keep ? e.x : 0xFFFFFFFFu; hit_col[k] = keep ? col : 0u;
          continue;
@@ -207,7 +274,7 @@
       if (a.ig_thr != 0u && (e.w & 2u) != 0u && q >= a.seg_base) holds = order_marker_holds(a, q) ? 1u : 0u;
       if (!holds) {
          keep = e.w & 1u;
-         ent[k].w = e.w | 4u;
+         atomicOr(&ent[k].w, 4u);
       }
       uint32_t out_start, out_col;
       if (q < a.seg_base) { atomicOr(&c->overflow, OVF_NO_STREAM); out_start = 0xFFFFFFFFu; out_col = 0u; }
@@ -218,4 +285,24 @@
    }
 }
 
+__global__ __launch_bounds__(256) void k_bounds2(ScanArgs a, uint4 *ent, uint32_t *hit_col)
+{
+   bounds2_body(a, ent, hit_col, a.cnt->seg_nhitlines, a.cnt->prev_hit_line);
+}
+
+__global__ __launch_bounds__(256) void k_bounds2_g(ScanArgs a, PostGroup g, uint4 *ent, uint32_t *hit_col)
+{
+   const uint32_t z = blockIdx.z;
+   const PostGroupView v = post_group_view(g, z);
+   if (v.nhl == 0u) return;
+   uint32_t prev0 = g.tot->prev_hit_line;
+   if (a.use_nh == 3u)
+      for (uint32_t i = z; i-- > 0u; ) {
+         const uint32_t n = g.grp[i].seg_nhitlines;
+         if (n) { prev0 = ent[(size_t)i * g.hl_stride + n - 1u].y; break; }
+      }
+   post_group_args(a, g, z);
+   bounds2_body(a, ent + (size_t)z * g.hl_stride, hit_col + (size_t)z * g.hl_stride, v.nhl, prev0);
+}
+
 #endif
diff --git a/seeq_amd/csrc/seeq_post.h b/seeq_amd/csrc/seeq_post.h
--- a/seeq_amd/csrc/seeq_post.h
+++ b/seeq_amd/csrc/seeq_post.h
@@ -4,6 +4,7 @@
 #include <hip/hip_runtime.h>
 #include "seeq_types.h"
 #include "seeq_scan_common.h"
+#include "seeq_post_group.h"
 
 #define VERIFY_ANY  0
 #define VERIFY_BEST 1
@@ -23,4 +24,12 @@
 void seeq_launch_order(unsigned grid, hipStream_t st, const FusedArgs &f, uint32_t nslices, const uint32_t *bsum, uint32_t nb, uint4 *ent);
 void seeq_launch_bounds2(unsigned grid, hipStream_t st, const ScanArgs &a, uint4 *ent, uint32_t *hit_col);
 
+void seeq_launch_tiles_post_group(hipStream_t st, const FusedArgs &f, const PostGroup &g, uint32_t nslices, uint32_t *bsum, uint32_t nb);
+void seeq_launch_order_group(unsigned grid, hipStream_t st, const FusedArgs &f, const PostGroup &g, uint32_t nslices, const uint32_t *bsum, uint4 *ent);
+void seeq_launch_bounds2_group(unsigned grid, hipStream_t st, const ScanArgs &a, const PostGroup &g, uint4 *ent, uint32_t *hit_col);
+void seeq_launch_verify_group(int fw, int var, unsigned grid, hipStream_t st, const ScanArgs &a, const PostGroup &g, const uint32_t *eq, const uint32_t *hit_col,
+                              uint4 *cache);
+void seeq_launch_emit1_group(unsigned grid, hipStream_t st, const ScanArgs &a, const PostGroup &g, const uint4 *cache);
+void seeq_launch_emit_all_group(int fw, unsigned grid, unsigned vgrid, hipStream_t st, const ScanArgs &a, const PostGroup &g, const uint32_t *eq, const uint32_t *hit_col, uint4 *cache);
+
 #endif
diff --git a/seeq_amd/csrc/seeq_post_group.h b/seeq_amd/csrc/seeq_post_group.h
--- /dev/null
+++ b/seeq_amd/csrc/seeq_post_group.h
@@ -0,0 +1,102 @@
+#ifndef SEEQ_POST_GROUP_H_
+#define SEEQ_POST_GROUP_H_
+
+#include <stddef.h>
+#include <stdint.h>
+#include <stdlib.h>
+#include "seeq_types.h"
+
+#define SEEQ_POST_GROUP_MAX     8
+#define SEEQ_POST_GROUP_DEFAULT 4
+#define SEEQ_POST_ORDER_MAX_BLOCKS 1024
+#define SEEQ_POST_ORDER_BLOCK      2048
+
+struct PostGroupRow {
+   uint64_t base;
+   uint32_t seg_len;
+   uint32_t ntiles;
+   uint32_t pos_bias;
+   uint32_t first_seg;
+};
+
+struct PostGroup {
+   uint32_t  n;
+   uint32_t  hl_stride;
+   uint32_t  tile_stride;
+   uint32_t  slice_stride;
+   uint32_t  bsum_stride;
+   uint32_t  nhsum_stride;
+   uint32_t  end_flags;
+   uint32_t  pad;
+   Counters *grp;
+   Counters *tot;
+   PostGroupRow row[SEEQ_POST_GROUP_MAX];
+};
+
+static inline unsigned seeq_post_group_knob(const char *env)
+{
+   if (!env || !*env) return SEEQ_POST_GROUP_DEFAULT;
+   char *end = NULL;
+   const long v = strtol(env, &end, 10);
+   if (*end || v < 1 || v > SEEQ_POST_GROUP_MAX) return SEEQ_POST_GROUP_DEFAULT;
+   return (unsigned)v;
+}
+
+static inline uint32_t seeq_stream_pos_bias(uint64_t seg_base, uint32_t seg_len)
+{
+   uint64_t room = 0xFFFFFFF0ull - seg_len;
+   if (room > ((uint64_t)1 << 30)) room = (uint64_t)1 << 30;
+   return (uint32_t)(seg_base < room ? seg_base : room) & ~127u;
+}
+
+static inline uint32_t seeq_post_tiles(uint32_t seg_len, uint32_t tile_bytes) { return (uint32_t)(((uint64_t)seg_len + tile_bytes - 1) / tile_bytes); }
+static inline uint32_t seeq_post_order_blocks(uint32_t ntiles) { return (ntiles + SEEQ_POST_ORDER_BLOCK - 1) / SEEQ_POST_ORDER_BLOCK; }
+static inline size_t seeq_post_nhsum_words(size_t cap_hitlines) { return 2 * (cap_hitlines / 256 + 2); }
+
+static inline size_t seeq_post_nseg(uint64_t nbytes, uint64_t seg_bytes) { return nbytes ? (size_t)((nbytes + seg_bytes - 1) / seg_bytes) : 0; }
+static inline uint32_t seeq_post_seg_len(uint64_t nbytes, uint64_t seg_bytes, size_t sg)
+{
+   const uint64_t base = (uint64_t)sg * seg_bytes;
+   return (uint32_t)(nbytes - base < seg_bytes ? nbytes - base : seg_bytes);
+}
+
+static inline unsigned seeq_post_group_size(unsigned knob, unsigned ws_regions, uint32_t order_nb, size_t cap_bsum_words)
+{
+   if (order_nb > SEEQ_POST_ORDER_MAX_BLOCKS || 2 * (size_t)order_nb > cap_bsum_words) return 0;
+   unsigned g = knob < ws_regions ? knob : ws_regions;
+   if (g > SEEQ_POST_GROUP_MAX) g = SEEQ_POST_GROUP_MAX;
+   if (g < 1) g = 1;
+   while (g > 1 && 2 * (size_t)order_nb * g > cap_bsum_words) g--;
+   return g;
+}
+
+static inline unsigned seeq_post_group_rows(PostGroup *g, uint64_t nbytes, uint64_t seg_bytes, uint32_t tile_bytes, size_t sg0, unsigned gsize)
+{
+   const size_t nseg = seeq_post_nseg(nbytes, seg_bytes);
+   unsigned n = 0;
+   for (; n < gsize && n < SEEQ_POST_GROUP_MAX && sg0 + n < nseg; n++) {
+      const uint64_t seg_base = (uint64_t)(sg0 + n) * seg_bytes;
+      PostGroupRow &r = g->row[n];
+      r.seg_len = seeq_post_seg_len(nbytes, seg_bytes, sg0 + n);
+      r.pos_bias = seeq_stream_pos_bias(seg_base, r.seg_len);
+      r.base = seg_base - r.pos_bias;
+      r.ntiles = seeq_post_tiles(r.seg_len, tile_bytes);
+      r.first_seg = sg0 + n == 0 ? 1u : 0u;
+   }
+   g->n = n;
+   return n;
+}
+
+static inline void seeq_post_group_strides(PostGroup *g, size_t cap_hitlines, size_t cap_ftiles, size_t cap_slices, uint32_t order_nb)
+{
+   g->hl_stride = (uint32_t)cap_hitlines;
+   g->tile_stride = (uint32_t)cap_ftiles;
+   g->slice_stride = (uint32_t)cap_slices;
+   g->bsum_stride = 2 * order_nb;
+   g->nhsum_stride = (uint32_t)seeq_post_nhsum_words(cap_hitlines);
+}
+
+static inline uint32_t seeq_post_region_of(const PostGroup *g, uint64_t i) { return (uint32_t)(i / g->hl_stride); }
+static inline uint32_t seeq_post_entry_of(const PostGroup *g, uint64_t i) { return (uint32_t)(i % g->hl_stride); }
+
+#endif
diff --git a/seeq_amd/csrc/seeq_text_alloc.h b/seeq_amd/csrc/seeq_text_alloc.h
--- a/seeq_amd/csrc/seeq_text_alloc.h
+++ b/seeq_amd/csrc/seeq_text_alloc.h
@@ -36,7 +36,8 @@
    while (p2 < bytes) p2 <<= 1;
    seeqdev_scan_t *sc = nullptr;
    const size_t seg = bytes < (size_t)0xF0000000u ? bytes : (size_t)0xF0000000u;
-   const size_t headroom = seg / 2 + ((size_t)256 << 20);
+   const size_t regions = scan ? scan->ws_regions : seeq_post_group_knob(getenv("SEEQ_POST_GROUP"));
+   const size_t headroom = seg / 2 + (regions - 1) * (seg / 12) + ((size_t)256 << 20);
    size_t peak = 0;
    for (int i = 0; i < candidates; i++) {
       size_t want = bytes;
diff --git a/seeq_amd/csrc/seeq_verify.h b/seeq_amd/csrc/seeq_verify.h
--- a/seeq_amd/csrc/seeq_verify.h
+++ b/seeq_amd/csrc/seeq_verify.h
@@ -193,7 +193,7 @@
 }
 
 template <int W, int VAR>
-__device__ __forceinline__ void verify_body(const ScanArgs &a, const uint32_t *eq2, const uint32_t *hit_col, uint4 *cache)
+__device__ __forceinline__ void verify_body(const ScanArgs &a, const uint32_t *eq2, const uint32_t *hit_col, uint4 *cache, const uint32_t nhl, const bool dirty)
 {
    __shared__ __align__(8) uint32_t s_eqf[256 * W];
    __shared__ __align__(8) uint32_t s_eqr[256 * W];
@@ -204,10 +204,8 @@
    const uint32_t eqf_base = (uint32_t)(uintptr_t)(fused_lds_cu32 *)s_eqf;
    const uint32_t eqr_base = (uint32_t)(uintptr_t)(fused_lds_cu32 *)s_eqr;
    Counters *c = a.cnt;
-   const uint32_t nhl = c->seg_nhitlines;
    const uint32_t m = (uint32_t)a.m, tau = (uint32_t)a.tau, tau1 = tau + 1u;
    const bool caching = cache != nullptr && a.want == SEEQDEV_WANT_RECORDS;
-   const bool dirty = c->dirty != 0;
    uint32_t sh = W == 1 ? 2u : 3u;
    asm volatile("" : "+v"(sh));
    const uint32_t ovf_r = (a.cap_hitlines > nhl ? a.cap_hitlines - nhl : 0u) / (gridDim.x * 4u);
@@ -409,7 +407,68 @@
    }
 }
 
-__global__ __launch_bounds__(256) void k_emit1(ScanArgs a, const uint4 *cache)
+__global__ __launch_bounds__(256) void k_nh_top_g(ScanArgs a0, PostGroup g)
+{
+   __shared__ uint32_t s_wave[4];
+   __shared__ uint32_t s_nhl;
+   Counters *t = g.tot;
+   for (uint32_t z = 0; z < g.n; z++) {
+      ScanArgs a = a0;
+      post_group_args(a, g, z);
+      Counters *gz = g.grp + z;
+      if (threadIdx.x == 0) {
+         t->overflow |= gz->overflow;
+         t->dirty |= gz->dirty;
+         if (gz->need_hitlines > t->need_hitlines) t->need_hitlines = gz->need_hitlines;
+         const uint32_t hits = (t->overflow & OVF_HITLINES) ? 0u : gz->seg_nhitlines;
+         t->seg_nlines = gz->seg_nlines; t->seg_nheaders = gz->seg_nheaders; t->seg_last_nl = gz->seg_last_nl;
+         t->seg_nhitlines = hits; t->seg_novf = gz->seg_novf;
+         s_nhl = hits;
+      }
+      __syncthreads();
+      const uint32_t nhl = s_nhl;
+      const uint32_t nch = (nhl + 255u) >> 8;
+      uint32_t running = 0, nz = 0;
+      for (uint32_t b0 = 0; b0 < nch; b0 += 2048u) {
+         uint32_t item[8], v = 0;
+#pragma unroll
+         for (int q = 0; q < 8; q++) {
+            const uint32_t i = b0 + threadIdx.x * 8u + q;
+            item[q] = i < nch ? a.nh_sum[i] : 0u;
+            if (a.nz_sum && i < nch) nz += a.nz_sum[i];
+         }
+#pragma unroll
+         for (int q = 0; q < 8; q++) v += item[q];
+         uint32_t tot;
+         uint32_t ex = running + block_excl_scan(v, &tot, s_wave);
+#pragma unroll
+         for (int q = 0; q < 8; q++) {
+            const uint32_t i = b0 + threadIdx.x * 8u + q;
+            if (i < nch) a.nh_sum[i] = ex;
+            ex += item[q];
+         }
+         running += tot;
+      }
+      if (a.nz_sum) {
+         uint32_t tot;
+         block_excl_scan(nz, &tot, s_wave);
+         nz = tot;
+      }
+      if (threadIdx.x == 0) {
+         a.cnt = t;
+         t->seg_nrec = running;
+         if (a.nz_sum) t->seg_nmatch = nz;
+         if (a.want == SEEQDEV_WANT_RECORDS) rec_check_body(a);
+         t->emit_nhl = nhl;
+         t->emit_base = t->records;
+         *gz = *t;
+         seg_end_body(a, (int)g.end_flags);
+      }
+      __syncthreads();
+   }
+}
+
+__device__ __forceinline__ void emit1_body(const ScanArgs &a, const uint4 *cache)
 {
    const Counters *c = a.cnt;
    if (c->overflow & OVF_RECORDS) return;
@@ -430,8 +489,17 @@
    }
 }
 
+__global__ __launch_bounds__(256) void k_emit1(ScanArgs a, const uint4 *cache) { emit1_body(a, cache); }
+
+__global__ __launch_bounds__(256) void k_emit1_g(ScanArgs a, PostGroup g, const uint4 *cache)
+{
+   const uint32_t z = blockIdx.z;
+   post_group_args(a, g, z);
+   emit1_body(a, cache + (size_t)z * g.hl_stride);
+}
+
 template <int W>
-__global__ __launch_bounds__(256, W == 1 ? 6 : 5) void k_emit_all(ScanArgs a, const uint32_t *eq2, const uint32_t *hit_col, uint4 *cache, uint32_t vgrid)
+__device__ __forceinline__ void emit_all_body(const ScanArgs &a, const uint32_t *eq2, const uint32_t *hit_col, uint4 *cache, uint32_t vgrid)
 {
    const Counters *c = a.cnt;
    if (c->overflow & OVF_RECORDS) return;
@@ -486,10 +554,33 @@
    }
 }
 
+template <int W>
+__global__ __launch_bounds__(256, W == 1 ? 6 : 5) void k_emit_all(ScanArgs a, const uint32_t *eq2, const uint32_t *hit_col, uint4 *cache, uint32_t vgrid)
+{
+   emit_all_body<W>(a, eq2, hit_col, cache, vgrid);
+}
+
+template <int W>
+__global__ __launch_bounds__(256, W == 1 ? 6 : 5) void k_emit_all_g(ScanArgs a, PostGroup g, const uint32_t *eq2, const uint32_t *hit_col, uint4 *cache, uint32_t vgrid)
+{
+   const uint32_t z = blockIdx.z;
+   post_group_args(a, g, z);
+   emit_all_body<W>(a, eq2, hit_col + (size_t)z * g.hl_stride, cache + (size_t)z * g.hl_stride, vgrid);
+}
+
 template <int W, int VAR, int OCC>
 __global__ __launch_bounds__(256, OCC) void k_verify(ScanArgs a, const uint32_t *eq2, const uint32_t *hit_col, uint4 *cache)
 {
-   verify_body<W, VAR>(a, eq2, hit_col, cache);
+   verify_body<W, VAR>(a, eq2, hit_col, cache, a.cnt->seg_nhitlines, a.cnt->dirty != 0);
+}
+
+template <int W, int VAR, int OCC>
+__global__ __launch_bounds__(256, OCC) void k_verify_g(ScanArgs a, PostGroup g, const uint32_t *eq2, const uint32_t *hit_col, uint4 *cache)
+{
+   const uint32_t z = blockIdx.z;
+   const PostGroupView v = post_group_view(g, z);
+   post_group_args(a, g, z);
+   verify_body<W, VAR>(a, eq2, hit_col + (size_t)z * g.hl_stride, cache ? cache + (size_t)z * g.hl_stride : nullptr, v.nhl, v.dirty != 0u);
 }
 
 #undef VERIFY_ADDR
diff --git a/seeq_amd/csrc/seeq_verify.hip b/seeq_amd/csrc/seeq_verify.hip
--- a/seeq_amd/csrc/seeq_verify.hip
+++ b/seeq_amd/csrc/seeq_verify.hip
@@ -8,9 +8,9 @@
 #include "seeq_scan_common.h"
 #include "seeq_direct.h"
 #include "seeq_exact1.h"
+#include "seeq_order.h"
 #include "seeq_verify.h"
 #include "seeq_verify_packed.h"
-#include "seeq_order.h"
 #include "seeq_post.h"
 
 void seeq_launch_verify(int fw, int var, unsigned grid, hipStream_t st, const ScanArgs &a, const uint32_t *eq, const uint32_t *hit_col,
@@ -69,3 +69,44 @@
 #undef SEEQ_VERIFYP
    hipLaunchKernelGGL(k_nh_top, dim3(1), dim3(256), 0, st, a);
 }
+
+void seeq_launch_tiles_post_group(hipStream_t st, const FusedArgs &f, const PostGroup &g, uint32_t nslices, uint32_t *bsum, uint32_t nb)
+{
+   hipLaunchKernelGGL(k_tiles_post_g, dim3(nb ? nb : 1, 3, g.n), dim3(256), 0, st, f, g, nslices, bsum);
+}
+
+void seeq_launch_order_group(unsigned grid, hipStream_t st, const FusedArgs &f, const PostGroup &g, uint32_t nslices, const uint32_t *bsum, uint4 *ent)
+{
+   hipLaunchKernelGGL(k_order_g, dim3(grid, 1, g.n), dim3(256), 0, st, f, g, nslices, bsum, ent);
+}
+
+void seeq_launch_bounds2_group(unsigned grid, hipStream_t st, const ScanArgs &a, const PostGroup &g, uint4 *ent, uint32_t *hit_col)
+{
+   hipLaunchKernelGGL(k_bounds2_g, dim3(grid, 1, g.n), dim3(256), 0, st, a, g, ent, hit_col);
+}
+
+void seeq_launch_verify_group(int fw, int var, unsigned grid, hipStream_t st, const ScanArgs &a, const PostGroup &g, const uint32_t *eq, const uint32_t *hit_col,
+                              uint4 *cache)
+{
+#define SEEQ_VERIFY_G(WW, VV) hipLaunchKernelGGL((k_verify_g<WW, VV, (WW == 1 ? 6 : 5)>), dim3(grid, 1, g.n), dim3(256), 0, st, a, g, eq, hit_col, cache)
+   if (fw == 1) {
+      if (var == VERIFY_BEST) SEEQ_VERIFY_G(1, VERIFY_BEST); else if (var == VERIFY_ALL) SEEQ_VERIFY_G(1, VERIFY_ALL); else SEEQ_VERIFY_G(1, VERIFY_ANY);
+   } else {
+      if (var == VERIFY_BEST) SEEQ_VERIFY_G(2, VERIFY_BEST); else if (var == VERIFY_ALL) SEEQ_VERIFY_G(2, VERIFY_ALL); else SEEQ_VERIFY_G(2, VERIFY_ANY);
+   }
+#undef SEEQ_VERIFY_G
+   hipLaunchKernelGGL(k_nh_top_g, dim3(1), dim3(256), 0, st, a, g);
+}
+
+void seeq_launch_emit1_group(unsigned grid, hipStream_t st, const ScanArgs &a, const PostGroup &g, const uint4 *cache)
+{
+   hipLaunchKernelGGL(k_emit1_g, dim3(grid, 1, g.n), dim3(256), 0, st, a, g, cache);
+}
+
+void seeq_launch_emit_all_group(int fw, unsigned grid, unsigned vgrid, hipStream_t st, const ScanArgs &a, const PostGroup &g, const uint32_t *eq, const uint32_t *hit_col, uint4 *cache)
+{
+   if (fw == 1) hipLaunchKernelGGL(k_emit_all_g<1>, dim3(grid, 1, g.n), dim3(256), 0, st, a, g, eq, hit_col, cache, vgrid);
+   else hipLaunchKernelGGL(k_emit_all_g<2>, dim3(grid, 1, g.n), dim3(256), 0, st, a, g, eq, hit_col, cache, vgrid);
+}
+
+static_assert(SEEQ_POST_ORDER_MAX_BLOCKS == SEEQ_ORDER_MAX_BLOCKS && SEEQ_POST_ORDER_BLOCK == SEEQ_ORDER_BLOCK, "seeq_post_group.h / seeq_post.h");
```

New measurement: 27.33 billion (median of 6 runs). 1.02x the previous value.
